# patrickfrey/strusPattern

Hardware: AMD Instinct MI355X
Metric: GB/s input text scanned + matches/s, 10k-regex lexer + 10k-rule automaton (higher is better)
Workload: dtype u64; 1 GPU; configs[4] per-GPU shard: 10001 regexes + 10000 token rules, 12288 docs x 64KiB UTF-8 per step (the same 805 MB resident in HBM every step; configs[4] asks 32 GB per GPU: 39 such steps)

## Files before the change

include/strus_pattern_amd.h:

```cpp
#ifndef STRUS_PATTERN_AMD_H
#define STRUS_PATTERN_AMD_H
#include <stddef.h>
#include <stdint.h>

#ifdef __cplusplus
extern "C" {
#endif

#define SP_OK                    0
#define SP_ERR_INVALID          -1
#define SP_ERR_NOMEM            -2
#define SP_ERR_DEVICE           -3
#define SP_ERR_COMPILE          -4
#define SP_ERR_MATCH            -5
#define SP_ERR_UNAVAILABLE      -6

#define SP_DOC_OK                0
#define SP_DOC_ERR_ORDER         1
#define SP_DOC_ERR_ARENA         2
#define SP_DOC_ERR_KEYTRIGGERS   3
#define SP_DOC_ERR_PASTFOLLOW    4
#define SP_DOC_ERR_RANGE         5
#define SP_DOC_ERR_DATAREF       6
#define SP_DOC_ERR_LEXEMSIZE     7
#define SP_DOC_ERR_INTERNAL      8
#define SP_DOC_ERR_OUTPUT        9

enum sp_join_op {
	SP_OP_SEQUENCE = 0, SP_OP_SEQUENCE_IMM = 1, SP_OP_SEQUENCE_STRUCT = 2,
	SP_OP_WITHIN = 3, SP_OP_WITHIN_STRUCT = 4, SP_OP_ANY = 5, SP_OP_AND = 6
};

enum sp_position_bind {
	SP_BIND_CONTENT = 0, SP_BIND_SUCCESSOR = 1, SP_BIND_PREDECESSOR = 2, SP_BIND_UNIQUE = 3
};

typedef struct sp_lexem {
	uint32_t id;
	uint32_t ordpos;
	uint32_t origpos;
	uint32_t origsize;
} sp_lexem_t;

typedef struct sp_result {
	uint32_t handle;
	uint32_t ordpos;
	uint32_t ordend;
	uint32_t origseg;
	uint32_t origpos;
	uint32_t origendseg;
	uint32_t origend;
	uint32_t item_begin;
	uint32_t item_count;
} sp_result_t;

typedef struct sp_result_item {
	uint32_t variable;
	uint32_t ordpos;
	uint32_t ordend;
	uint32_t origseg;
	uint32_t origpos;
	uint32_t origendseg;
	uint32_t origend;
} sp_result_item_t;

typedef struct sp_matcher_stats {
	double nofProgramsInstalled;
	double nofAltKeyProgramsInstalled;
	double nofSignalsFired;
	double nofTriggersAvgActive;
} sp_matcher_stats_t;

typedef struct sp_matcher sp_matcher_t;
typedef struct sp_matcher_ctx sp_matcher_ctx_t;
typedef struct sp_lexer sp_lexer_t;
typedef struct sp_lexer_ctx sp_lexer_ctx_t;

const char* sp_version(void);
int sp_device_count(void);
void sp_free(void* p);
void sp_test_fail_alloc_above(uint64_t bytes);


sp_matcher_t* sp_matcher_create(void);
void sp_matcher_free(sp_matcher_t* m);
const char* sp_matcher_last_error(const sp_matcher_t* m);

int sp_matcher_define_term_frequency(sp_matcher_t* m, uint32_t termid, double df);
int sp_matcher_push_term(sp_matcher_t* m, uint32_t termid);
int sp_matcher_push_expression(sp_matcher_t* m, int joinop, size_t argc, uint32_t range, uint32_t cardinality);
int sp_matcher_push_pattern(sp_matcher_t* m, const char* name);
int sp_matcher_attach_variable(sp_matcher_t* m, const char* name);
int sp_matcher_define_pattern(sp_matcher_t* m, const char* name, const char* formatstring, int visible);
int sp_matcher_define_option(sp_matcher_t* m, const char* name, double value);
int sp_matcher_compile(sp_matcher_t* m);
uint32_t sp_matcher_pattern_id(const sp_matcher_t* m, const char* name);
const char* sp_matcher_pattern_name(const sp_matcher_t* m, uint32_t handle);
uint32_t sp_matcher_variable_id(const sp_matcher_t* m, const char* name);
const char* sp_matcher_variable_name(const sp_matcher_t* m, uint32_t variable);
size_t sp_matcher_dump_table(const sp_matcher_t* m, uint32_t** out);
int sp_matcher_fast_tier(const sp_matcher_t* m, char* why, size_t whysize);
int sp_matcher_result_set_tier(const sp_matcher_t* m, char* why, size_t whysize, uint32_t* alt_programs);

int sp_matcher_serialize(const sp_matcher_t* m, void** blob, size_t* size);
sp_matcher_t* sp_matcher_deserialize(const void* blob, size_t size, char* err, size_t errsize);

uint32_t sp_matcher_format_count(const sp_matcher_t* m);
const char* sp_matcher_format_string(const sp_matcher_t* m, uint32_t format_handle);

sp_matcher_ctx_t* sp_matcher_ctx_create(const sp_matcher_t* m, int device);
#define SP_CTX_RESULT_SETS       1u
sp_matcher_ctx_t* sp_matcher_ctx_create_ex(const sp_matcher_t* m, int device, uint32_t flags);
void sp_matcher_ctx_free(sp_matcher_ctx_t* c);
const char* sp_matcher_ctx_last_error(const sp_matcher_ctx_t* c);

int sp_matcher_ctx_put_input(sp_matcher_ctx_t* c, const sp_lexem_t* lexems, const uint32_t* origseg, size_t n);
int sp_matcher_ctx_fetch_results(sp_matcher_ctx_t* c, sp_result_t** results, size_t* nresults,
                                 sp_result_item_t** items, size_t* nitems);
int sp_matcher_ctx_fetch_formats(sp_matcher_ctx_t* c, const uint32_t** result_format, const uint32_t** item_format);
int sp_matcher_ctx_statistics(sp_matcher_ctx_t* c, sp_matcher_stats_t* out);
int sp_matcher_ctx_reset(sp_matcher_ctx_t* c);

typedef struct sp_match_batch {
	size_t ndocs;
	size_t nresults;
	size_t nitems;
	sp_result_t* results;
	sp_result_item_t* items;
	uint64_t* doc_result_offsets;
	uint64_t* doc_stats;
	int32_t* doc_status;
	uint32_t* result_format;
	uint32_t* item_format;
} sp_match_batch_t;

int sp_matcher_ctx_match_docs(sp_matcher_ctx_t* c, const sp_lexem_t* lexems, const uint32_t* origseg,
                              const uint64_t* doc_offsets, size_t ndocs, sp_match_batch_t* out);
void sp_match_batch_free(sp_match_batch_t* b);

typedef struct sp_match_device_batch {
	size_t ndocs;
	void* d_results;
	void* d_items;
	void* d_doc_result_offsets;
	void* d_doc_stats;
	void* d_doc_status;
	void* d_counters;
	void* d_result_format;
	void* d_item_format;
} sp_match_device_batch_t;
int sp_matcher_ctx_match_docs_device(sp_matcher_ctx_t* c, const void* d_lexems, const void* d_origseg,
                                     const void* d_doc_offsets, size_t ndocs, size_t nlexems,
                                     void* stream, sp_match_device_batch_t* out);
int sp_matcher_ctx_match_lexed_device(sp_matcher_ctx_t* c, const void* d_lexems, const void* d_doc_ranges,
                                      size_t ndocs, size_t nlexems_hint, void* stream, sp_match_device_batch_t* out);
typedef struct sp_match_finished_batch {
	size_t ndocs;
	void* d_results;
	void* d_items;
	void* d_doc_result_offsets;
	void* d_doc_item_offsets;
	void* d_result_format;
	void* d_item_format;
	void* d_totals;
} sp_match_finished_batch_t;
int sp_matcher_ctx_batch_finish_device(sp_matcher_ctx_t* c, void* stream, sp_match_finished_batch_t* out);
int sp_matcher_ctx_finished_fetch(sp_matcher_ctx_t* c, sp_match_batch_t* out);
int sp_matcher_ctx_last_finish_ms(sp_matcher_ctx_t* c, double* count_ms, double* offsets_ms, double* place_ms);
int sp_matcher_ctx_batch_fetch(sp_matcher_ctx_t* c, sp_match_batch_t* out);
int sp_matcher_ctx_batch_fetch_docs(sp_matcher_ctx_t* c, size_t first_doc, size_t ndocs, sp_match_batch_t* out);
int sp_matcher_ctx_batch_counters(sp_matcher_ctx_t* c, uint64_t counters[8]);
double sp_matcher_ctx_last_kernel_ms(sp_matcher_ctx_t* c);
int sp_matcher_ctx_kernel_kind(const sp_matcher_ctx_t* c);
const char* sp_matcher_ctx_kernel_name(const sp_matcher_ctx_t* c);
int sp_matcher_ctx_batch_status(sp_matcher_ctx_t* c, int32_t* status, size_t ndocs);
int sp_matcher_ctx_grow_arena(sp_matcher_ctx_t* c);
int sp_matcher_ctx_reserve_output(sp_matcher_ctx_t* c, uint64_t results, uint64_t items);
int sp_matcher_ctx_set_arena(sp_matcher_ctx_t* c, uint32_t max_rules, uint32_t max_triggers, uint32_t bucket_capacity,
                             uint32_t max_items, uint32_t max_follow);


sp_lexer_t* sp_lexer_create(void);
void sp_lexer_free(sp_lexer_t* l);
const char* sp_lexer_last_error(const sp_lexer_t* l);
// ... 54 lines not shown
```

struspattern_amd/__init__.py:

```python
import ctypes

import numpy as np

from . import capi
from .capi import SpLexem, SpResult, SpResultItem

__all__ = ["PatternMatcher", "PatternMatcherInstance", "PatternMatcherContext", "PatternLexer", "PatternLexerInstance",
           "PatternLexerContext", "PatternError", "JOIN_OP", "POSITION_BIND"]

SP_CTX_RESULT_SETS = 1
SP_ERR_UNAVAILABLE = -6

JOIN_OP = {"sequence": 0, "sequence_imm": 1, "sequence_struct": 2, "within": 3, "within_struct": 4, "any": 5, "and": 6}

DOC_STATUS = {
    0: "ok", 1: "term events not fed in ascending order", 2: "working set of the document exceeds the arena",
    3: "pattern with too many identical key events defined", 4: "internal: encountered past trigger with follow",
    5: "term event out of range", 6: "illegal free of event data reference",
}


class PatternError(RuntimeError):
    pass

# ... 112 lines not shown
    def matchDocsDevice(self, d_lexems, d_doc_offsets, ndocs, nlexems, stream=0, d_origseg=0):
        out = capi.SpMatchDeviceBatch()
        rc = self._L.sp_matcher_ctx_match_docs_device(self._h, d_lexems, d_origseg or None, d_doc_offsets, ndocs, nlexems, stream or None, ctypes.byref(out))
        if rc != 0:
            raise PatternError("device batch match failed (%d): %s" % (rc, self._err()))
        return out

    def matchLexedDevice(self, d_lexems, d_doc_ranges, ndocs, nlexems_hint, stream=0):
        out = capi.SpMatchDeviceBatch()
        rc = self._L.sp_matcher_ctx_match_lexed_device(self._h, d_lexems, d_doc_ranges, ndocs, nlexems_hint, stream or None, ctypes.byref(out))
        if rc != 0:
            raise PatternError("device batch match failed (%d): %s" % (rc, self._err()))
        return out

    def batchFinishDevice(self, stream=0):
        out = capi.SpMatchFinishedBatch()
        rc = self._L.sp_matcher_ctx_batch_finish_device(self._h, stream or None, ctypes.byref(out))
        if rc != 0:
            raise PatternError("finishing the batch on the device failed (%d): %s" % (rc, self._err()))
        return out

    def finishedFetch(self):
        return self._fetched(lambda b: self._L.sp_matcher_ctx_finished_fetch(self._h, ctypes.byref(b)))

    def lastFinishMs(self):
        a, b, d = ctypes.c_double(-1.0), ctypes.c_double(-1.0), ctypes.c_double(-1.0)
        if self._L.sp_matcher_ctx_last_finish_ms(self._h, ctypes.byref(a), ctypes.byref(b), ctypes.byref(d)) != 0:
            raise PatternError("no timed finish")
        return a.value, b.value, d.value

    def batchFetch(self, first_doc=None, ndocs=None):
        if first_doc is None:
            return self._fetched(lambda b: self._L.sp_matcher_ctx_batch_fetch(self._h, ctypes.byref(b)))
        return self._fetched(lambda b: self._L.sp_matcher_ctx_batch_fetch_docs(self._h, first_doc, ndocs, ctypes.byref(b)))

    def _fetched(self, call):
        b = capi.SpMatchBatch()
        rc = call(b)
        try:
            if rc != 0:
                raise PatternError("fetching the batch failed (%d): %s" % (rc, self._err()))
            ndocs = b.ndocs
            u32p = ctypes.POINTER(ctypes.c_uint32)
            res = np.ctypeslib.as_array(ctypes.cast(b.results, u32p), shape=(b.nresults * 9 + 1,))[:b.nresults * 9].reshape(-1, 9).copy()
            items = np.ctypeslib.as_array(ctypes.cast(b.items, u32p), shape=(b.nitems * 7 + 1,))[:b.nitems * 7].reshape(-1, 7).copy()
            offs = np.ctypeslib.as_array(b.doc_result_offsets, shape=(ndocs + 1,)).copy()
            stats = np.ctypeslib.as_array(b.doc_stats, shape=(ndocs * 4 + 1,))[:ndocs * 4].reshape(-1, 4).copy()
            status = np.ctypeslib.as_array(b.doc_status, shape=(ndocs + 1,))[:ndocs].copy()
            rfmt, ifmt = _formats_of(b)
        finally:
            self._L.sp_match_batch_free(ctypes.byref(b))
        return MatchBatch(res, items, offs, stats, status, rfmt, ifmt)

    def batchCounters(self):
        arr = (ctypes.c_uint64 * 8)()
        rc = self._L.sp_matcher_ctx_batch_counters(self._h, arr)
        if rc != 0:
            raise PatternError("reading batch counters failed: " + self._err())
        return {"results": arr[0], "items": arr[1], "events": arr[2], "failed_docs": arr[3], "handed_over": arr[4], "prof": [arr[4], arr[5], arr[6], arr[7]]}

    def batchStatus(self, ndocs):
        st = np.zeros(ndocs, np.int32)
        rc = self._L.sp_matcher_ctx_batch_status(self._h, st.ctypes.data, ndocs)
        if rc != 0:
            raise PatternError("reading batch status failed: " + self._err())
        return st

    def growArena(self):
        return self._L.sp_matcher_ctx_grow_arena(self._h) == 0

    def reserveOutput(self, results, items):
        self._L.sp_matcher_ctx_reserve_output(self._h, results, items)

    def lastKernelMs(self):
        return self._L.sp_matcher_ctx_last_kernel_ms(self._h)

    def kernelKind(self):
        return self._L.sp_matcher_ctx_kernel_kind(self._h)

    def kernelName(self):
        return self._L.sp_matcher_ctx_kernel_name(self._h).decode()


def _serialize(L, fn, handle, err):
    blob = ctypes.c_void_p()
    size = ctypes.c_size_t()
    if fn(handle, ctypes.byref(blob), ctypes.byref(size)) != 0:
        raise PatternError("serialisation failed: " + err())
    try:
        return ctypes.string_at(blob, size.value)
    finally:
        L.sp_free(blob)


class PatternMatcherInstance:

    def __init__(self, _handle=None):
        self._L = capi.lib()
        self._h = _handle or self._L.sp_matcher_create()
        if not self._h:
            raise PatternError("failed to create pattern matcher instance")

    def serialize(self):
        return _serialize(self._L, self._L.sp_matcher_serialize, self._h, lambda: self._L.sp_matcher_last_error(self._h).decode())

    @classmethod
    def deserialize(cls, blob):
        L = capi.lib()
        err = ctypes.create_string_buffer(256)
        h = L.sp_matcher_deserialize(blob, len(blob), err, 256)
        if not h:
            raise PatternError("cannot load the rule set: " + err.value.decode())
        return cls(_handle=h)

    def __del__(self):
        try:
            if self._h:
                self._L.sp_matcher_free(self._h)
        except Exception:
            pass

    def _chk(self, rc, what):
        if rc != 0:
            raise PatternError("%s: %s" % (what, self._L.sp_matcher_last_error(self._h).decode()))

    def defineTermFrequency(self, termid, df):
        self._chk(self._L.sp_matcher_define_term_frequency(self._h, termid, df), "failed to define term frequency")

    def pushTerm(self, termid):
        self._chk(self._L.sp_matcher_push_term(self._h, termid), "failed to push term on the pattern match expression stack")

    def pushExpression(self, joinop, argc, range_, cardinality=0):
        op = JOIN_OP[joinop] if isinstance(joinop, str) else int(joinop)
        self._chk(self._L.sp_matcher_push_expression(self._h, op, argc, range_, cardinality), "failed to push expression on the pattern match expression stack")

    def pushPattern(self, name):
        self._chk(self._L.sp_matcher_push_pattern(self._h, name.encode()), "failed to push pattern reference on the pattern match expression stack")

    def attachVariable(self, name):
        self._chk(self._L.sp_matcher_attach_variable(self._h, name.encode()), "failed to attach variable to top element of the pattern match expression stack")

    def definePattern(self, name, formatstring="", visible=True):
        self._chk(self._L.sp_matcher_define_pattern(self._h, name.encode(), formatstring.encode(), int(visible)), "failed to close pattern definition on the pattern match expression stack")

    def defineOption(self, name, value=0.0):
        self._chk(self._L.sp_matcher_define_option(self._h, name.encode(), value), "failed to define pattern matching automaton option")

    def compile(self):
        self._chk(self._L.sp_matcher_compile(self._h), "failed to compile (optimize) pattern matching automaton")
        return True

    def createContext(self, device=0, result_sets=False):
        return PatternMatcherContext(self, device, result_sets)

    def patternId(self, name):
        return self._L.sp_matcher_pattern_id(self._h, name.encode())

    def patternName(self, handle):
        s = self._L.sp_matcher_pattern_name(self._h, handle)
        return s.decode() if s else None

    def variableId(self, name):
        return self._L.sp_matcher_variable_id(self._h, name.encode())

    def variableName(self, vid):
        s = self._L.sp_matcher_variable_name(self._h, vid)
        return s.decode() if s else None

    def formatCount(self):
        return int(self._L.sp_matcher_format_count(self._h))

    def formatString(self, handle):
        s = self._L.sp_matcher_format_string(self._h, handle)
        return s.decode() if s else None

    def fastTier(self):
        buf = ctypes.create_string_buffer(256)
        ok = self._L.sp_matcher_fast_tier(self._h, buf, 256)
        return bool(ok), buf.value.decode()

    def resultSetTier(self):
        buf = ctypes.create_string_buffer(256)
        alt = ctypes.c_uint32(0)
        ok = self._L.sp_matcher_result_set_tier(self._h, buf, 256, ctypes.byref(alt))
        return bool(ok), buf.value.decode(), int(alt.value)

    def dumpTable(self):
        p = ctypes.POINTER(ctypes.c_uint32)()
        n = self._L.sp_matcher_dump_table(self._h, ctypes.byref(p))
        arr = np.ctypeslib.as_array(p, shape=(n,)).copy() if n else np.zeros(0, np.uint32)
        self._L.sp_free(p)
        return arr

    def name(self):
        return "std"


class PatternMatcher:

    def getCompileOptionNames(self):
        return ["stopwordOccurrenceFactor", "weightFactor", "maxRange", "exclusive", "maxResultSize"]

    def createInstance(self):
        return PatternMatcherInstance()

    def name(self):
        return "std"


POSITION_BIND = {"content": 0, "successor": 1, "predecessor": 2, "unique": 3}


class LexBatch:
    def __init__(self, lexems, doc_offsets, status):
        self.lexems = lexems
        self.doc_offsets = doc_offsets
        self.status = status

    def doc(self, i):
        return self.lexems[self.doc_offsets[i]:self.doc_offsets[i + 1]]


class PatternLexerContext:

    def __init__(self, instance, device=0):
        self._L = capi.lib()
        self._inst = instance
        self._h = self._L.sp_lexer_ctx_create(instance._h, device)
        if not self._h:
            raise PatternError("failed to create term match context: " + self._L.sp_lexer_last_error(instance._h).decode())

    def __del__(self):
        try:
            if self._h:
                self._L.sp_lexer_ctx_free(self._h)
        except Exception:
            pass

    def _err(self):
        return self._L.sp_lexer_ctx_last_error(self._h).decode(errors="replace")

    def match(self, src):
        buf = bytes(src)
        lex = ctypes.POINTER(SpLexem)()
        n = ctypes.c_size_t()
        rc = self._L.sp_lexer_ctx_match(self._h, buf, len(buf), ctypes.byref(lex), ctypes.byref(n))
        if rc != 0:
            raise PatternError("failed to run pattern matching terms with regular expressions: " + self._err())
        try:
            arr = np.ctypeslib.as_array(ctypes.cast(lex, ctypes.POINTER(ctypes.c_uint32)), shape=(n.value * 4 + 1,))[:n.value * 4].reshape(-1, 4).copy()
        finally:
            self._L.sp_free(lex)
        return arr

    def reset(self):
        self._L.sp_lexer_ctx_reset(self._h)

    def matchDocs(self, text, doc_offsets, check=True):
        buf = bytes(text)
        doc_offsets = np.ascontiguousarray(doc_offsets, dtype=np.uint64)
        ndocs = len(doc_offsets) - 1
        b = capi.SpLexBatch()
        rc = self._L.sp_lexer_ctx_match_docs(self._h, buf, doc_offsets.ctypes.data, ndocs, ctypes.byref(b))
# ... 159 lines not shown
```

struspattern_amd/capi.py:

```python
import ctypes
import os

from . import build as _build

c_u32 = ctypes.c_uint32
c_u64 = ctypes.c_uint64
c_vp = ctypes.c_void_p
c_cp = ctypes.c_char_p
P = ctypes.POINTER


class SpLexem(ctypes.Structure):
    _fields_ = [("id", c_u32), ("ordpos", c_u32), ("origpos", c_u32), ("origsize", c_u32)]


class SpResult(ctypes.Structure):
    _fields_ = [(n, c_u32) for n in ("handle", "ordpos", "ordend", "origseg", "origpos", "origendseg", "origend", "item_begin", "item_count")]


class SpResultItem(ctypes.Structure):
    _fields_ = [(n, c_u32) for n in ("variable", "ordpos", "ordend", "origseg", "origpos", "origendseg", "origend")]


class SpMatcherStats(ctypes.Structure):
    _fields_ = [(n, ctypes.c_double) for n in ("nofProgramsInstalled", "nofAltKeyProgramsInstalled", "nofSignalsFired", "nofTriggersAvgActive")]


class SpMatchBatch(ctypes.Structure):
    _fields_ = [
        ("ndocs", ctypes.c_size_t), ("nresults", ctypes.c_size_t), ("nitems", ctypes.c_size_t),
        ("results", P(SpResult)), ("items", P(SpResultItem)),
        ("doc_result_offsets", P(c_u64)), ("doc_stats", P(c_u64)), ("doc_status", P(ctypes.c_int32)),
        ("result_format", P(c_u32)), ("item_format", P(c_u32)),
    ]


class SpLexBatch(ctypes.Structure):
    _fields_ = [
        ("ndocs", ctypes.c_size_t), ("nlexems", ctypes.c_size_t), ("lexems", P(SpLexem)),
        ("doc_lexem_offsets", P(c_u64)), ("doc_status", P(ctypes.c_int32)),
    ]


class SpLexDeviceBatch(ctypes.Structure):
    _fields_ = [("ndocs", ctypes.c_size_t), ("d_lexems", c_vp), ("d_doc_ranges", c_vp), ("d_doc_status", c_vp), ("d_counters", c_vp)]


class SpMatchDeviceBatch(ctypes.Structure):
    _fields_ = [
        ("ndocs", ctypes.c_size_t), ("d_results", c_vp), ("d_items", c_vp), ("d_doc_result_offsets", c_vp),
        ("d_doc_stats", c_vp), ("d_doc_status", c_vp), ("d_counters", c_vp),
        ("d_result_format", c_vp), ("d_item_format", c_vp),
    ]


class SpMatchFinishedBatch(ctypes.Structure):
    _fields_ = [
        ("ndocs", ctypes.c_size_t), ("d_results", c_vp), ("d_items", c_vp), ("d_doc_result_offsets", c_vp),
        ("d_doc_item_offsets", c_vp), ("d_result_format", c_vp), ("d_item_format", c_vp), ("d_totals", c_vp),
    ]


SIGNATURES = {
    "sp_version": (c_cp, []),
    "sp_device_count": (ctypes.c_int, []),
    "sp_free": (None, [c_vp]),
    "sp_test_fail_alloc_above": (None, [c_u64]),
    "sp_matcher_create": (c_vp, []),
    "sp_matcher_free": (None, [c_vp]),
    "sp_matcher_last_error": (c_cp, [c_vp]),
    "sp_matcher_define_term_frequency": (ctypes.c_int, [c_vp, c_u32, ctypes.c_double]),
    "sp_matcher_push_term": (ctypes.c_int, [c_vp, c_u32]),
    "sp_matcher_push_expression": (ctypes.c_int, [c_vp, ctypes.c_int, ctypes.c_size_t, c_u32, c_u32]),
    "sp_matcher_push_pattern": (ctypes.c_int, [c_vp, c_cp]),
    "sp_matcher_attach_variable": (ctypes.c_int, [c_vp, c_cp]),
    "sp_matcher_define_pattern": (ctypes.c_int, [c_vp, c_cp, c_cp, ctypes.c_int]),
    "sp_matcher_define_option": (ctypes.c_int, [c_vp, c_cp, ctypes.c_double]),
    "sp_matcher_compile": (ctypes.c_int, [c_vp]),
    "sp_matcher_pattern_id": (c_u32, [c_vp, c_cp]),
    "sp_matcher_pattern_name": (c_cp, [c_vp, c_u32]),
    "sp_matcher_variable_id": (c_u32, [c_vp, c_cp]),
    "sp_matcher_variable_name": (c_cp, [c_vp, c_u32]),
    "sp_matcher_dump_table": (ctypes.c_size_t, [c_vp, P(P(c_u32))]),
    "sp_matcher_fast_tier": (ctypes.c_int, [c_vp, ctypes.c_char_p, ctypes.c_size_t]),
    "sp_matcher_result_set_tier": (ctypes.c_int, [c_vp, ctypes.c_char_p, ctypes.c_size_t, P(c_u32)]),
    "sp_matcher_serialize": (ctypes.c_int, [c_vp, P(c_vp), P(ctypes.c_size_t)]),
    "sp_matcher_deserialize": (c_vp, [c_vp, ctypes.c_size_t, ctypes.c_char_p, ctypes.c_size_t]),
    "sp_lexer_serialize": (ctypes.c_int, [c_vp, P(c_vp), P(ctypes.c_size_t)]),
    "sp_lexer_deserialize": (c_vp, [c_vp, ctypes.c_size_t, ctypes.c_char_p, ctypes.c_size_t]),
    "sp_matcher_format_count": (c_u32, [c_vp]),
    "sp_matcher_format_string": (c_cp, [c_vp, c_u32]),
    "sp_matcher_ctx_fetch_formats": (ctypes.c_int, [c_vp, P(P(c_u32)), P(P(c_u32))]),
    "sp_matcher_ctx_create": (c_vp, [c_vp, ctypes.c_int]),
    "sp_matcher_ctx_create_ex": (c_vp, [c_vp, ctypes.c_int, c_u32]),
    "sp_matcher_ctx_free": (None, [c_vp]),
    "sp_matcher_ctx_last_error": (c_cp, [c_vp]),
    "sp_matcher_ctx_put_input": (ctypes.c_int, [c_vp, c_vp, c_vp, ctypes.c_size_t]),
    "sp_matcher_ctx_fetch_results": (ctypes.c_int, [c_vp, P(P(SpResult)), P(ctypes.c_size_t), P(P(SpResultItem)), P(ctypes.c_size_t)]),
    "sp_matcher_ctx_statistics": (ctypes.c_int, [c_vp, P(SpMatcherStats)]),
    "sp_matcher_ctx_reset": (ctypes.c_int, [c_vp]),
    "sp_matcher_ctx_match_docs": (ctypes.c_int, [c_vp, c_vp, c_vp, c_vp, ctypes.c_size_t, P(SpMatchBatch)]),
    "sp_match_batch_free": (None, [P(SpMatchBatch)]),
    "sp_matcher_ctx_match_docs_device": (ctypes.c_int, [c_vp, c_vp, c_vp, c_vp, ctypes.c_size_t, ctypes.c_size_t, c_vp, P(SpMatchDeviceBatch)]),
    "sp_matcher_ctx_match_lexed_device": (ctypes.c_int, [c_vp, c_vp, c_vp, ctypes.c_size_t, ctypes.c_size_t, c_vp, P(SpMatchDeviceBatch)]),
    "sp_matcher_ctx_batch_fetch": (ctypes.c_int, [c_vp, P(SpMatchBatch)]),
    "sp_matcher_ctx_batch_fetch_docs": (ctypes.c_int, [c_vp, ctypes.c_size_t, ctypes.c_size_t, P(SpMatchBatch)]),
    "sp_matcher_ctx_batch_finish_device": (ctypes.c_int, [c_vp, c_vp, P(SpMatchFinishedBatch)]),
    "sp_matcher_ctx_finished_fetch": (ctypes.c_int, [c_vp, P(SpMatchBatch)]),
    "sp_matcher_ctx_last_finish_ms": (ctypes.c_int, [c_vp, P(ctypes.c_double), P(ctypes.c_double), P(ctypes.c_double)]),
    "sp_matcher_ctx_batch_counters": (ctypes.c_int, [c_vp, P(c_u64)]),
    "sp_matcher_ctx_last_kernel_ms": (ctypes.c_double, [c_vp]),
    "sp_matcher_ctx_kernel_kind": (ctypes.c_int, [c_vp]),
    "sp_matcher_ctx_kernel_name": (ctypes.c_char_p, [c_vp]),
    "sp_matcher_ctx_batch_status": (ctypes.c_int, [c_vp, c_vp, ctypes.c_size_t]),
    "sp_matcher_ctx_grow_arena": (ctypes.c_int, [c_vp]),
    "sp_matcher_ctx_reserve_output": (ctypes.c_int, [c_vp, c_u64, c_u64]),
    "sp_matcher_ctx_set_arena": (ctypes.c_int, [c_vp, c_u32, c_u32, c_u32, c_u32, c_u32]),
    "sp_lexer_create": (c_vp, []),
    "sp_lexer_free": (None, [c_vp]),
    "sp_lexer_last_error": (c_cp, [c_vp]),
    "sp_lexer_define_lexem_name": (ctypes.c_int, [c_vp, c_u32, c_cp]),
    "sp_lexer_get_lexem_name": (c_cp, [c_vp, c_u32]),
    "sp_lexer_define_lexem": (ctypes.c_int, [c_vp, c_u32, c_cp, c_u32, c_u32, ctypes.c_int]),
    "sp_lexer_define_symbol": (ctypes.c_int, [c_vp, c_u32, c_u32, c_cp]),
    "sp_lexer_get_symbol": (c_u32, [c_vp, c_u32, c_cp]),
    "sp_lexer_define_option": (ctypes.c_int, [c_vp, c_cp, ctypes.c_double]),
    "sp_lexer_compile": (ctypes.c_int, [c_vp]),
    "sp_lexer_dump_tables": (ctypes.c_size_t, [c_vp, P(P(c_u64))]),
    "sp_lexer_ctx_create": (c_vp, [c_vp, ctypes.c_int]),
    "sp_lexer_ctx_free": (None, [c_vp]),
    "sp_lexer_ctx_last_error": (c_cp, [c_vp]),
    "sp_lexer_ctx_match": (ctypes.c_int, [c_vp, c_cp, ctypes.c_size_t, P(P(SpLexem)), P(ctypes.c_size_t)]),
    "sp_lexer_ctx_reset": (ctypes.c_int, [c_vp]),
    "sp_lexer_ctx_match_docs": (ctypes.c_int, [c_vp, c_cp, c_vp, ctypes.c_size_t, P(SpLexBatch)]),
    "sp_lex_batch_free": (None, [P(SpLexBatch)]),
    "sp_lexer_ctx_match_docs_device": (ctypes.c_int, [c_vp, c_vp, c_vp, ctypes.c_size_t, ctypes.c_size_t, c_vp, P(SpLexDeviceBatch)]),
    "sp_lexer_ctx_batch_fetch_docs": (ctypes.c_int, [c_vp, ctypes.c_size_t, ctypes.c_size_t, P(SpLexBatch)]),
    "sp_lexer_ctx_batch_counters": (ctypes.c_int, [c_vp, P(c_u64)]),
    "sp_lexer_ctx_batch_status": (ctypes.c_int, [c_vp, c_vp, ctypes.c_size_t]),
    "sp_lexer_ctx_last_kernel_ms": (ctypes.c_double, [c_vp]),
    "sp_lexer_ctx_last_kernel_ms_split": (ctypes.c_int, [c_vp, ctypes.POINTER(ctypes.c_double), ctypes.POINTER(ctypes.c_double)]),
    "sp_lexer_ctx_scan_kernel_name": (ctypes.c_char_p, [c_vp]),
    "sp_lexer_ctx_words_kernel_name": (ctypes.c_char_p, [c_vp]),
    "sp_lexer_ctx_last_kernel_ms_split3": (ctypes.c_int, [c_vp, ctypes.POINTER(ctypes.c_double), ctypes.POINTER(ctypes.c_double), ctypes.POINTER(ctypes.c_double)]),
    "sp_lexer_ctx_reserve_output": (ctypes.c_int, [c_vp, c_u64]),
    "sp_lexer_ctx_grow_arena": (ctypes.c_int, [c_vp]),
}

_LIB = None


def lib():
    global _LIB
    if _LIB is None:
        path = _build.LIB
        if _build.needs_build():
            path = _build.build()
        L = ctypes.CDLL(path, mode=ctypes.RTLD_GLOBAL)
        for name, (res, args) in SIGNATURES.items():
            fn = getattr(L, name)
            fn.restype = res
            fn.argtypes = args
        _LIB = L
    return _LIB
```

struspattern_amd/csrc/capi_l2.cpp:

```cpp
#include "../../include/strus_pattern_amd.h"
#include "l2_compile.hpp"
#include "l2_device.h"
#include "l2_fast.h"
#include "l2_join.h"
#include "l2_finish.h"
#include "hip_util.hpp"
#include <hip/hip_runtime_api.h>
#include <cstdlib>
#include <cstdio>
#include <cstring>
#include <new>
#include <stdexcept>
#include <string>
#include <vector>

namespace spa {
hipError_t launchL2Match( const L2Params& P, unsigned nblocks, hipStream_t stream);
hipError_t launchL2Fast( const FastParams& P, unsigned variant, unsigned nblocks, hipStream_t stream);
int fastBlocksPerCU( unsigned variant);
void fastCapacities( unsigned variant, uint32_t& R, uint32_t& T);
unsigned fastVariantNamed( const char* size);
const char* fastKernelName( unsigned variant);
std::string buildFastTables( const FlatTables& ft, std::vector<FastKeyInst>& out, std::vector<FastStatic>* statics);
std::string buildJoinTables( const FlatTables& ft, std::vector<JoinKey>& keytab, std::vector<JoinRule>& rules, std::vector<uint32_t>& filter, uint32_t& maxRange, uint32_t& delimiter, uint32_t& altPrograms);
hipError_t launchL2Join( const JoinParams& P, unsigned nwaves, hipStream_t stream);
void layoutFast( FastSpillLayout& S, uint32_t bucketMeta[16], uint32_t& expShift, const std::vector<FastKeyInst>& keyinst, uint32_t R, uint32_t T, uint32_t maxRules, uint32_t maxStaged);
}

using namespace spa;

#ifndef SPA_L2_WAVES_PER_CU
#define SPA_L2_WAVES_PER_CU 12
#endif

struct sp_matcher
{
	RuleCompiler compiler;
	bool compiled;
	mutable std::string lasterror;
	sp_matcher() :compiled(false){}
};

namespace {

template <class FN>
int guardedCall( std::string& err, int errcode, FN fn)
{
	try { fn(); return SP_OK; }
	catch (const std::bad_alloc&) { err = "memory allocation error in strus pattern"; return SP_ERR_NOMEM; }
	catch (const HipError& e) { err = e.what(); return SP_ERR_DEVICE; }
	catch (const std::exception& e) { err = e.what(); return errcode; }
}

uint32_t alignUp( uint32_t v, uint32_t a) { return (v + a-1) / a * a; }

void layoutArena( ArenaLayout& L)
{
	uint32_t o = 0;
	L.oRules = o;	o += L.maxRules*32;
	L.oTrigs = 0; L.oBIdx = 0; L.oTrigFree = 0;
	L.oBEvent = o;	o += alignUp( 2*16*L.bucketCap, 32);
	L.oBSize = o;	o += 16;
	L.oWindow = o;	o += 64;
	L.oHeap = o;	o += alignUp( L.maxHeap*2, 4);
	L.oFollow = o;	o += alignUp( L.maxFollow*12, 4);
	L.oDispose = o;	o += alignUp( L.maxDispose, 4);
	L.oStop = o;	o += alignUp( (L.nStop?L.nStop:1)*12, 4);
	L.oItems = o;	o += alignUp( L.maxItems*12, 4);
	L.oRefs = o;	o += alignUp( L.maxRefs*2, 4);
	L.oGStack = o;	o += alignUp( L.maxGStack, 4);
	L.oStaged = o;	o += alignUp( L.maxStaged*8, 4);
	L.oRuleFree = o; o += alignUp( L.maxRules, 4);
	L.oItemFree = o; o += alignUp( L.maxItems, 4);
	L.oRefFree = o;	o += alignUp( L.maxRefs, 4);
	L.winChunk = L.winCap/8 < 16 ? 16 : L.winCap/8;
	L.winChunks = L.maxRules/L.winChunk + 64;
	L.oWinArr = o;	o += alignUp( L.winChunks*L.winChunk, 4);
	L.oWinChunk = o; o += 64*8;
	L.oWinFree = o;	o += alignUp( L.winChunks, 4);
	L.oScratch = o;	o += alignUp( 16*L.scratchCap, 4);
	L.totalWords = alignUp( o, 64);
}

}

struct sp_matcher_ctx
{
	const sp_matcher* inst;
	int device;
	std::string lasterror;
	DeviceBuffer dPrograms, dTrigdefs, dKeytab, dKeylist;
	uint32_t keymask, nofStopWords;
	bool fast;
	std::string whyNotFast;
	DeviceBuffer dKeyinst, dStatics, dSpill, dFallbackList;
	bool join, joinAltRules; std::string whyNotJoin; uint32_t joinKeymask, joinMaxRange, joinDelimiter; DeviceBuffer dJoinKeytab, dJoinRules, dJoinFilter, dJoinCounts;
	std::vector<FastKeyInst> fastKeyinst;
	FastSpillLayout fastSpill; uint32_t fastBucketMeta[ 16]; uint32_t fastExpShift;
	unsigned fastWaves, fastBlocksPerCU, fastVariant;
	uint32_t fastMaxRules, fastMaxStaged;
	ArenaLayout arena;
	DeviceBuffer dArena; unsigned arenaWaves;
	DeviceBuffer dCursor, dCounters;
	DeviceBuffer dLexems, dOrigseg, dDocOffsets, dResults, dItems, dDocRange, dDocStats, dDocStatus;
	DeviceBuffer dResultFormat, dItemFormat;
	bool withFormats;
	std::vector<uint32_t> curResultFormat, curItemFormat;
	uint64_t resultCapacity, itemCapacity, minResultCapacity, minItemCapacity;
	size_t lastNdocs;
	hipEvent_t evStart, evStop; bool evValid;
	hipStream_t lastStream;
	hipStream_t own;
	bool withItems;
	unsigned numCUs;
	std::vector<sp_lexem_t> curLexems;
	std::vector<uint32_t> curOrigseg; bool curHasSeg;
	sp_matcher_stats_t lastStats;
	DeviceBuffer fResults, fItems, fResultFormat, fItemFormat, fDocResultOffsets, fDocItemOffsets, fTotals, fKept, fCovered, fCursor;
	bool haveBatch, finished;
	hipStream_t finishStream;
	hipEvent_t evFinish[ 4]; bool evFinishValid;

	sp_matcher_ctx() :inst(0),device(0),keymask(0),nofStopWords(0),fast(false),join(false),joinAltRules(false),joinKeymask(0),joinMaxRange(0),joinDelimiter(0),fastWaves(0),fastBlocksPerCU(0),fastVariant(4),fastMaxRules(2048),fastMaxStaged(32768),arenaWaves(0),withFormats(false),resultCapacity(0),itemCapacity(0),minResultCapacity(0),minItemCapacity(0)
		,lastNdocs(0),evStart(0),evStop(0),evValid(false),lastStream(0),own(0),withItems(true),numCUs(256),curHasSeg(false),haveBatch(false),finished(false),finishStream(0),evFinishValid(false)
	{
		std::memset( evFinish, 0, sizeof(evFinish));
		std::memset( &arena, 0, sizeof(arena));
		std::memset( &fastSpill, 0, sizeof(fastSpill)); std::memset( fastBucketMeta, 0, sizeof(fastBucketMeta));
		std::memset( &lastStats, 0, sizeof(lastStats));
		arena.maxRules = 1024; arena.maxTrigs = 1024; arena.bucketCap = 256; arena.maxItems = 2048;
		arena.maxRefs = 1024; arena.maxFollow = 256; arena.maxDispose = 512; arena.maxHeap = 256;
		arena.maxGStack = 64; arena.maxStaged = 1024; arena.winCap = 128; arena.scratchCap = 256;
	}
};

static void copySync( sp_matcher_ctx* c, void* dst, const void* src, size_t n, hipMemcpyKind kind)
{
	HIP_CHECK( hipMemcpyAsync( dst, src, n, kind, c->own));
	HIP_CHECK( hipStreamSynchronize( c->own));
}

extern "C" {

const char* sp_version(void) { return "struspattern_amd 0.1 (gfx950)"; }

int sp_device_count(void)
{
	int n = 0;
	if (hipGetDeviceCount( &n) != hipSuccess) return 0;
	return n;
}

void sp_free( void* p) { std::free( p); }

void sp_test_fail_alloc_above( uint64_t bytes) { allocFailureThreshold().store( bytes, std::memory_order_relaxed); }

sp_matcher_t* sp_matcher_create(void)
{
	try { return new sp_matcher(); } catch (...) { return 0; }
}
void sp_matcher_free( sp_matcher_t* m) { delete m; }
const char* sp_matcher_last_error( const sp_matcher_t* m) { return m->lasterror.c_str(); }

#define MGUARD( CODE, BODY) return guardedCall( m->lasterror, CODE, [&]{ BODY; })

int sp_matcher_define_term_frequency( sp_matcher_t* m, uint32_t termid, double df)
{ MGUARD( SP_ERR_INVALID, m->compiler.defineTermFrequency( termid, df)); }
int sp_matcher_push_term( sp_matcher_t* m, uint32_t termid)
{ MGUARD( SP_ERR_INVALID, m->compiler.pushTerm( termid)); }
int sp_matcher_push_expression( sp_matcher_t* m, int joinop, size_t argc, uint32_t range, uint32_t cardinality)
{ MGUARD( SP_ERR_INVALID, m->compiler.pushExpression( joinop, argc, range, cardinality)); }
int sp_matcher_push_pattern( sp_matcher_t* m, const char* name)
{ MGUARD( SP_ERR_INVALID, m->compiler.pushPattern( name ? name : "")); }
int sp_matcher_attach_variable( sp_matcher_t* m, const char* name)
{ MGUARD( SP_ERR_INVALID, m->compiler.attachVariable( name ? name : "")); }
int sp_matcher_define_pattern( sp_matcher_t* m, const char* name, const char* formatstring, int visible)
{ MGUARD( SP_ERR_INVALID, m->compiler.definePattern( name ? name : "", formatstring ? formatstring : "", visible != 0)); }
int sp_matcher_define_option( sp_matcher_t* m, const char* name, double value)
{ MGUARD( SP_ERR_INVALID, m->compiler.defineOption( name ? name : "", value)); }
int sp_matcher_compile( sp_matcher_t* m)
{ MGUARD( SP_ERR_COMPILE, m->compiler.compile(); m->compiled = true); }

uint32_t sp_matcher_pattern_id( const sp_matcher_t* m, const char* name) { return m->compiler.patterns().get( name); }
const char* sp_matcher_pattern_name( const sp_matcher_t* m, uint32_t handle) { return m->compiler.patterns().key( handle); }
uint32_t sp_matcher_variable_id( const sp_matcher_t* m, const char* name) { return m->compiler.variables().get( name); }
const char* sp_matcher_variable_name( const sp_matcher_t* m, uint32_t variable) { return m->compiler.variables().key( variable); }

uint32_t sp_matcher_format_count( const sp_matcher_t* m) { return m->compiler.formatCount(); }
const char* sp_matcher_format_string( const sp_matcher_t* m, uint32_t format_handle) { return m->compiler.formatString( format_handle); }

int sp_matcher_ctx_kernel_kind( const sp_matcher_ctx_t* c) { return c->join ? 2 : c->fast ? 1 : 0; }
const char* sp_matcher_ctx_kernel_name( const sp_matcher_ctx_t* c)
{
	if (c->join) return "spa_l2_join_kernel";
	if (!c->fast) return "spa_l2_match_kernel";
	return fastKernelName( c->fastVariant);
}

int sp_matcher_fast_tier( const sp_matcher_t* m, char* why, size_t whysize)
{
	try
	{
		FlatTables ft;
		m->compiler.flatten( ft);
		std::vector<FastKeyInst> ki;
		const std::string reason = buildFastTables( ft, ki, 0);
		if (why && whysize) { std::strncpy( why, reason.c_str(), whysize-1); why[ whysize-1] = 0; }
		return reason.empty() ? 1 : 0;
	}
	catch (const std::exception& e)
	{
		if (why && whysize) { std::strncpy( why, e.what(), whysize-1); why[ whysize-1] = 0; }
		return 0;
	}
}

static std::string buildResultSetTables( const sp_matcher* m, const FlatTables& ft, std::vector<JoinKey>& keytab, std::vector<JoinRule>& rules,
					std::vector<uint32_t>& filter, uint32_t& maxRange, uint32_t& delimiter, uint32_t& altPrograms)
{
	altPrograms = 0;
	if (m->compiler.exclusive()) return "the `exclusive` option (its outcome depends on the order of the results)";
	return buildJoinTables( ft, keytab, rules, filter, maxRange, delimiter, altPrograms);
}

int sp_matcher_result_set_tier( const sp_matcher_t* m, char* why, size_t whysize, uint32_t* alt_programs)
{
	if (alt_programs) *alt_programs = 0;
	try
	{
		FlatTables ft;
		m->compiler.flatten( ft);
		std::vector<JoinKey> jk; std::vector<JoinRule> jr; std::vector<uint32_t> jf;
		uint32_t maxRange = 0, delimiter = 0, alt = 0;
		const std::string reason = buildResultSetTables( m, ft, jk, jr, jf, maxRange, delimiter, alt);
		if (why && whysize) { std::strncpy( why, reason.c_str(), whysize-1); why[ whysize-1] = 0; }
		if (alt_programs && reason.empty()) *alt_programs = alt;
		return reason.empty() ? 1 : 0;
	}
	catch (const std::exception& e)
	{
		if (why && whysize) { std::strncpy( why, e.what(), whysize-1); why[ whysize-1] = 0; }
		return 0;
	}
}

int sp_matcher_serialize( const sp_matcher_t* m, void** blob, size_t* size)
{
	*blob = 0; *size = 0;
	return guardedCall( m->lasterror, SP_ERR_INVALID, [&]{
		std::vector<uint8_t> buf;
		m->compiler.save( buf, m->compiled);
		*blob = std::malloc( buf.size() ? buf.size() : 1);
		if (!*blob) throw std::bad_alloc();
		std::memcpy( *blob, buf.data(), buf.size());
		*size = buf.size();
	});
}
sp_matcher_t* sp_matcher_deserialize( const void* blob, size_t size, char* err, size_t errsize)
{
	sp_matcher* m = 0;
	try
	{
		m = new sp_matcher();
		m->compiled = m->compiler.load( blob, size);
		return m;
	}
	catch (const std::exception& e)
	{
		if (err && errsize) { std::strncpy( err, e.what(), errsize-1); err[ errsize-1] = 0; }
		delete m;
		return 0;
	}
}

size_t sp_matcher_dump_table( const sp_matcher_t* m, uint32_t** out)
{
	std::vector<uint32_t> buf = m->compiler.dump();
	*out = (uint32_t*)std::malloc( buf.size()*sizeof(uint32_t) + 4);
	if (!*out) return 0;
	std::memcpy( *out, buf.data(), buf.size()*sizeof(uint32_t));
	return buf.size();
}

sp_matcher_ctx_t* sp_matcher_ctx_create( const sp_matcher_t* m, int device)
{
	return sp_matcher_ctx_create_ex( m, device, 0);
}

sp_matcher_ctx_t* sp_matcher_ctx_create_ex( const sp_matcher_t* m, int device, uint32_t flags)
{
	sp_matcher_ctx* c = 0;
	if (flags & ~(uint32_t)SP_CTX_RESULT_SETS)
	{
		m->lasterror = "unknown context flags";
		return 0;
	}
	try
	{
		c = new sp_matcher_ctx();
		c->inst = m; c->device = device;
		int ndev = 0;
		hipError_t e = hipGetDeviceCount( &ndev);
		if (e != hipSuccess || ndev <= 0 || device < 0 || device >= ndev)
		{
			m->lasterror = "no usable HIP device: the rule automaton runs on the GPU only (no CPU fallback)";
			delete c; return 0;
		}
		HIP_CHECK( hipSetDevice( device));
		hipDeviceProp_t prop;
		HIP_CHECK( hipGetDeviceProperties( &prop, device));
		c->numCUs = prop.multiProcessorCount > 0 ? (unsigned)prop.multiProcessorCount : 256u;

		FlatTables ft;
		m->compiler.flatten( ft);
		c->dPrograms.upload( ft.programs.data(), ft.programs.size()*sizeof(DevProgram));
		c->dTrigdefs.upload( ft.trigdefs.data(), ft.trigdefs.size()*sizeof(DevTrigDef));
		c->dKeytab.upload( ft.keytab.data(), ft.keytab.size()*sizeof(DevKeyEntry));
		c->dKeylist.upload( ft.keylist.data(), ft.keylist.size()*sizeof(DevKeyRef));
		c->keymask = (uint32_t)ft.keytab.size()-1;
		c->nofStopWords = ft.nofStopWords;
		c->arena.nStop = ft.nofStopWords;
		c->withFormats = m->compiler.formatCount() != 0;
		{
			std::vector<FastKeyInst> ki;
			std::vector<FastStatic> ks;
			c->whyNotFast = buildFastTables( ft, ki, &ks);
			const char* sw = getenv( "SPA_L2_FAST");
			if (sw && sw[0] == '0') c->whyNotFast = "disabled by SPA_L2_FAST=0";
			c->fast = c->whyNotFast.empty();
			if (c->fast)
			{
				if (ki.empty()) ki.resize( 1);
				c->dKeyinst.upload( ki.data(), ki.size()*sizeof(FastKeyInst));
				c->dStatics.upload( ks.data(), ks.size()*sizeof(FastStatic));
				c->fastKeyinst.swap( ki);
				if (const char* e = getenv( "SPA_L2_FAST_SIZE")) c->fastVariant = fastVariantNamed( e);
				if (const char* e = getenv( "SPA_L2_FAST_MAXRULES")) c->fastMaxRules = (uint32_t)atoi( e);
				if (const char* e = getenv( "SPA_L2_FAST_MAXSTAGED")) c->fastMaxStaged = (uint32_t)atoi( e);
				if (c->fastMaxRules > 4095) c->fastMaxRules = 4095;
			}
			if (getenv( "SPA_L2_VERBOSE")) fprintf( stderr, "[spa] fast tier: %s\n", c->fast ? "on" : c->whyNotFast.c_str());
		}
		if (const char* e = getenv( "SPA_L2_JOIN")) if (e[0] == '1') flags |= SP_CTX_RESULT_SETS;
		if (flags & SP_CTX_RESULT_SETS)
		{
			std::vector<JoinKey> jk; std::vector<JoinRule> jr; std::vector<uint32_t> jf;
			uint32_t altPrograms = 0;
			c->whyNotJoin = buildResultSetTables( m, ft, jk, jr, jf, c->joinMaxRange, c->joinDelimiter, altPrograms);
			c->join = c->whyNotJoin.empty();
			if (c->join)
			{
				c->dJoinKeytab.upload( jk.data(), jk.size()*sizeof(JoinKey)); c->dJoinRules.upload( jr.data(), jr.size()*sizeof(JoinRule)); c->dJoinFilter.upload( jf.data(), jf.size()*sizeof(uint32_t));
				c->joinKeymask = (uint32_t)jk.size()-1;
				c->joinAltRules = altPrograms != 0;
			}
			if (getenv( "SPA_L2_VERBOSE")) fprintf( stderr, "[spa] result-set mode: %s\n", c->join ? "join kernel" : c->whyNotJoin.c_str());
		}
		c->dCursor.alloc( 256);
		c->dCounters.alloc( SPC_COUNT*sizeof(uint64_t));
		HIP_CHECK( hipStreamCreateWithFlags( &c->own, hipStreamNonBlocking));
		HIP_CHECK( hipEventCreate( &c->evStart));
		HIP_CHECK( hipEventCreate( &c->evStop));
		return c;
	}
	catch (const std::exception& e)
	{
		m->lasterror = e.what();
		delete c;
		return 0;
	}
}

void sp_matcher_ctx_free( sp_matcher_ctx_t* c)
{
	if (!c) return;
	if (c->own) { (void)hipSetDevice( c->device); (void)hipStreamSynchronize( c->own); (void)hipStreamDestroy( c->own); }
	if (c->evStart) (void)hipEventDestroy( c->evStart);
	if (c->evStop) (void)hipEventDestroy( c->evStop);
	for (int i=0; i<4; ++i) if (c->evFinish[ i]) (void)hipEventDestroy( c->evFinish[ i]);
	delete c;
}
const char* sp_matcher_ctx_last_error( const sp_matcher_ctx_t* c) { return c->lasterror.c_str(); }

int sp_matcher_ctx_set_arena( sp_matcher_ctx_t* c, uint32_t max_rules, uint32_t max_triggers, uint32_t bucket_capacity,
				uint32_t max_items, uint32_t max_follow)
{
	if (max_rules) { c->arena.maxRules = max_rules; c->arena.maxHeap = max_rules; c->arena.maxDispose = max_rules; c->arena.winCap = max_rules/4 < 64 ? 64 : max_rules/4; }
	if (max_triggers) c->arena.maxTrigs = max_triggers;
	if (bucket_capacity) c->arena.bucketCap = bucket_capacity;
	if (max_items) { c->arena.maxItems = max_items; c->arena.maxRefs = max_items; }
	if (max_follow) { c->arena.maxFollow = max_follow; }
	c->arenaWaves = 0;
	return SP_OK;
}

}

namespace {

void copyOutBatch( sp_matcher_ctx* c, size_t firstDoc, size_t ndocs, const uint64_t* counters, sp_match_batch_t* out)
{
	const bool whole = (firstDoc == 0 && ndocs == c->lastNdocs);
	std::vector<uint64_t> range( ndocs*2+2);
	if (ndocs) copySync( c, range.data(), (const uint64_t*)c->dDocRange.ptr + 2*firstDoc, ndocs*2*sizeof(uint64_t), hipMemcpyDeviceToHost);
	out->ndocs = ndocs;
	out->doc_stats = (uint64_t*)std::malloc( (ndocs*4+1)*sizeof(uint64_t));
	out->doc_status = (int32_t*)std::malloc( (ndocs+1)*sizeof(int32_t));
	out->doc_result_offsets = (uint64_t*)std::malloc( (ndocs+1)*sizeof(uint64_t));
	if (!out->doc_stats || !out->doc_status || !out->doc_result_offsets) throw std::bad_alloc();
	if (ndocs)
	{
		copySync( c, out->doc_stats, (const uint64_t*)c->dDocStats.ptr + 4*firstDoc, ndocs*4*sizeof(uint64_t), hipMemcpyDeviceToHost);
		copySync( c, out->doc_status, (const int32_t*)c->dDocStatus.ptr + firstDoc, ndocs*sizeof(int32_t), hipMemcpyDeviceToHost);
	}
	const uint64_t devResults = counters[ SPC_RESULTS] < c->resultCapacity ? counters[ SPC_RESULTS] : c->resultCapacity;
	const uint64_t devItems = counters[ SPC_ITEMS] < c->itemCapacity ? counters[ SPC_ITEMS] : c->itemCapacity;
	std::vector<sp_result_t> raw;
	std::vector<sp_result_item_t> rawitems;
	std::vector<uint32_t> rawrf, rawif;
	if (whole)
	{
		raw.resize( devResults+1); rawitems.resize( devItems+1);
// ... 194 lines not shown
		size_t maxWaves = ((size_t)48 << 30) / perWave;
		if (maxWaves < 4) maxWaves = 4;
		if (nwaves > maxWaves) { nblocks = (unsigned)maxWaves; nwaves = nblocks; }
	}
	if (c->arenaWaves < nwaves)
	{
		if (getenv( "SPA_L2_VERBOSE")) fprintf( stderr, "[spa] arena: rules %u bucket %u items %u refs %u staged %u winCap %u -> %.2f MB per wave, %u waves\n", c->arena.maxRules, c->arena.bucketCap, c->arena.maxItems, c->arena.maxRefs, c->arena.maxStaged, c->arena.winCap, c->arena.totalWords*4/1e6, nwaves);
		size_t perWave = (size_t)c->arena.totalWords * sizeof(uint32_t);
		size_t full = (size_t)c->numCUs*SPA_L2_WAVES_PER_CU;
		if (full * perWave > ((size_t)48 << 30)) full = ((size_t)48 << 30) / perWave;
		unsigned alloc = (nwaves >= 64 && nwaves < full && !rerun) ? (unsigned)full : nwaves;
		c->arenaWaves = 0;
		c->dArena.alloc( (size_t)alloc * perWave);
		c->arenaWaves = alloc;
	}
	uint64_t wantResults = (uint64_t)nlexems*2 + 1024;
	if (wantResults < c->minResultCapacity) wantResults = c->minResultCapacity;
	if (wantResults > 0xFFFFFFFFull) wantResults = 0xFFFFFFFFull;
	if (c->resultCapacity < wantResults)
	{
		c->resultCapacity = 0;
		c->dResults.alloc( wantResults*sizeof(sp_result_t));
		c->resultCapacity = wantResults;
	}
	uint64_t wantItems = (uint64_t)nlexems*6 + 1024;
	if (wantItems < c->minItemCapacity) wantItems = c->minItemCapacity;
	if (wantItems > 0xFFFFFFFFull) wantItems = 0xFFFFFFFFull;
	if (c->itemCapacity < wantItems)
	{
		c->itemCapacity = 0;
		c->dItems.alloc( wantItems*sizeof(sp_result_item_t));
		c->itemCapacity = wantItems;
	}
	if (c->withFormats)
	{
		c->dResultFormat.reserve( c->resultCapacity*sizeof(uint32_t));
		c->dItemFormat.reserve( c->itemCapacity*2*sizeof(uint32_t));
	}
	c->dDocRange.reserve( (ndocs+1)*2*sizeof(uint64_t));
	c->dDocStats.reserve( (ndocs+1)*4*sizeof(uint64_t));
	c->dDocStatus.reserve( (ndocs+1)*sizeof(int32_t));

	HIP_CHECK( hipMemsetAsync( c->dCursor.ptr, 0, 256, stream));
	if (!rerun) HIP_CHECK( hipMemsetAsync( c->dCounters.ptr, 0, SPC_COUNT*sizeof(uint64_t), stream));
	else HIP_CHECK( hipMemsetAsync( (uint64_t*)c->dCounters.ptr + SPC_FAILED, 0, sizeof(uint64_t), stream));

	L2Params P;
	std::memset( &P, 0, sizeof(P));
	P.programs = (const DevProgram*)c->dPrograms.ptr;
	P.trigdefs = (const DevTrigDef*)c->dTrigdefs.ptr;
	P.keytab = (const DevKeyEntry*)c->dKeytab.ptr;
	P.keylist = (const DevKeyRef*)c->dKeylist.ptr;
	P.keymask = c->keymask; P.nofStopWords = c->nofStopWords;
	P.io = batchIO( c, d_lexems, d_origseg, d_doc_offsets, d_doc_ranges, ndocs);
	P.arenaBase = (uint32_t*)c->dArena.ptr; P.arena = c->arena;
	HIP_CHECK( hipEventRecord( c->evStart, stream));
	if (rerun)
	{
		const uint32_t n = (uint32_t)rerun->size();
		c->dFallbackList.reserve( (ndocs+1)*sizeof(uint32_t));
		HIP_CHECK( hipMemcpyAsync( c->dFallbackList.ptr, rerun->data(), n*sizeof(uint32_t), hipMemcpyHostToDevice, stream));
		HIP_CHECK( hipMemcpyAsync( (uint32_t*)c->dCursor.ptr + 2, &n, sizeof(uint32_t), hipMemcpyHostToDevice, stream));
		HIP_CHECK( hipStreamSynchronize( stream));
		P.docList = (const uint32_t*)c->dFallbackList.ptr; P.docListCount = (const uint32_t*)c->dCursor.ptr + 2;
		P.io.docCursor = (uint32_t*)c->dCursor.ptr + 1;
		HIP_CHECK( launchL2Match( P, nblocks, stream));
	}
	else if (c->join)
	{
		JoinParams J;
		std::memset( &J, 0, sizeof(J));
		c->dJoinCounts.reserve( (nlexems + 64) * sizeof(uint32_t));
		J.filter = (const uint32_t*)c->dJoinFilter.ptr; J.counts = (uint32_t*)c->dJoinCounts.ptr; J.countsCapacity = nlexems;
		J.keytab = (const JoinKey*)c->dJoinKeytab.ptr; J.keymask = c->joinKeymask; J.rules = (const JoinRule*)c->dJoinRules.ptr; J.maxRange = c->joinMaxRange; J.delimiter = c->joinDelimiter; J.altRules = c->joinAltRules ? 1u : 0u;
		J.io = P.io;
		const size_t jslots = (size_t)c->numCUs * 32;
		HIP_CHECK( launchL2Join( J, (unsigned)(ndocs < jslots ? (ndocs ? ndocs : 1) : jslots), stream));
	}
	else if (c->fast)
	{
		uint32_t fR = 0, fT = 0;
		fastCapacities( c->fastVariant, fR, fT);
		layoutFast( c->fastSpill, c->fastBucketMeta, c->fastExpShift, c->fastKeyinst, fR, fT, c->fastMaxRules, c->fastMaxStaged);
		if (!c->fastBlocksPerCU) c->fastBlocksPerCU = (unsigned)fastBlocksPerCU( c->fastVariant);
		size_t fslots = (size_t)c->numCUs * c->fastBlocksPerCU;
		unsigned fblocks = (unsigned)(ndocs < fslots ? ndocs : fslots);
		if (fblocks == 0) fblocks = 1;
		if (c->fastWaves < fblocks)
		{
			c->fastWaves = 0;
			const size_t spillSlots = fblocks >= 64 ? fslots : fblocks;
			c->dSpill.alloc( spillSlots * (size_t)c->fastSpill.totalWords * sizeof(uint32_t));
			c->fastWaves = (unsigned)spillSlots;
			if (getenv( "SPA_L2_VERBOSE")) fprintf( stderr, "[spa] fast tier: %u waves/CU, LDS capacities R %u T %u, spill %.2f MB per wave\n", c->fastBlocksPerCU, fR, fT, c->fastSpill.totalWords*4/1e6);
		}
		c->dFallbackList.reserve( (ndocs+1)*sizeof(uint32_t));
		FastParams F;
		std::memset( &F, 0, sizeof(F));
		F.keyinst = (const FastKeyInst*)c->dKeyinst.ptr; F.statics = (const FastStatic*)c->dStatics.ptr; F.keytab = (const FastKeyEntry*)c->dKeytab.ptr;
		F.keymask = c->keymask; F.nofStopWords = c->nofStopWords;
		F.io = P.io;
		std::memcpy( F.bucketMeta, c->fastBucketMeta, sizeof(F.bucketMeta)); F.expShift = c->fastExpShift;
		F.spill = c->fastSpill; F.spillBase = (uint32_t*)c->dSpill.ptr;
		F.fallbackList = (uint32_t*)c->dFallbackList.ptr; F.fallbackCount = (uint32_t*)c->dCursor.ptr + 2;
		F.diag = (uint32_t*)c->dCursor.ptr + 16; F.prof = (uint64_t*)((uint32_t*)c->dCursor.ptr + 32);
		HIP_CHECK( launchL2Fast( F, c->fastVariant, fblocks, stream));
		P.docList = F.fallbackList; P.docListCount = F.fallbackCount;
		P.io.docCursor = (uint32_t*)c->dCursor.ptr + 1;
		const unsigned listBlocks = nblocks < 2*c->numCUs ? nblocks : 2*c->numCUs;
		HIP_CHECK( launchL2Match( P, listBlocks, stream));
	}
	else
	{
		HIP_CHECK( launchL2Match( P, nblocks, stream));
	}
	HIP_CHECK( hipEventRecord( c->evStop, stream));
	c->evValid = true; c->lastStream = stream; c->lastNdocs = ndocs; c->haveBatch = true;
}

void deviceBatch( const sp_matcher_ctx* c, size_t ndocs, sp_match_device_batch_t* out)
{
	out->ndocs = ndocs;
	out->d_results = c->dResults.ptr; out->d_items = c->dItems.ptr;
	out->d_doc_result_offsets = c->dDocRange.ptr;
	out->d_doc_stats = c->dDocStats.ptr; out->d_doc_status = c->dDocStatus.ptr;
	out->d_counters = c->dCounters.ptr;
	out->d_result_format = c->withFormats ? c->dResultFormat.ptr : 0;
	out->d_item_format = c->withFormats ? c->dItemFormat.ptr : 0;
}

}

extern "C" {

int sp_matcher_ctx_match_docs_device( sp_matcher_ctx_t* c, const void* d_lexems, const void* d_origseg,
				      const void* d_doc_offsets, size_t ndocs, size_t nlexems,
				      void* stream, sp_match_device_batch_t* out)
{
	return guardedCall( c->lasterror, SP_ERR_INVALID, [&]{
		if (ndocs >= 0xFFFFFFFFull) throw std::runtime_error( "too many documents in one batch");
		launchBatch( c, d_lexems, d_origseg, d_doc_offsets, ndocs, nlexems, (hipStream_t)stream);
		if (out) deviceBatch( c, ndocs, out);
	});
}

int sp_matcher_ctx_match_lexed_device( sp_matcher_ctx_t* c, const void* d_lexems, const void* d_doc_ranges,
				       size_t ndocs, size_t nlexems_hint, void* stream, sp_match_device_batch_t* out)
{
	return guardedCall( c->lasterror, SP_ERR_INVALID, [&]{
		if (ndocs >= 0xFFFFFFFFull) throw std::runtime_error( "too many documents in one batch");
		launchBatch( c, d_lexems, 0, 0, ndocs, nlexems_hint, (hipStream_t)stream, d_doc_ranges);
		if (out) deviceBatch( c, ndocs, out);
	});
}

int sp_matcher_ctx_batch_counters( sp_matcher_ctx_t* c, uint64_t counters[8])
{
	return guardedCall( c->lasterror, SP_ERR_DEVICE, [&]{
		HIP_CHECK( hipSetDevice( c->device));
		HIP_CHECK( hipStreamSynchronize( c->lastStream));
		copySync( c, counters, c->dCounters.ptr, SPC_COUNT*sizeof(uint64_t), hipMemcpyDeviceToHost);
		if (c->fast && getenv( "SPA_L2_VERBOSE"))
		{
			uint32_t diag[ 16];
			copySync( c, diag, (const uint32_t*)c->dCursor.ptr + 16, sizeof(diag), hipMemcpyDeviceToHost);
#ifdef SPA_PROF
			uint64_t prof[ 12];
			copySync( c, prof, (const uint32_t*)c->dCursor.ptr + 32, sizeof(prof), hipMemcpyDeviceToHost);
			double tot = 0; for (int i=0; i<6; ++i) tot += (double)prof[ i];
			
			fprintf( stderr, "[spa] fast tier phases (share of wave cycles): scan+fire %.1f%% install %.1f%% deactivate %.1f%% expiry %.1f%% results %.1f%% fetch %.1f%% | inside deactivation: loads %.1f%% ranks+queue %.1f%% replay %.1f%% (%.2f replay steps, %.2f batches, %.2f rules per event); %.0f cycles per event\n",
				100*prof[0]/tot, 100*prof[1]/tot, 100*prof[2]/tot, 100*prof[3]/tot, 100*prof[4]/tot, 100*prof[5]/tot, 100*prof[6]/tot, 100*prof[7]/tot, 100*prof[11]/tot,
				(double)prof[ 8] / (double)(counters[ SPC_EVENTS] ? counters[ SPC_EVENTS] : 1), (double)prof[ 9] / (double)(counters[ SPC_EVENTS] ? counters[ SPC_EVENTS] : 1), (double)prof[ 10] / (double)(counters[ SPC_EVENTS] ? counters[ SPC_EVENTS] : 1),
				tot / (double)(counters[ SPC_EVENTS] ? counters[ SPC_EVENTS] : 1));
#endif
			if (diag[ 0])
			{
				fprintf( stderr, "[spa] fast tier handed %u of %zu documents to the general kernel; by reason:", diag[ 0], c->lastNdocs);
				for (int i=1; i<16; ++i) if (diag[ i]) fprintf( stderr, " [%d]=%u", i, diag[ i]);
				fprintf( stderr, "\n");
			}
		}
	});
}

int sp_matcher_ctx_batch_finish_device( sp_matcher_ctx_t* c, void* stream_, sp_match_finished_batch_t* out)
{
	if (out) std::memset( out, 0, sizeof(*out));
	return guardedCall( c->lasterror, SP_ERR_INVALID, [&]{
// ... 272 lines not shown
```

struspattern_amd/csrc/l2_fast.h:

```cpp
#ifndef SPA_L2_FAST_H
#define SPA_L2_FAST_H
#include <stdint.h>
#include "l2_tables.h"
#include "l2_device.h"

namespace spa {

struct FastKeyInst
{
	uint32_t resultHandle;
	uint32_t formatHandle;
	uint32_t pastEvent;
	uint32_t meta;
	struct { uint32_t event; uint32_t info; } trig[ 3];
	uint32_t hw0;
	uint32_t ranksA;
	uint32_t ranksB;
	uint32_t totals;
	uint32_t items;
	uint32_t flags;
};
enum {
	FKI_VALUE_MASK=0xFu, FKI_COUNT_SHIFT=4, FKI_COUNT_MASK=0x1Fu, FKI_RANGE_SHIFT=9, FKI_RANGE_MASK=0x3Fu,
	FKI_NTRIG_SHIFT=15, FKI_NTRIG_MASK=0x3u, FKI_PASTSTOP_SHIFT=17, FKI_PASTSTOP_MASK=0xFFu,
	FTI_SIGVAL_MASK=0xFu, FTI_SIGTYPE_SHIFT=4, FTI_SIGTYPE_MASK=0x7u, FTI_INSTALL=1u<<7, FTI_KEY=1u<<8,
	FTI_BUCKET_SHIFT=9, FTI_HASVAR=1u<<13, FTI_DELSTOP_SHIFT=14, FTI_DELSTOP_MASK=0xFFu, FTI_VAR_SHIFT=24,
	FKF_BATCH_STATIC=1u,
	FKF_END_SET=2u,
	FKF_START_SET=4u,
	FKF_RESULT_NOW=8u,
	FKF_DISPOSE_NOW=16u
};
struct FastStatic
{
	uint32_t ev0, info0;
	uint32_t ev1, info1;
	uint32_t hw0;
	uint32_t misc;
	uint32_t ranks;
	uint32_t totals;
};
enum {
	FSI_BUCKET_SHIFT=16, FSI_RANK_SHIFT=20, FSI_LAST=1u<<28, FSI_PRESENT=1u<<29, FSI_SLOT_SHIFT=30,
	FSM_RANGE_MASK=0x3Fu, FSM_EXPRANK_SHIFT=6, FSM_EXPCLOSE_SHIFT=14,
	FSM_END_SET=1u<<22, FSM_START_SET=1u<<23, FSM_RESULT_NOW=1u<<24, FSM_DISPOSE_NOW=1u<<25, FSM_BATCH_COMPACT=1u<<26
};

enum {
	H_VALUE_MASK=0xFu, H_COUNT_SHIFT=4, H_COUNT_MASK=0x1Fu, H_END_SHIFT=9, H_END_MASK=0xFFu, H_ENDZERO=1u<<17,
	H_DONE=1u<<18, H_ACTIVE=1u<<19, H_TMASK_SHIFT=20, H_TMASK_MASK=0x7u, H_NITEMS_SHIFT=23, H_NITEMS_MASK=0x3u, H_HASSTART=1u<<25,
	H_COLD=1u<<26,
	H_LISTED=1u<<27,
	H_VISIBLE=1u<<28,
	H_MARK=1u<<31
};

enum {S_HASSTART=1u, S_DONE=2u, S_FIN=4u, S_DEL=8u, S_ODD=16u, S_RESULT=32u, S_HASLIST=64u, S_TOOK=128u};
struct Sim
{
	uint32_t value, count, end, startLex, nItems, it0, it1, it2, nFires, flags;
};
SPA_HD static inline void fireLocal( Sim& s, uint32_t info, uint32_t esord, uint32_t elex, uint32_t withItems)
{
	const uint32_t sigtype = (info >> FTI_SIGTYPE_SHIFT) & FTI_SIGTYPE_MASK, sigval = info & FTI_SIGVAL_MASK;
	uint32_t m = 0, f = 0, took = 0;
	s.nFires += 1;
	if (sigtype == SIG_ANY)
	{
		took = 1;
		if (s.count > 0) { m = 1; s.count -= 1; f = (s.count == 0); if (s.end < esord+1) s.end = esord+1; }
	}
	else if (sigtype == SIG_SEQUENCE || sigtype == SIG_SEQUENCE_IMM)
	{
		if (sigval == s.value && (sigtype == SIG_SEQUENCE ? (s.end <= esord) : (s.end == esord)))
		{
			s.end = esord+1; s.value = sigval-1;
			if (s.count > 0) { s.count -= 1; m = (s.count == 0); } else m = 1;
			f = (s.value == 0); took = 1;
		}
	}
	else if (sigtype == SIG_WITHIN)
	{
		if ((sigval & s.value) != 0 && s.end <= esord)
		{
			s.end = esord+1; s.value &= ~sigval;
			if (s.count > 0) { s.count -= 1; m = (s.count == 0); } else m = 1;
			took = 1;
		}
	}
	else
	{
		s.count = 0; s.value = 0; s.flags |= S_DEL;
		return;
	}
	if (took)
	{
		if ((info & FTI_HASVAR) && withItems)
		{
			const uint32_t item = elex | ((info >> FTI_VAR_SHIFT) << 24);
			if ((s.flags & S_DONE) && !(s.flags & S_HASLIST)) {}
			else if (s.nItems == 0) { s.it0 = item; s.nItems = 1; }
			else if (s.nItems == 1) { s.it1 = item; s.nItems = 2; }
			else if (s.nItems == 2) { s.it2 = item; s.nItems = 3; }
			else s.flags |= S_ODD;
		}
		if (!(s.flags & S_HASSTART)) { s.startLex = elex; s.flags |= S_TOOK; if (esord) s.flags |= S_HASSTART; }
	}
	if (m)
	{
		if (!(s.flags & S_DONE)) { s.flags |= S_DONE | S_RESULT; if (s.nItems) s.flags |= S_HASLIST; }
		if (f) s.flags |= S_FIN;
	}
}

struct FastKeyEntry
{
	uint32_t event;
	uint32_t kiBegin;
	uint32_t kiCount;
	uint32_t stopIdx;
};

enum {FAST_LISTCAP=64, FAST_EXPCAP=1024, FAST_MAXSTOP=64, FAST_SPILL_BUCKET=1024, FAST_VARIANTS=5, FAST_RQCAP=192};

struct FastSpillLayout
{
	uint32_t maxRules;
	uint32_t oCold;
	uint32_t oHot, oLink;
	uint32_t oKi, oLex0;
	uint32_t oFree;
	uint32_t oEnt;
	uint32_t oStaged;
	uint32_t maxStaged;
	uint32_t oList;
	uint32_t oExp;
	uint32_t totalWords;
};

enum {SPD_FAST_FALLBACK=100};

struct FastParams
{
	const FastKeyInst* keyinst;
	const FastStatic* statics;
	const FastKeyEntry* keytab;
	uint32_t keymask;
	uint32_t nofStopWords;
	uint32_t expShift;
	uint32_t bucketMeta[ 16];
	FastSpillLayout spill;
	uint32_t* spillBase;
	uint32_t* fallbackList; uint32_t* fallbackCount;
	uint32_t* diag;
	L2BatchIO io;
	uint64_t* prof;
};

}
#endif
```

struspattern_amd/csrc/l2_fast_kernel.hip:

```cpp
#include <hip/hip_runtime.h>
#include <stdint.h>
#include "l2_fast.h"
#include "l2_device.h"
#include "wave_scan.h"

using namespace spa;

namespace {

typedef uint16_t u16;
typedef uint8_t u8;

typedef const __attribute__((address_space(4))) FastParams& KP;
__device__ __forceinline__ KP kernelParams() { return *(const __attribute__((address_space(4))) FastParams*)__builtin_amdgcn_kernarg_segment_ptr(); }

#define WAVE_FENCE() __builtin_amdgcn_fence( __ATOMIC_ACQ_REL, "wavefront")

enum {NIL16=0xFFFFu};

#ifdef SPA_PROF
#define PROF_DECL u64 prof_t0 = __builtin_amdgcn_s_memtime()
#define PROF_ADD( SLOT) do { const u64 prof_t1 = __builtin_amdgcn_s_memtime(); w.prof[ SLOT] += prof_t1 - prof_t0; prof_t0 = prof_t1; } while (0)
#else
#define PROF_DECL do {} while (0)
// ... 5 lines not shown
{
	a += ~(a>>5);
	a +=  (a<<3);
	a ^=  (a>>4);
	return a;
}
__device__ __forceinline__ void st4( void* p, u32 a, u32 b, u32 c, u32 d) { u32x4 v; v.x = a; v.y = b; v.z = c; v.w = d; *(u32x4*)p = v; }
__device__ __forceinline__ uint4 ldu4( const void* p)
{
	uint4 v = ld4( p);
	v.x = uni( v.x); v.y = uni( v.y); v.z = uni( v.z); v.w = uni( v.w);
	return v;
}
__device__ __forceinline__ u32 waveScanOr( u32 v)
{
	v |= (u32)__builtin_amdgcn_update_dpp( 0, (int)v, 0x111, 0xF, 0xF, true);
	v |= (u32)__builtin_amdgcn_update_dpp( 0, (int)v, 0x112, 0xF, 0xF, true);
	v |= (u32)__builtin_amdgcn_update_dpp( 0, (int)v, 0x114, 0xF, 0xF, true);
	v |= (u32)__builtin_amdgcn_update_dpp( 0, (int)v, 0x118, 0xF, 0xF, true);
	v |= (u32)__builtin_amdgcn_update_dpp( 0, (int)v, 0x142, 0xA, 0xF, false);
	v |= (u32)__builtin_amdgcn_update_dpp( 0, (int)v, 0x143, 0xC, 0xF, false);
	return v;
}
__device__ __forceinline__ u32 fromLaneBelow( u32 v)
{
	const u32 t = (u32)__builtin_amdgcn_ds_bpermute( (int)((LANE - 1u) << 2), (int)v);
	return LANE ? t : 0u;
}
__device__ __forceinline__ u32 byteField( u32 c0, u32 c1, u32 c2, u32 c3, u32 h)
{
	const u32 wsel = h >> 2;
	const u32 v = wsel == 0 ? c0 : wsel == 1 ? c1 : wsel == 2 ? c2 : c3;
	return (v >> ((h & 3u)*8)) & 0xFFu;
}
__device__ __forceinline__ void byteInc( u32& c0, u32& c1, u32& c2, u32& c3, u32 h)
{
	const u32 inc = 1u << ((h & 3u)*8), ws = h >> 2;
	c0 += ws == 0 ? inc : 0u; c1 += ws == 1 ? inc : 0u; c2 += ws == 2 ? inc : 0u; c3 += ws == 3 ? inc : 0u;
}

#define FALLBACK( WHY) do { w.err = SPD_FAST_FALLBACK; w.why = (WHY); } while (0)
enum {FB_LEXEMS=1, FB_DISPOSE=2, FB_ITEM_AFTER_RESULT=3, FB_ITEMS=4, FB_STAGED=5, FB_RULES=8, FB_BUCKET_SIZE=9, FB_POSLEXEMS=10};

__device__ __forceinline__ bool endLE( u32 hw, u32 pos) { return (hw & H_ENDZERO) || ((hw >> H_END_SHIFT) & H_END_MASK) != ((pos + 1u) & 0xFFu); }
__device__ __forceinline__ bool endEQ( u32 hw, u32 pos) { return (hw & H_ENDZERO) ? (pos == 0) : (((hw >> H_END_SHIFT) & H_END_MASK) == (pos & 0xFFu)); }
__device__ __forceinline__ u32 withEnd( u32 hw, u32 end) { return (hw & ~((H_END_MASK << H_END_SHIFT) | H_ENDZERO)) | ((end & 0xFFu) << H_END_SHIFT); }

template <bool SMALL> struct FreeId { typedef u8 type; };
template <> struct FreeId<false> { typedef u16 type; };
template <int R, int T>
struct LdsDoc
{
	u32 hot[ R];
	u32 kl[ R];
	u64 ent[ T];
	u32 bsize[ 16];
	u32 bmeta[ 16];
	u16 link[ 3*R];
	typename FreeId<(R <= 256)>::type freeS[ R];
	u16 exp[ FAST_EXPCAP];
	u16 expCnt[ 64];
	u16 list[ FAST_LISTCAP];
	u16 rq[ FAST_RQCAP];
};

struct Wave
{
	u32* sp;
	u32 curpos, timestamp, nInstalled, nAlt, nSignals, nTrig, openLo, openHi;
	u32 freeN, usedL, sFreeN, usedS;
	u32 nDispose, nStaged, nStagedItems, err;
	u32 lbase;
	u32 spill;
	u32 why;
	u32 posLexems;
	u32 stopLex, stopOrd, stopTs;
	u32 bsizeV, bmetaV;
	u32 expCntV;
#ifdef SPA_PROF
	u64 prof[ 12];
#endif
};

template <int R, int T>
struct Engine
{
typedef LdsDoc<R,T> Lds;
typedef __attribute__((address_space(3))) Lds& LR;

template <bool SP> static __device__ __forceinline__ u32 ldHot( LR L, const Wave& w, KP P, u32 r) { if (!SP || r < (u32)R) return L.hot[ r]; return w.sp[ P.spill.oHot + (r - R)]; }
template <bool SP> static __device__ __forceinline__ void stHot( LR L, const Wave& w, KP P, u32 r, u32 v) { if (!SP || r < (u32)R) L.hot[ r] = v; else w.sp[ P.spill.oHot + (r - R)] = v; }
template <bool SP> static __device__ __forceinline__ u32 ldLink( LR L, const Wave& w, KP P, u32 r, u32 j) { if (!SP || r < (u32)R) return (u32)L.link[ 3*r + j]; return w.sp[ P.spill.oLink + 3*(r - R) + j]; }
template <bool SP> static __device__ __forceinline__ void stLink( LR L, const Wave& w, KP P, u32 r, u32 j, u32 v) { if (!SP || r < (u32)R) L.link[ 3*r + j] = (u16)v; else w.sp[ P.spill.oLink + 3*(r - R) + j] = v; }
template <bool SP> static __device__ __forceinline__ void ldLinks( LR L, const Wave& w, KP P, u32 r, u32& l0, u32& l1, u32& l2)
{
	if (!SP || r < (u32)R) { l0 = (u32)L.link[ 3*r]; l1 = (u32)L.link[ 3*r+1]; l2 = (u32)L.link[ 3*r+2]; }
	else { const u32* q = &w.sp[ P.spill.oLink + 3*(r - R)]; l0 = q[0]; l1 = q[1]; l2 = q[2]; }
}
template <bool SP> static __device__ __forceinline__ u32 ldKl( LR L, const Wave& w, KP P, u32 r) { if (!SP || r < (u32)R) return L.kl[ r]; return w.sp[ P.spill.oKi + (r - R)]; }
template <bool SP> static __device__ __forceinline__ void stKl( LR L, const Wave& w, KP P, u32 r, u32 ki, u32 lx)
{ const u32 v = ki | (lx << 20); if (!SP || r < (u32)R) L.kl[ r] = v; else w.sp[ P.spill.oKi + (r - R)] = v; }
static __device__ __forceinline__ u32 keyLexemOf( u32 kl, u32 lbase) { return lbase - ((lbase - (kl >> 20)) & 0xFFFu); }
template <bool SP> static __device__ __forceinline__ u32 ldExp( LR L, const Wave& w, KP P, u32 row, u32 i)
{ const u32 C = (u32)FAST_EXPCAP >> P.expShift; if (!SP || i < C) return (u32)L.exp[ row*C + i]; return w.sp[ P.spill.oExp + row*P.spill.maxRules + (i - C)]; }
template <bool SP> static __device__ __forceinline__ void stExp( LR L, const Wave& w, KP P, u32 row, u32 i, u32 r)
{ const u32 C = (u32)FAST_EXPCAP >> P.expShift; if (!SP || i < C) L.exp[ row*C + i] = (u16)r; else w.sp[ P.spill.oExp + row*P.spill.maxRules + (i - C)] = r; }
template <bool SP> static __device__ __forceinline__ u32 ldEv( LR L, const Wave& w, KP P, u32 h, u32 meta, u32 pos)
{ if (!SP || pos < (meta >> 16)) return (u32)L.ent[ (meta & 0xFFFFu) + pos]; return w.sp[ P.spill.oEnt + 2*(h*FAST_SPILL_BUCKET + pos - (meta >> 16))]; }
template <bool SP> static __device__ __forceinline__ uint2 ldEnt( LR L, const Wave& w, KP P, u32 h, u32 meta, u32 pos)
{ if (!SP || pos < (meta >> 16)) { const u64 v = L.ent[ (meta & 0xFFFFu) + pos]; return make_uint2( (u32)v, (u32)(v >> 32)); } return *(const uint2*)&w.sp[ P.spill.oEnt + 2*(h*FAST_SPILL_BUCKET + pos - (meta >> 16))]; }
template <bool SP> static __device__ __forceinline__ u32 ldTs( LR L, const Wave& w, KP P, u32 h, u32 meta, u32 pos) { return ldEnt<SP>( L, w, P, h, meta, pos).y; }
template <bool SP> static __device__ __forceinline__ void stEnt( LR L, const Wave& w, KP P, u32 h, u32 meta, u32 pos, u32 e, u32 t)
{
	if (!SP || pos < (meta >> 16)) L.ent[ (meta & 0xFFFFu) + pos] = (u64)e | ((u64)t << 32);
	else *(uint2*)&w.sp[ P.spill.oEnt + 2*(h*FAST_SPILL_BUCKET + pos - (meta >> 16))] = make_uint2( e, t);
}
template <bool SP> static __device__ __forceinline__ u32 ldList( LR L, const Wave& w, KP P, u32 i) { if (!SP || i < (u32)FAST_LISTCAP) return (u32)L.list[ i]; return w.sp[ P.spill.oList + i]; }
static __device__ __forceinline__ void pushList( LR L, Wave& w, KP P, u32 i, u32 r)
{
	if (i < (u32)FAST_LISTCAP) { if (LANE == 0) L.list[ i] = (u16)r; }
	else { w.spill = 1; if (LANE == 0) w.sp[ P.spill.oList + i] = r; }
}

enum {STAGED_LINE=0x80000000u};
static __device__ __forceinline__ void stageLineResult( Wave& w, KP P, u32 at, u32 ki, u32 startLex, u32 endLex, u32 nStatic, u32 hasNew, u32 newVar, u32 keyLex)
{
	u32* S = &w.sp[ P.spill.oStaged + 8*at];
	st4( S, (u32)STAGED_LINE | ki, 0u, startLex, endLex);
	*(uint2*)(S+4) = make_uint2( nStatic | (hasNew << 2) | (newVar << 8), keyLex);
}
static __device__ __forceinline__ void stageResult( Wave& w, KP P, u32 at, u32 handle, u32 fmt, u32 startLex, u32 endLex, u32 nItems, u32 vars, u32 i0, u32 i1, u32 i2)
{
	u32* S = &w.sp[ P.spill.oStaged + 8*at];
	st4( S, handle, fmt, startLex, endLex);
	st4( S+4, nItems | (vars << 8), i0, i1, i2);
}

template <bool SP>
static __device__ __forceinline__ void fireSignal( LR L, Wave& w, KP P, u32 tsv, u32 sord)
{
	const u32 tid = tsv & 0xFFFFu, r = tid >> 2;
	const u32 sigval = (tsv >> 16) & 0xFu, sigtype = (tsv >> 20) & 0x7u, hasVar = (tsv >> 23) & 1u, variable = tsv >> 24;
	u32 hw = uni( ldHot<SP>( L, w, P, r));
	w.nSignals += 1;
	u32 value = hw & H_VALUE_MASK, count = (hw >> H_COUNT_SHIFT) & H_COUNT_MASK;
	bool match = false, take = false, fin = false;
	switch (sigtype)
	{
		case SIG_ANY:
			take = true;
			if (count > 0) { match = true; --count; fin = (count == 0); hw = withEnd( hw, sord+1); }
			break;
		case SIG_SEQUENCE:
		case SIG_SEQUENCE_IMM:
			if (sigval == value && (sigtype == SIG_SEQUENCE ? endLE( hw, sord) : endEQ( hw, sord)))
			{
				hw = withEnd( hw, sord+1); value = sigval-1;
				if (count > 0) { --count; match = (count == 0); } else match = true;
				fin = (value == 0); take = true;
			}
			break;
		case SIG_WITHIN:
			if ((sigval & value) != 0 && endLE( hw, sord))
			{
				hw = withEnd( hw, sord+1); value &= ~sigval;
				if (count > 0) { --count; match = (count == 0); } else match = true;
				take = true;
			}
			break;
		default:
			hw &= ~(H_VALUE_MASK | (H_COUNT_MASK << H_COUNT_SHIFT));
			if (!(hw & H_LISTED))
			{
				if (w.nDispose < P.spill.maxRules) { pushList( L, w, P, w.nDispose, r); w.nDispose += 1; hw |= H_LISTED; } else FALLBACK( FB_DISPOSE);
			}
			if (LANE == 0) stHot<SP>( L, w, P, r, hw);
			return;
	}
	const bool done = (hw & H_DONE) != 0;
	u32 nItems = (hw >> H_NITEMS_SHIFT) & H_NITEMS_MASK;
	bool newItem = false, newStart = false;
	if (take)
	{
		if (hasVar && P.io.withItems)
		{
			if (done)
			{
				if (nItems) { FALLBACK( FB_ITEM_AFTER_RESULT); return; }
			}
			else if (nItems < 3u) newItem = true;
			else { FALLBACK( FB_ITEMS); return; }
		}
		newStart = !(hw & H_HASSTART);
	}
	if (!done && match && !(hw & H_COLD))
	{
		if (hw & H_VISIBLE)
		{
			if (w.nStaged < P.spill.maxStaged)
			{
				const u32 kl = uni( ldKl<SP>( L, w, P, r)), lx = keyLexemOf( kl, w.lbase);
				if (LANE == 0) stageLineResult( w, P, w.nStaged, kl & 0xFFFFFu, newStart ? w.lbase : lx, w.lbase, nItems, newItem ? 1u : 0u, variable, lx);
				w.nStaged += 1; w.nStagedItems += nItems + (newItem ? 1u : 0u);
			}
			else FALLBACK( FB_STAGED);
		}
		if (newItem) ++nItems;
	}
	else if (!done && (match || newItem || newStart))
	{
		u32* cold = &w.sp[ P.spill.oCold + 8*r];
		u32 handle, fmt, startLex, it0, it1, it2;
		if (hw & H_COLD)
		{
			const uint4 c0 = ldu4( cold), c1 = ldu4( cold + 4);
			handle = c0.x; fmt = c0.y; startLex = c0.z; it0 = c0.w; it1 = c1.x; it2 = c1.y;
		}
		else
		{
			const u32 kl = uni( ldKl<SP>( L, w, P, r)), lx = keyLexemOf( kl, w.lbase);
			const u32* K = (const u32*)&P.keyinst[ kl & 0xFFFFFu];
			handle = ldu( K); fmt = ldu( K+1);
			const u32 vars = ldu( K+14);
			startLex = lx;
			it0 = lx | ((vars & 0xFFu) << 24); it1 = lx | (((vars >> 8) & 0xFFu) << 24); it2 = lx | (((vars >> 16) & 0xFFu) << 24);
		}
		if (newItem)
		{
			const u32 item = w.lbase | (variable << 24);
			if (nItems == 0) it0 = item; else if (nItems == 1) it1 = item; else it2 = item;
			++nItems;
		}
		if (newStart) startLex = w.lbase;
		if (match)
		{
			if (handle)
			{
				if (w.nStaged < P.spill.maxStaged)
				{
					const u32 ia = nItems == 3 ? it2 : nItems == 2 ? it1 : it0;
					const u32 ib = nItems == 3 ? it1 : it0;
					const u32 ic = it0;
					const u32 vars = nItems == 0 ? 0u : nItems == 1 ? (ia >> 24) : nItems == 2 ? ((ia >> 24) | ((ib >> 24) << 8)) : ((ia >> 24) | ((ib >> 24) << 8) | ((ic >> 24) << 16));
					if (LANE == 0) stageResult( w, P, w.nStaged, handle, fmt, startLex, w.lbase, nItems, vars, ia & 0xFFFFFFu, ib & 0xFFFFFFu, ic & 0xFFFFFFu);
					w.nStaged += 1; w.nStagedItems += nItems;
				}
				else FALLBACK( FB_STAGED);
			}
		}
		else
		{
			if (LANE == 0) { st4( cold, handle, fmt, startLex, it0); *(uint2*)(cold + 4) = make_uint2( it1, it2); }
			hw |= H_COLD;
			WAVE_FENCE();
		}
	}
	if (newStart && sord) hw |= H_HASSTART;
	hw = (hw & ~(H_VALUE_MASK | (H_COUNT_MASK << H_COUNT_SHIFT) | (H_NITEMS_MASK << H_NITEMS_SHIFT))) | value | (count << H_COUNT_SHIFT) | (nItems << H_NITEMS_SHIFT);
	if (match && !done) hw |= H_DONE;
	if (match && fin && !(hw & H_LISTED))
	{
		if (w.nDispose < P.spill.maxRules) { pushList( L, w, P, w.nDispose, r); w.nDispose += 1; hw |= H_LISTED; } else FALLBACK( FB_DISPOSE);
	}
	if (LANE == 0) stHot<SP>( L, w, P, r, hw);
}

static __device__ __forceinline__ bool fireBatch( LR L, Wave& w, KP P, const u64 m, const u32 tsv, const u32 sord)
{
	const bool hit = ((m >> LANE) & 1ull) != 0;
	const u32 nh = (u32)__popcll( m);
	if (w.nDispose + nh > (u32)FAST_LISTCAP) return false;
	const u32 tid = tsv & 0xFFFFu, r = hit ? (tid >> 2) : 0u;
	const u32 sigval = (tsv >> 16) & 0xFu, sigtype = (tsv >> 20) & 0x7u, hasVar = (tsv >> 23) & 1u, variable = tsv >> 24;
	u32 hw = 0;
	if (hit) hw = __hip_atomic_fetch_or( &L.hot[ r], (u32)H_MARK, __ATOMIC_RELAXED, __HIP_MEMORY_SCOPE_WAVEFRONT);
	if (__ballot( hit && (hw & (u32)H_MARK)))
	{
		if (hit) __hip_atomic_fetch_and( &L.hot[ r], ~(u32)H_MARK, __ATOMIC_RELAXED, __HIP_MEMORY_SCOPE_WAVEFRONT);
		WAVE_FENCE();
		return false;
	}
	u32 value = hw & H_VALUE_MASK, count = (hw >> H_COUNT_SHIFT) & H_COUNT_MASK;
	bool match = false, take = false, fin = false;
	const bool isDel = hit && sigtype != (u32)SIG_ANY && sigtype != (u32)SIG_SEQUENCE && sigtype != (u32)SIG_SEQUENCE_IMM && sigtype != (u32)SIG_WITHIN;
	if (hit && !isDel)
	{
		if (sigtype == (u32)SIG_ANY)
		{
			take = true;
			if (count > 0) { match = true; --count; fin = (count == 0); hw = withEnd( hw, sord+1); }
		}
		else if (sigtype == (u32)SIG_WITHIN)
		{
			if ((sigval & value) != 0 && endLE( hw, sord))
			{
				hw = withEnd( hw, sord+1); value &= ~sigval;
				if (count > 0) { --count; match = (count == 0); } else match = true;
				take = true;
			}
		}
		else if (sigval == value && (sigtype == (u32)SIG_SEQUENCE ? endLE( hw, sord) : endEQ( hw, sord)))
		{
			hw = withEnd( hw, sord+1); value = sigval-1;
			if (count > 0) { --count; match = (count == 0); } else match = true;
			fin = (value == 0); take = true;
		}
	}
	if (isDel) hw &= ~(H_VALUE_MASK | (H_COUNT_MASK << H_COUNT_SHIFT));
	const bool done = (hw & H_DONE) != 0;
	u32 nItems = (hw >> H_NITEMS_SHIFT) & H_NITEMS_MASK;
	bool newItem = false, newStart = false;
	u32 why = 0;
	if (take)
	{
		if (hasVar && P.io.withItems)
		{
			if (done) { if (nItems) why = FB_ITEM_AFTER_RESULT; }
			else if (nItems < 3u) newItem = true;
			else why = FB_ITEMS;
		}
		newStart = !(hw & H_HASSTART);
	}
	const bool live = hit && !isDel && !done;
	const bool lineCase = live && match && !(hw & H_COLD);
	const bool recCase = live && !lineCase && (match || newItem || newStart);
	u32 handle = 0, fmt = 0, startLex = 0, it0 = 0, it1 = 0, it2 = 0, kl = 0, lx = 0;
	if ((lineCase && (hw & H_VISIBLE)) || (recCase && !(hw & H_COLD))) { kl = L.kl[ r]; lx = keyLexemOf( kl, w.lbase); }
	u32* cold = &w.sp[ P.spill.oCold + 8*r];
	u32 nItemsOut = nItems;
	if (recCase)
	{
		if (hw & H_COLD)
		{
			const uint4 c0 = ld4( cold); const uint2 c1 = *(const uint2*)(cold + 4);
			handle = c0.x; fmt = c0.y; startLex = c0.z; it0 = c0.w; it1 = c1.x; it2 = c1.y;
		}
		else
		{
			const u32* K = (const u32*)&P.keyinst[ kl & 0xFFFFFu];
			handle = K[ 0]; fmt = K[ 1];
			const u32 vars = K[ 14];
			startLex = lx;
			it0 = lx | ((vars & 0xFFu) << 24); it1 = lx | (((vars >> 8) & 0xFFu) << 24); it2 = lx | (((vars >> 16) & 0xFFu) << 24);
		}
		if (newItem)
		{
			const u32 item = w.lbase | (variable << 24);
			if (nItems == 0) it0 = item; else if (nItems == 1) it1 = item; else it2 = item;
			nItemsOut = nItems + 1u;
		}
		if (newStart) startLex = w.lbase;
	}
	else if (lineCase && newItem) nItemsOut = nItems + 1u;
	const bool resLine = lineCase && (hw & H_VISIBLE) != 0, resRec = recCase && match && handle != 0;
	const u64 resM = __ballot( resLine || resRec);
	const u32 nres = (u32)__popcll( resM);
	const bool listNow = hit && !(hw & H_LISTED) && (isDel || (match && fin));
	const u64 listM = __ballot( listNow);
	const u32 nlist = (u32)__popcll( listM);
	{
		const u64 whyM = __ballot( why != 0);
		u32 fb = 0;
		if (whyM) fb = (u32)__builtin_amdgcn_readlane( why, (u32)__builtin_ctzll( whyM));
		else if (w.nStaged + nres > P.spill.maxStaged) fb = FB_STAGED;
		else if (w.nDispose + nlist > P.spill.maxRules) fb = FB_DISPOSE;
		if (fb) { FALLBACK( fb); return true; }
	}
	w.nSignals += nh;
	if (nres)
	{
		const u32 at = w.nStaged + (u32)__popcll( resM & lanesBelow());
		if (resLine) stageLineResult( w, P, at, kl & 0xFFFFFu, newStart ? w.lbase : lx, w.lbase, nItems, newItem ? 1u : 0u, variable, lx);
		if (resRec)
		{
			const u32 ia = nItemsOut == 3 ? it2 : nItemsOut == 2 ? it1 : it0;
			const u32 ib = nItemsOut == 3 ? it1 : it0;
			const u32 ic = it0;
			const u32 vars = nItemsOut == 0 ? 0u : nItemsOut == 1 ? (ia >> 24) : nItemsOut == 2 ? ((ia >> 24) | ((ib >> 24) << 8)) : ((ia >> 24) | ((ib >> 24) << 8) | ((ic >> 24) << 16));
			stageResult( w, P, at, handle, fmt, startLex, w.lbase, nItemsOut, vars, ia & 0xFFFFFFu, ib & 0xFFFFFFu, ic & 0xFFFFFFu);
		}
		w.nStaged += nres;
		const u32 itemsIncl = waveScanAdd( (resLine || resRec) ? nItemsOut : 0u);
		w.nStagedItems += (u32)__builtin_amdgcn_readlane( itemsIncl, 63);
	}
	if (recCase && !match)
	{
		st4( cold, handle, fmt, startLex, it0); *(uint2*)(cold + 4) = make_uint2( it1, it2);
		hw |= H_COLD;
	}
	if (nlist)
	{
		if (listNow) L.list[ w.nDispose + (u32)__popcll( listM & lanesBelow())] = (u16)r;
		w.nDispose += nlist;
	}
	if (hit)
	{
		if (listNow) hw |= H_LISTED;
		if (!isDel)
		{
			if (newStart && sord) hw |= H_HASSTART;
			hw = (hw & ~(H_VALUE_MASK | (H_COUNT_MASK << H_COUNT_SHIFT) | (H_NITEMS_MASK << H_NITEMS_SHIFT))) | value | (count << H_COUNT_SHIFT) | ((live ? nItemsOut : nItems) << H_NITEMS_SHIFT);
			if (match && !done) hw |= H_DONE;
		}
		L.hot[ r] = hw & ~(u32)H_MARK;
	}
	WAVE_FENCE();
	return true;
}

template <bool SP>
static __device__ __forceinline__ void deactivateList( LR L, Wave& w, KP P, const u32 nD, const u32 nE, const u32 row)
{
	const u32 n = nD + nE;
	for (u32 base=0; base<n && !w.err; base+=64)
	{
		const u32 nb = (n - base) < 64u ? (n - base) : 64u;
		const bool have = LANE < nb;
		const bool isExp = base + LANE >= nD;
		u32 r = 0, hw = 0;
#if defined(SPA_PROF) && !defined(SPA_PROF_INSTALL)
		u64 pd0 = __builtin_amdgcn_s_memtime();
#define PROF_D( SLOT) do { if (__ballot( hw == 0xFFFFFFFFu)) w.err = SPD_ERR_INTERNAL; const u64 pd1 = __builtin_amdgcn_s_memtime(); w.prof[ SLOT] += pd1 - pd0; pd0 = pd1; } while (0)
#else
#define PROF_D( SLOT) do {} while (0)
#endif
		if (have)
		{
			r = isExp ? ldExp<SP>( L, w, P, row, nE - 1u - (base + LANE - nD)) : ldList<SP>( L, w, P, base + LANE);
			hw = ldHot<SP>( L, w, P, r);
		}
		const bool act = have && (hw & H_ACTIVE) && !(isExp && (hw & H_LISTED));
		const u32 mask = act ? ((hw >> H_TMASK_SHIFT) & H_TMASK_MASK) : 0u;
		if (act) stHot<SP>( L, w, P, r, hw & ~(H_ACTIVE | (H_TMASK_MASK << H_TMASK_SHIFT)));
		if (__ballot( mask != 0))
		{
			u32 lk[ 3] = {0,0,0};
			if (mask) ldLinks<SP>( L, w, P, r, lk[ 0], lk[ 1], lk[ 2]);
#if defined(SPA_PROF) && !defined(SPA_PROF_INSTALL)
			if (__ballot( lk[ 0] == 0xFFFFFFFFu)) w.err = SPD_ERR_INTERNAL;
#endif
			PROF_D( 6);
			const bool slot2 = __ballot( (mask & 4u) != 0) != 0;
			u32 c0 = 0, c1 = 0, c2 = 0, c3 = 0;
#pragma unroll
			for (int j=0; j<2; ++j) if ((mask >> j) & 1u) byteInc( c0, c1, c2, c3, lk[ j] >> 12);
			if (slot2) { if (mask & 4u) byteInc( c0, c1, c2, c3, lk[ 2] >> 12); }
			const u32 i0 = waveScanAdd( c0), i1 = waveScanAdd( c1), i2 = waveScanAdd( c2), i3 = waveScanAdd( c3);
			const u32 e0 = i0 - c0, e1 = i1 - c1, e2 = i2 - c2, e3 = i3 - c3;
			const u32 t0 = (u32)__builtin_amdgcn_readlane( i0, 63), t1 = (u32)__builtin_amdgcn_readlane( i1, 63);
			const u32 t2 = (u32)__builtin_amdgcn_readlane( i2, 63), t3 = (u32)__builtin_amdgcn_readlane( i3, 63);
			const u32 tot = LANE < 16u ? byteField( t0, t1, t2, t3, LANE) : 0u;
			const u32 qoff = waveScanAdd( tot) - tot;
			const u32 total = (u32)__builtin_amdgcn_readlane( qoff + tot, 15);
			if (slot2)
			{
				const u32 h = lk[ 2] >> 12;
				const u32 qo = (u32)__builtin_amdgcn_ds_bpermute( (int)(h << 2), (int)qoff);
				if (mask & 4u) L.rq[ qo + byteField( e0, e1, e2, e3, h)] = (u16)(4u*r + 2u);
			}
#pragma unroll
			for (int j=1; j>=0; --j)
			{
				const u32 h = lk[ j] >> 12;
				const u32 qo = (u32)__builtin_amdgcn_ds_bpermute( (int)(h << 2), (int)qoff);
				if ((mask >> j) & 1u)
				{
					u32 mineBefore = 0;
					if (slot2 && (mask & 4u) && (lk[ 2] >> 12) == h) ++mineBefore;
					if (j == 0 && (mask & 2u) && (lk[ 1] >> 12) == h) ++mineBefore;
					L.rq[ qo + byteField( e0, e1, e2, e3, h) + mineBefore] = (u16)(4u*r + (u32)j);
				}
			}
			WAVE_FENCE();
			PROF_D( 7);
			if (LANE < 16u && tot)
			{
				const u32 h = LANE, meta = w.bmetaV;
				u32 size = w.bsizeV;
				u32 tidNext = (u32)L.rq[ qoff];
				for (u32 q=0; q<tot; ++q)
				{
					const u32 tid = tidNext;
					{ const u32 nx = qoff + q + 1u; tidNext = (u32)L.rq[ nx < (u32)FAST_RQCAP ? nx : (u32)FAST_RQCAP - 1u]; }
					const u32 pos = ldLink<SP>( L, w, P, tid >> 2, tid & 3u) & 0xFFFu;
					const u32 last = size - 1u;
					const uint2 m = ldEnt<SP>( L, w, P, h, meta, last);
					if (!SP || pos != last)
					{
						stEnt<SP>( L, w, P, h, meta, pos, m.x, m.y);
						stLink<SP>( L, w, P, (m.y & 0xFFFFu) >> 2, m.y & 3u, (h << 12) | pos);
					}
					size = last;
					if (SP) WAVE_FENCE();
				}
				L.bsize[ h] = size;
				w.bsizeV = size;
			}
			WAVE_FENCE();
			PROF_D( 11);
			w.nTrig -= total;
#ifdef SPA_PROF
			w.prof[ 8] += (u32)__builtin_amdgcn_readlane( waveScanMax( tot), 63); w.prof[ 9] += 1; w.prof[ 10] += nb;
#endif
		}
		if (nE)
		{
			const bool fr = have && isExp;
			const u64 mL = __ballot( fr && r < (u32)R);
			if (fr && r < (u32)R) L.freeS[ w.freeN + (u32)__popcll( mL & lanesBelow())] = (typename FreeId<(R <= 256)>::type)r;
			w.freeN += (u32)__popcll( mL);
			if (SP)
			{
				const u64 mS = __ballot( fr && r >= (u32)R);
				if (fr && r >= (u32)R) w.sp[ P.spill.oFree + w.sFreeN + (u32)__popcll( mS & lanesBelow())] = r - R;
				w.sFreeN += (u32)__popcll( mS);
			}
		}
		WAVE_FENCE();
	}
}

static __device__ __forceinline__ void setCurrentPos( LR L, Wave& w, KP P, u32 pos)
{
	const u32 W = 1u << P.expShift;
	u32 wcnt = 0;
	while (!w.err)
	{
		u32 n = 0, row = 0;
		while (wcnt < W && w.curpos < pos && !n)
		{
			row = w.curpos & (W-1u);
			n = (u32)__builtin_amdgcn_readlane( w.expCntV, row);
			++wcnt; ++w.curpos;
		}
		u32 nD = w.nDispose;
		if (!n && !nD) break;
		if (nD && n && nD + n > 64u) { n = 0; --wcnt; --w.curpos; }
		w.nDispose = 0;
		if (w.spill) deactivateList<true>( L, w, P, nD, n, row); else deactivateList<false>( L, w, P, nD, n, row);
		if (n)
		{
			if (LANE == 0) L.expCnt[ row] = 0;
			if (LANE == row) w.expCntV = 0;
			WAVE_FENCE();
		}
	}
	if (w.curpos < pos) w.curpos = pos;
	if (w.spill)
	{
		bool over = false;
		if (LANE < 16u) over = w.bsizeV > (w.bmetaV >> 16);
		if (w.expCntV > ((u32)FAST_EXPCAP >> P.expShift)) over = true;
		if (!__ballot( over) && w.sFreeN == w.usedS) { w.spill = 0; w.sFreeN = 0; w.usedS = 0; }
	}
}

template <bool SP>
static __device__ __forceinline__ void installBatchT( LR L, Wave& w, KP P, u32 kb, u32 nb, u32 sord, u64 matMaskIn, u32 rIn,
	const uint4 q0, const uint4 q1, const uint4 q2, const Sim sim)
{
	const u32 value = sim.value, count = sim.count, end = sim.end, startLex = sim.startLex, nItems = sim.nItems, it0 = sim.it0, it1 = sim.it1, it2 = sim.it2;
	const bool hasStart = (sim.flags & S_HASSTART) != 0, done = (sim.flags & S_DONE) != 0, fin = (sim.flags & S_FIN) != 0, del = (sim.flags & S_DEL) != 0, resultNow = (sim.flags & S_RESULT) != 0;
	const bool have = LANE < nb;
	const u32 handle = q0.x, fmt = q0.y, meta = q0.w;
	const u32 tEv[ 3] = {q1.x, q1.z, q2.x};
	const u32 tInfo[ 3] = {q1.y, q1.w, q2.y};
	const u32 range = (meta >> FKI_RANGE_SHIFT) & FKI_RANGE_MASK;
	const u64 matMask = matMaskIn;
	const bool mat = (matMask >> LANE) & 1ull;
	const u32 nmat = (u32)__popcll( matMask);
	const u32 r = rIn;
	if (nmat)
	{
		const u32 row = (sord + range) & ((1u << P.expShift) - 1u);
		u64 same = matMask;
#pragma unroll
		for (int k=0; k<6; ++k)
		{
			const u64 bk = __ballot( mat && ((row >> k) & 1u));
			same &= ((row >> k) & 1u) ? bk : ~bk;
		}
		if (mat)
		{
			const u32 cnt = (u32)L.expCnt[ row];
			stExp<SP>( L, w, P, row, cnt + (u32)__popcll( same & lanesBelow()), r);
			WAVE_FENCE();
			if (!(same >> LANE >> 1)) L.expCnt[ row] = (u16)(cnt + (u32)__popcll( same));
		}
	}
	u32 c0 = 0, c1 = 0, c2 = 0, c3 = 0;
	u32 hB[ 3]; bool inst[ 3];
#pragma unroll
	for (int j=0; j<3; ++j)
	{
		hB[ j] = (tInfo[ j] >> FTI_BUCKET_SHIFT) & 15u;
		inst[ j] = mat && (tInfo[ j] & FTI_INSTALL);
		if (inst[ j]) byteInc( c0, c1, c2, c3, hB[ j]);
	}
	u32 tmask = 0;
	if (__ballot( inst[ 0] || inst[ 1] || inst[ 2]))
	{
		u32 i0 = waveScanAdd( c0), i1 = waveScanAdd( c1), i2 = waveScanAdd( c2), i3 = waveScanAdd( c3);
		const u32 e0 = i0 - c0, e1 = i1 - c1, e2 = i2 - c2, e3 = i3 - c3;
		const u32 t0 = (u32)__builtin_amdgcn_readlane( i0, 63), t1 = (u32)__builtin_amdgcn_readlane( i1, 63);
		const u32 t2 = (u32)__builtin_amdgcn_readlane( i2, 63), t3 = (u32)__builtin_amdgcn_readlane( i3, 63);
		u32 oldSize = 0, add = 0;
		if (LANE < 16u) { oldSize = L.bsize[ LANE]; add = byteField( t0, t1, t2, t3, LANE); }
#pragma unroll
		for (int j=0; j<3; ++j)
		{
			if (inst[ j])
			{
				const u32 h = hB[ j];
				u32 sameB = 0;
#pragma unroll
				for (int jj=0; jj<j; ++jj) if (inst[ jj] && hB[ jj] == h) ++sameB;
				const u32 pos = L.bsize[ h] + byteField( e0, e1, e2, e3, h) + sameB;
				const u32 sv = (tInfo[ j] & FTI_SIGVAL_MASK) | (((tInfo[ j] >> FTI_SIGTYPE_SHIFT) & FTI_SIGTYPE_MASK) << 4) | ((tInfo[ j] & FTI_HASVAR) ? 0x80u : 0u);
				stEnt<SP>( L, w, P, h, L.bmeta[ h], pos, tEv[ j], (4*r + (u32)j) | (sv << 16) | ((tInfo[ j] >> FTI_VAR_SHIFT) << 24));
				stLink<SP>( L, w, P, r, (u32)j, (h << 12) | pos);
				tmask |= 1u << j;
			}
		}
		WAVE_FENCE();
		if (LANE < 16u && add) L.bsize[ LANE] = oldSize + add;
		{
			const u32 s = t0 + t1 + t2 + t3;
			w.nTrig += (s & 0xFFu) + ((s >> 8) & 0xFFu) + ((s >> 16) & 0xFFu) + (s >> 24);
		}
	}
	if (mat)
	{
		u32 hw = value | (count << H_COUNT_SHIFT) | H_ACTIVE | H_COLD | (tmask << H_TMASK_SHIFT) | (nItems << H_NITEMS_SHIFT);
		hw |= end ? ((end & 0xFFu) << H_END_SHIFT) : (u32)H_ENDZERO;
		if (done) hw |= H_DONE;
		if (hasStart) hw |= H_HASSTART;
		if (del || fin) hw |= H_LISTED;
		stHot<SP>( L, w, P, r, hw);
		u32* cold = &w.sp[ P.spill.oCold + 8*r];
		st4( cold, handle, fmt, startLex, it0);
		*(uint2*)(cold + 4) = make_uint2( it1, it2);
	}
	{
		const bool emit = have && resultNow && handle != 0;
		const u64 rm = __ballot( emit);
		if (rm)
		{
			const u32 nr = (u32)__popcll( rm);
			if (w.nStaged + nr > P.spill.maxStaged) { FALLBACK( FB_STAGED); return; }
			if (emit)
			{
				const u32 ia = nItems == 3 ? it2 : nItems == 2 ? it1 : it0;
				const u32 ib = nItems == 3 ? it1 : it0;
				const u32 ic = it0;
				const u32 vars = nItems == 0 ? 0u : nItems == 1 ? (ia >> 24) : nItems == 2 ? ((ia >> 24) | ((ib >> 24) << 8)) : ((ia >> 24) | ((ib >> 24) << 8) | ((ic >> 24) << 16));
				stageResult( w, P, w.nStaged + (u32)__popcll( rm & lanesBelow()), handle, fmt, startLex, w.lbase, nItems, vars, ia & 0xFFFFFFu, ib & 0xFFFFFFu, ic & 0xFFFFFFu);
			}
			w.nStaged += nr;
			u32 incl = waveScanAdd( emit ? nItems : 0u);
			w.nStagedItems += (u32)__builtin_amdgcn_readlane( incl, 63);
		}
	}
	{
		const bool wantDispose = mat && (del || fin);
		const u64 dm = __ballot( wantDispose);
		if (dm)
		{
			const u32 nd = (u32)__popcll( dm);
			if (w.nDispose + nd > P.spill.maxRules) { FALLBACK( FB_DISPOSE); return; }
			if (w.nDispose + nd > (u32)FAST_LISTCAP) w.spill = 1;
			if (wantDispose)
			{
				const u32 at = w.nDispose + (u32)__popcll( dm & lanesBelow());
				if (at < (u32)FAST_LISTCAP) L.list[ at] = (u16)r; else w.sp[ P.spill.oList + at] = r;
			}
			w.nDispose += nd;
		}
	}
	WAVE_FENCE();
}

template <bool SP>
static __device__ __forceinline__ void installStaticT( LR L, Wave& w, KP P, u32 ki0, u32 nb, u32 sord, u32 r,
	const uint4 q0, const uint4 q1, const uint4 q2, const uint4 q3)
{
	const bool have = LANE < nb;
	const u32 handle = q0.x, fmt = q0.y, meta = q0.w;
	const u32 tEv[ 3] = {q1.x, q1.z, q2.x};
	const u32 tInfo[ 3] = {q1.y, q1.w, q2.y};
	const u32 hw0 = q2.z, ranksA = q2.w, ranksB = q3.x, fl = q3.w;
	const u32 totals = uni( q3.y), itemsTotal = uni( q3.z) >> 24;
	const u32 range = (meta >> FKI_RANGE_SHIFT) & FKI_RANGE_MASK;
	const u32 row = (sord + range) & ((1u << P.expShift) - 1u);
	u32 cnt = 0, oldB[ 3] = {0,0,0};
	if (have)
	{
		cnt = (u32)L.expCnt[ row];
		stExp<SP>( L, w, P, row, cnt + (ranksA & 0xFFu), r);
#pragma unroll
		for (int j=0; j<3; ++j)
		{
			if (tInfo[ j] & FTI_INSTALL)
			{
				const u32 h = (tInfo[ j] >> FTI_BUCKET_SHIFT) & 15u;
				oldB[ j] = L.bsize[ h];
				const u32 pos = oldB[ j] + ((ranksB >> (8*j)) & 0xFFu);
				const u32 sv = (tInfo[ j] & FTI_SIGVAL_MASK) | (((tInfo[ j] >> FTI_SIGTYPE_SHIFT) & FTI_SIGTYPE_MASK) << 4) | ((tInfo[ j] & FTI_HASVAR) ? 0x80u : 0u);
				stEnt<SP>( L, w, P, h, L.bmeta[ h], pos, tEv[ j], (4*r + (u32)j) | (sv << 16) | ((tInfo[ j] >> FTI_VAR_SHIFT) << 24));
				stLink<SP>( L, w, P, r, (u32)j, (h << 12) | pos);
			}
		}
	}
	WAVE_FENCE();
	const u32 nItems = P.io.withItems ? ((hw0 >> H_NITEMS_SHIFT) & H_NITEMS_MASK) : 0u;
	if (have)
	{
		const u32 close = (ranksA >> 8) & 0xFFu;
		if (close) L.expCnt[ row] = (u16)(cnt + close);
#pragma unroll
		for (int j=0; j<3; ++j)
		{
			if ((tInfo[ j] & FTI_INSTALL) && ((ranksB >> (24+j)) & 1u)) L.bsize[ (tInfo[ j] >> FTI_BUCKET_SHIFT) & 15u] = oldB[ j] + ((ranksB >> (8*j)) & 0xFFu) + 1u;
		}
		u32 hw = (hw0 & ~(H_NITEMS_MASK << H_NITEMS_SHIFT)) | (nItems << H_NITEMS_SHIFT);
		hw |= (fl & FKF_END_SET) ? (((sord + 1u) & 0xFFu) << H_END_SHIFT) : (u32)H_ENDZERO;
		stHot<SP>( L, w, P, r, hw);
		stKl<SP>( L, w, P, r, ki0 + LANE, w.lbase);
	}
	const u32 nres = (totals >> 16) & 0xFFu;
	if (nres)
	{
		if (w.nStaged + nres > P.spill.maxStaged) { FALLBACK( FB_STAGED); return; }
		if (have && (fl & FKF_RESULT_NOW))
		{
			const u32 v0 = q3.z & 0xFFu, v1 = (q3.z >> 8) & 0xFFu, v2 = (q3.z >> 16) & 0xFFu;
			const u32 va = nItems == 3 ? v2 : nItems == 2 ? v1 : v0;
			const u32 vb = nItems == 3 ? v1 : v0;
			const u32 vars = nItems == 0 ? 0u : nItems == 1 ? va : nItems == 2 ? (va | (vb << 8)) : (va | (vb << 8) | (v0 << 16));
			stageResult( w, P, w.nStaged + ((ranksA >> 16) & 0xFFu), handle, fmt, (fl & FKF_START_SET) ? w.lbase : 0u, w.lbase, nItems, vars, w.lbase, w.lbase, w.lbase);
		}
		w.nStaged += nres;
		if (P.io.withItems) w.nStagedItems += itemsTotal;
	}
	const u32 nd = totals >> 24;
	if (nd)
	{
		if (w.nDispose + nd > P.spill.maxRules) { FALLBACK( FB_DISPOSE); return; }
		if (w.nDispose + nd > (u32)FAST_LISTCAP) w.spill = 1;
		if (have && (fl & FKF_DISPOSE_NOW))
		{
			const u32 at = w.nDispose + (ranksA >> 24);
			if (at < (u32)FAST_LISTCAP) L.list[ at] = (u16)r; else w.sp[ P.spill.oList + at] = r;
		}
		w.nDispose += nd;
	}
	w.nTrig += totals & 0xFFu;
	WAVE_FENCE();
}

static __device__ __forceinline__ bool allocRuleIds( LR L, Wave& w, KP P, u64 matMask, u32& r)
{
	const bool mat = (matMask >> LANE) & 1ull;
	const u32 nmat = (u32)__popcll( matMask);
	const u32 rank = (u32)__popcll( matMask & lanesBelow());
	r = 0;
	if (nmat)
	{
		const u32 a = w.freeN < nmat ? w.freeN : nmat;
		const u32 roomL = (u32)R - w.usedL;
		const u32 b = (nmat - a) < roomL ? (nmat - a) : roomL;
		const u32 rest = nmat - a - b;
		if (rest)
		{
			const u32 c = w.sFreeN < rest ? w.sFreeN : rest;
			const u32 d = rest - c;
			if ((u32)R + w.usedS + d > P.spill.maxRules) { FALLBACK( FB_RULES); return false; }
			w.spill = 1;
			if (mat && rank >= a+b)
			{
				if (rank < a+b+c) r = (u32)R + w.sp[ P.spill.oFree + w.sFreeN - 1 - (rank - a - b)];
				else r = (u32)R + w.usedS + (rank - a - b - c);
			}
			w.sFreeN -= c; w.usedS += d;
		}
		if (mat)
		{
			if (rank < a) r = (u32)L.freeS[ w.freeN - 1 - rank];
			else if (rank < a+b) r = w.usedL + (rank - a);
		}
		w.freeN -= a; w.usedL += b;
	}
	return true;
}
static __device__ __forceinline__ bool checkBuckets( LR L, Wave& w, KP P, u32 bound, const bool inst[ 3], const u32 hB[ 3])
{
	bool over = false, fail = false;
	if (LANE < 16u)
	{
		const u32 sz = w.bsizeV, cap = w.bmetaV >> 16;
		over = sz + bound > cap;
		fail = sz + bound > cap + (u32)FAST_SPILL_BUCKET || sz + bound > 0xFFFu;
	}
	if (__ballot( over))
	{
		u32 c0 = 0, c1 = 0, c2 = 0, c3 = 0;
#pragma unroll
		for (int j=0; j<3; ++j) if (inst[ j]) byteInc( c0, c1, c2, c3, hB[ j]);
		const u32 i0 = waveScanAdd( c0), i1 = waveScanAdd( c1), i2 = waveScanAdd( c2), i3 = waveScanAdd( c3);
		const u32 t0 = (u32)__builtin_amdgcn_readlane( i0, 63), t1 = (u32)__builtin_amdgcn_readlane( i1, 63);
		const u32 t2 = (u32)__builtin_amdgcn_readlane( i2, 63), t3 = (u32)__builtin_amdgcn_readlane( i3, 63);
		over = false; fail = false;
		if (LANE < 16u)
		{
			const u32 sz = w.bsizeV + byteField( t0, t1, t2, t3, LANE), cap = w.bmetaV >> 16;
			over = sz > cap;
			fail = sz > cap + (u32)FAST_SPILL_BUCKET || sz > 0xFFFu;
		}
		if (__ballot( fail)) { FALLBACK( FB_BUCKET_SIZE); return false; }
		if (__ballot( over)) w.spill = 1;
	}
	return true;
}

template <bool SP>
static __device__ __forceinline__ void installCompactT( LR L, Wave& w, KP P, u32 ki0, u32 nb, u32 sord, u32 r,
	const uint4 c0, const uint4 c1, u32 row, u32 cnt, const u32 oldB[ 2], const u32 metaB[ 2])
{
	const bool have = LANE < nb;
	const u32 ev[ 2] = {c0.x, c0.z}, info[ 2] = {c0.y, c0.w};
	const u32 hw0 = c1.x, misc = c1.y, ranks = c1.z;
	const u32 totals = uni( c1.w), itemsTotal = (uni( c1.z) >> 16) & 0xFFu;
	if (have)
	{
		stExp<SP>( L, w, P, row, cnt + ((misc >> FSM_EXPRANK_SHIFT) & 0xFFu), r);
#pragma unroll
		for (int t=0; t<2; ++t)
		{
			if (info[ t] & FSI_PRESENT)
			{
				const u32 h = (info[ t] >> FSI_BUCKET_SHIFT) & 15u, j = info[ t] >> FSI_SLOT_SHIFT;
				const u32 pos = oldB[ t] + ((info[ t] >> FSI_RANK_SHIFT) & 0xFFu);
				stEnt<SP>( L, w, P, h, metaB[ t], pos, ev[ t], (4*r + j) | ((info[ t] & 0xFFu) << 16) | (((info[ t] >> 8) & 0xFFu) << 24));
				stLink<SP>( L, w, P, r, j, (h << 12) | pos);
			}
		}
	}
	WAVE_FENCE();
	const u32 nItems = P.io.withItems ? ((hw0 >> H_NITEMS_SHIFT) & H_NITEMS_MASK) : 0u;
	if (have)
	{
		const u32 close = (misc >> FSM_EXPCLOSE_SHIFT) & 0xFFu;
		if (close) L.expCnt[ row] = (u16)(cnt + close);
#pragma unroll
		for (int t=0; t<2; ++t) if (info[ t] & FSI_LAST) L.bsize[ (info[ t] >> FSI_BUCKET_SHIFT) & 15u] = oldB[ t] + ((info[ t] >> FSI_RANK_SHIFT) & 0xFFu) + 1u;
		u32 hw = (hw0 & ~(H_NITEMS_MASK << H_NITEMS_SHIFT)) | (nItems << H_NITEMS_SHIFT);
		hw |= (misc & FSM_END_SET) ? (((sord + 1u) & 0xFFu) << H_END_SHIFT) : (u32)H_ENDZERO;
		stHot<SP>( L, w, P, r, hw);
		stKl<SP>( L, w, P, r, ki0 + LANE, w.lbase);
	}
	const u32 nres = (totals >> 16) & 0xFFu;
	if (nres)
	{
		if (w.nStaged + nres > P.spill.maxStaged) { FALLBACK( FB_STAGED); return; }
		if (have && (misc & FSM_RESULT_NOW))
			stageLineResult( w, P, w.nStaged + (ranks & 0xFFu), ki0 + LANE, (misc & FSM_START_SET) ? w.lbase : 0u, w.lbase, nItems, 0u, 0u, w.lbase);
		w.nStaged += nres;
		if (P.io.withItems) w.nStagedItems += itemsTotal;
	}
	const u32 nd = totals >> 24;
	if (nd)
	{
		if (w.nDispose + nd > P.spill.maxRules) { FALLBACK( FB_DISPOSE); return; }
		if (w.nDispose + nd > (u32)FAST_LISTCAP) w.spill = 1;
		if (have && (misc & FSM_DISPOSE_NOW))
		{
			const u32 at = w.nDispose + ((ranks >> 8) & 0xFFu);
			if (at < (u32)FAST_LISTCAP) L.list[ at] = (u16)r; else w.sp[ P.spill.oList + at] = r;
		}
		w.nDispose += nd;
	}
	w.nTrig += totals & 0xFFu;
	w.nSignals += (totals >> 8) & 0xFFu;
	WAVE_FENCE();
}

static __device__ __forceinline__ void installBatch( LR L, Wave& w, KP P, u32 kb, u32 kc, u32 sord, const uint4 pc0, const uint4 pc1)
{
	for (u32 base=0; base<kc && !w.err; base+=64)
	{
		const u32 nb = (kc - base) < 64u ? (kc - base) : 64u;
		const bool have = LANE < nb;
		uint4 c0 = pc0, c1 = pc1;
		if (base)
		{
			c0 = make_uint4( 0,0,0,0); c1 = c0;
			if (have) { const u32* S = (const u32*)&P.statics[ kb + base + LANE]; c0 = ld4( S); c1 = ld4( S+4); }
		}
#ifdef SPA_PROF_INSTALL
		u64 pi0 = __builtin_amdgcn_s_memtime();
#define PROF_I( SLOT, V) do { if (__ballot( (V) == 0xFFFFFFF1u)) w.err = SPD_ERR_INTERNAL; const u64 pi1 = __builtin_amdgcn_s_memtime(); w.prof[ SLOT] += pi1 - pi0; pi0 = pi1; } while (0)
#else
#define PROF_I( SLOT, V) do {} while (0)
#endif
		if ((uni( c1.y) & FSM_BATCH_COMPACT) && sord != 0)
		{
			PROF_I( 6, c1.y);
			const u32 info[ 2] = {c0.y, c0.w};
			const u32 row = (sord + (c1.y & FSM_RANGE_MASK)) & ((1u << P.expShift) - 1u);
			u32 cnt = 0, oldB[ 2] = {0,0}, metaB[ 2] = {0,0};
			bool inst[ 3] = {false,false,false}; u32 hB[ 3] = {0,0,0};
			if (have)
			{
				cnt = (u32)L.expCnt[ row];
#pragma unroll
				for (int t=0; t<2; ++t)
				{
					if (info[ t] & FSI_PRESENT) { hB[ t] = (info[ t] >> FSI_BUCKET_SHIFT) & 15u; inst[ t] = true; oldB[ t] = L.bsize[ hB[ t]]; metaB[ t] = L.bmeta[ hB[ t]]; }
				}
			}
			w.nInstalled += nb;
			u32 r;
			if (!allocRuleIds( L, w, P, __ballot( have), r)) return;
			if (!w.spill)
			{
				if (__ballot( have && cnt + nb > ((u32)FAST_EXPCAP >> P.expShift))) w.spill = 1;
			}
			if (!checkBuckets( L, w, P, uni( c1.w) & 0xFFu, inst, hB)) return;
			PROF_I( 7, cnt + oldB[ 0] + oldB[ 1] + r);
			if (w.spill) installCompactT<true>( L, w, P, kb + base, nb, sord, r, c0, c1, row, cnt, oldB, metaB);
			else installCompactT<false>( L, w, P, kb + base, nb, sord, r, c0, c1, row, cnt, oldB, metaB);
			PROF_I( 11, 0u);
			w.bsizeV = L.bsize[ LANE & 15u];
			continue;
		}
		uint4 q0 = make_uint4( 0,0,0,0), q1 = q0, q2 = q0, q3 = q0;
		if (have)
		{
			const FastKeyInst* K = &P.keyinst[ kb + base + LANE];
			q0 = ld4( K); q1 = ld4( (const u32*)K + 4); q2 = ld4( (const u32*)K + 8); q3 = ld4( (const u32*)K + 12);
		}
		const bool isStatic = (uni( q3.w) & FKF_BATCH_STATIC) != 0 && sord != 0;
		const u32 pastEvent = q0.z, meta = q0.w;
		const u32 tEv[ 3] = {q1.x, q1.z, q2.x};
		const u32 tInfo[ 3] = {q1.y, q1.w, q2.y};
		const u32 range = (meta >> FKI_RANGE_SHIFT) & FKI_RANGE_MASK;
		Sim sim;
		sim.value = meta & FKI_VALUE_MASK; sim.count = (meta >> FKI_COUNT_SHIFT) & FKI_COUNT_MASK; sim.end = 0;
		sim.startLex = 0; sim.nItems = 0; sim.it0 = 0; sim.it1 = 0; sim.it2 = 0; sim.nFires = 0; sim.flags = 0;
		bool dropped = false;
		if (!isStatic && __ballot( have && pastEvent != 0))
		{
			const u32 psi = (have && pastEvent) ? ((meta >> FKI_PASTSTOP_SHIFT) & FKI_PASTSTOP_MASK) : 0u;
			const u32 plex = (u32)__builtin_amdgcn_ds_bpermute( (int)((psi-1u) << 2), (int)w.stopLex);
			const u32 psord = (u32)__builtin_amdgcn_ds_bpermute( (int)((psi-1u) << 2), (int)w.stopOrd);
			const u32 pts = (u32)__builtin_amdgcn_ds_bpermute( (int)((psi-1u) << 2), (int)w.stopTs);
			u32 delTs[ 3];
#pragma unroll
			for (int j=0; j<3; ++j)
			{
				const u32 esi = (tInfo[ j] >> FTI_DELSTOP_SHIFT) & FTI_DELSTOP_MASK;
				delTs[ j] = (u32)__builtin_amdgcn_ds_bpermute( (int)((esi-1u) << 2), (int)w.stopTs);
				if (!esi) delTs[ j] = 0;
			}
			if (psi)
			{
				if (pts && psord + range >= w.curpos)
				{
#pragma unroll
					for (int j=2; j>=0; --j)
					{
						if ((tInfo[ j] & FTI_INSTALL) && tEv[ j] == pastEvent) fireLocal( sim, tInfo[ j], psord, plex, P.io.withItems);
					}
					bool cancelled = false;
#pragma unroll
					for (int j=0; j<3; ++j)
					{
						if ((tInfo[ j] & FTI_INSTALL) && ((tInfo[ j] >> FTI_SIGTYPE_SHIFT) & FTI_SIGTYPE_MASK) == SIG_DEL)
						{
							const u32 ts = delTs[ j];
							if (ts && ts > pts) cancelled = true;
						}
					}
					if (cancelled || (sim.flags & (S_DEL | S_FIN))) dropped = true;
				}
			}
			w.nAlt += (u32)__popcll( __ballot( have && pastEvent != 0));
		}
		if (!isStatic)
		{
			if (have && !dropped)
			{
#pragma unroll
				for (int j=0; j<3; ++j) if (tInfo[ j] & FTI_KEY) fireLocal( sim, tInfo[ j], sord, w.lbase, P.io.withItems);
			}
			if (__ballot( (sim.flags & S_ODD) != 0)) { FALLBACK( FB_ITEMS); return; }
		}
		const bool mat = have && !dropped;
		const u64 matMask = __ballot( mat);
		const u32 nmat = (u32)__popcll( matMask);
		w.nInstalled += nb;
		if (isStatic) w.nSignals += (uni( q3.y) >> 8) & 0xFFu;
		else
		{
			u32 incl = waveScanAdd( have ? sim.nFires : 0u);
			w.nSignals += (u32)__builtin_amdgcn_readlane( incl, 63);
		}
		u32 r;
		if (!allocRuleIds( L, w, P, matMask, r)) return;
		if (nmat && !w.spill)
		{
			const u32 row = (sord + range) & ((1u << P.expShift) - 1u);
			const bool over = mat && (u32)L.expCnt[ row] + nmat > ((u32)FAST_EXPCAP >> P.expShift);
			if (__ballot( over)) w.spill = 1;
		}
		{
			bool inst[ 3]; u32 hB[ 3];
#pragma unroll
			for (int j=0; j<3; ++j) { inst[ j] = mat && (tInfo[ j] & FTI_INSTALL); hB[ j] = (tInfo[ j] >> FTI_BUCKET_SHIFT) & 15u; }
			if (!checkBuckets( L, w, P, isStatic ? (uni( q3.y) & 0xFFu) : 3*nmat, inst, hB)) return;
		}
		if (isStatic)
		{
			if (w.spill) installStaticT<true>( L, w, P, kb + base, nb, sord, r, q0, q1, q2, q3);
			else installStaticT<false>( L, w, P, kb + base, nb, sord, r, q0, q1, q2, q3);
		}
		else if (w.spill) installBatchT<true>( L, w, P, kb, nb, sord, matMask, r, q0, q1, q2, sim);
		else installBatchT<false>( L, w, P, kb, nb, sord, matMask, r, q0, q1, q2, sim);
		w.bsizeV = L.bsize[ LANE & 15u];
	}
	w.bsizeV = L.bsize[ LANE & 15u];
	w.expCntV = (u32)L.expCnt[ LANE];
}

template <bool SP>
static __device__ __forceinline__ void scanAndFire( LR L, Wave& w, KP P, u32 id, u32 ordpos)
{
	const u32 h = evhash( id) & 15u;
	const u32 n = (u32)__builtin_amdgcn_readlane( w.bsizeV, h);
	const u32 meta = (u32)__builtin_amdgcn_readlane( w.bmetaV, h);
	for (u32 base=0; base<n && !w.err; base+=64)
	{
		const u32 i = base + LANE;
		uint2 en = make_uint2( 0, 0);
		if (i < n) en = ldEnt<SP>( L, w, P, h, meta, i);
		u64 m = __ballot( i < n && en.x == id);
		if (!SP && (m & (m - 1ull)) != 0)
		{
			if (fireBatch( L, w, P, m, en.y, ordpos)) m = 0;
		}
		while (m && !w.err)
		{
			const u32 p = (u32)__builtin_ctzll( m);
			m &= m-1;
			const u32 tsv = (u32)__builtin_amdgcn_readlane( en.y, p);
			fireSignal<SP>( L, w, P, tsv, ordpos);
		}
	}
}

static __device__ __forceinline__ void runKernel()
{
	KP P = kernelParams();
	__shared__ Lds ldsDoc;
	LR L = *(__attribute__((address_space(3))) Lds*)&ldsDoc;
	Wave w;
	w.sp = P.spillBase + (u64)blockIdx.x * P.spill.totalWords;
	const u32 ndocs = P.io.ndocs;
	const u32 waveSlot = blockIdx.x, nWaveSlots = gridDim.x;

	for (u32 round=0; round<=ndocs; ++round)
	{
		u32 doc = waveSlot;
		if (round)
		{
			u32 nx = 0;
			if (LANE == 0) nx = atomicAdd( P.io.docCursor, 1u);
			doc = nWaveSlots + uni( nx);
		}
		if (doc >= ndocs) break;
		w.bmetaV = P.bucketMeta[ LANE & 15u]; w.bsizeV = 0; w.expCntV = 0;
		if (LANE < 16u) { L.bsize[ LANE] = 0; L.bmeta[ LANE] = w.bmetaV; }
		L.expCnt[ LANE] = 0;
		w.stopLex = 0; w.stopOrd = 0; w.stopTs = 0; w.posLexems = 0;
		w.curpos = 0; w.timestamp = 0; w.nInstalled = 0; w.nAlt = 0; w.nSignals = 0; w.nTrig = 0; w.openLo = 0; w.openHi = 0;
		w.freeN = 0; w.usedL = 0; w.sFreeN = 0; w.usedS = 0;
		w.nDispose = 0; w.nStaged = 0; w.nStagedItems = 0; w.err = 0; w.lbase = 0; w.why = 0; w.spill = 0;
#ifdef SPA_PROF
		for (int pi=0; pi<12; ++pi) w.prof[ pi] = 0;
#endif
		WAVE_FENCE();

		u64 lbeg, lend;
		docLexems( P.io, doc, lbeg, lend);
		if (lend - lbeg >= (1ull << 24)) FALLBACK( FB_LEXEMS);
		u32 curPosition = 0, nEvents = 0;
		for (u64 tile=lbeg; tile<lend && !w.err; tile+=64)
		{
			PROF_DECL;
			uint4 lx = make_uint4( 0,0,0,0); u32 seg = 0;
			const bool mine = tile + LANE < lend;
			if (mine)
			{
				lx = ((const uint4*)P.io.lexems)[ tile + LANE];
				if (P.io.origseg) seg = P.io.origseg[ tile + LANE];
			}
			u32 kBegin = 0, kCount = 0, kStop = 0;
			if (mine && lx.x && lx.x < (1u<<29))
			{
				u32 slot = keyHash( lx.x) & P.keymask;
				for (u32 probes=0; probes<=P.keymask; ++probes)
				{
					const uint4 eq = ld4( &P.keytab[ slot]);
					if (eq.x == lx.x) { kBegin = eq.y; kCount = eq.z; kStop = eq.w; break; }
					if (eq.x == 0) break;
					slot = (slot+1) & P.keymask;
				}
			}
			const u32 cnt = (lend - tile) < 64 ? (u32)(lend - tile) : 64u;
#ifdef SPA_PROF
			if (__ballot( kBegin == 0xFFFFFFFFu)) break;
#endif
			PROF_ADD( 5);
			for (u32 k=0; k<cnt && !w.err; ++k)
			{
				const u32 id = __builtin_amdgcn_readlane( lx.x, k), ordpos = __builtin_amdgcn_readlane( lx.y, k);
				const u32 origpos = __builtin_amdgcn_readlane( lx.z, k), origsize = __builtin_amdgcn_readlane( lx.w, k);
				const u32 origseg = __builtin_amdgcn_readlane( seg, k);
				if (curPosition > ordpos) { w.err = SPD_ERR_ORDER; break; }
				else if (curPosition < ordpos) { curPosition = ordpos; w.posLexems = 0; }
				else if (origsize >= 0x7FFFFFFFu || origseg >= 0x7FFFFFFFu || origpos >= 0x7FFFFFFFu) { w.err = SPD_ERR_RANGE; break; }
				if (w.curpos != ordpos || w.nDispose) { setCurrentPos( L, w, P, ordpos); PROF_ADD( 3); if (w.err) break; }
				if (id >= (1u<<29)) { w.err = SPD_ERR_RANGE; break; }
				w.lbase = (u32)(tile - lbeg) + k;
				if (++w.posLexems > 60u) { FALLBACK( FB_POSLEXEMS); break; }
				{
					const u32 lo = w.openLo + w.nTrig;
					if (lo < w.openLo) w.openHi += 1;
					w.openLo = lo;
				}
				const u32 kb = __builtin_amdgcn_readlane( kBegin, k), kc = __builtin_amdgcn_readlane( kCount, k);
				const u32 stopIdx = __builtin_amdgcn_readlane( kStop, k);
				uint4 pc0 = make_uint4( 0,0,0,0), pc1 = pc0;
				if (LANE < kc) { const u32* S = (const u32*)&P.statics[ kb + LANE]; pc0 = ld4( S); pc1 = ld4( S+4); }
				if (id)
				{
					if (w.spill) scanAndFire<true>( L, w, P, id, ordpos); else scanAndFire<false>( L, w, P, id, ordpos);
				}
				PROF_ADD( 0);
				if (w.err) break;
				if (kc) installBatch( L, w, P, kb, kc, ordpos, pc0, pc1);
				PROF_ADD( 1);
				if (w.err) break;
				WAVE_FENCE();
				if (stopIdx)
				{
					if (LANE == stopIdx-1u) { w.stopLex = w.lbase; w.stopOrd = ordpos; w.stopTs = w.timestamp + 1u; }
					w.timestamp += 1;
					WAVE_FENCE();
				}
				PROF_ADD( 2);
				++nEvents;
			}
		}

		PROF_DECL;
		u32 nres = w.err ? 0 : w.nStaged;
		const u32 nitems = (w.err || !P.io.withItems) ? 0 : w.nStagedItems;
		u64 resBase = 0, itemBase = 0;
		if (nres && !reserveOutput( P.io, SPC_RESULTS, nres, resBase)) { w.err = SPD_ERR_OUTPUT; nres = 0; }
		if (nres && nitems && !reserveOutput( P.io, SPC_ITEMS, nitems, itemBase)) { w.err = SPD_ERR_OUTPUT; nres = 0; }
		if (nres)
		{
			WAVE_FENCE();
			u64 ip = itemBase;
			for (u32 base=0; base<nres; base+=64)
			{
				const u32 ri = base + LANE;
				const bool hv = ri < nres;
				uint4 s0 = make_uint4( 0,0,0,0), s1 = s0;
				if (hv) { const u32* S = &w.sp[ P.spill.oStaged + 8*ri]; s0 = ld4( S); s1 = ld4( S+4); }
				if (hv && (s0.x & (u32)STAGED_LINE))
				{
					const u32* K = (const u32*)&P.keyinst[ s0.x & 0xFFFFFu];
					const u32 handle = K[ 0], fmt = K[ 1], vw = K[ 14];
					const u32 nStatic = s1.x & 3u, hasNew = (s1.x >> 2) & 1u, newVar = (s1.x >> 8) & 0xFFu, lx = s1.y, endLex = s0.w;
					u32 vv[ 3] = {0,0,0}, ll[ 3] = {0,0,0};
					u32 n = 0;
					if (hasNew) { vv[ 0] = newVar; ll[ 0] = endLex; n = 1; }
#pragma unroll
					for (int k=2; k>=0; --k)
					{
						if ((u32)k < nStatic)
						{
							const u32 v = (vw >> (8*k)) & 0xFFu;
							if (n == 0) { vv[ 0] = v; ll[ 0] = lx; } else if (n == 1) { vv[ 1] = v; ll[ 1] = lx; } else if (n == 2) { vv[ 2] = v; ll[ 2] = lx; }
							++n;
						}
					}
					s0.x = handle; s0.y = fmt;
					s1.x = n | (vv[ 0] << 8) | (vv[ 1] << 16) | (vv[ 2] << 24); s1.y = ll[ 0]; s1.z = ll[ 1]; s1.w = ll[ 2];
				}
				const u32 ni = P.io.withItems ? (s1.x & 0xFFu) : 0u;
				u32 incl = waveScanAdd( ni);
				const u64 mine = ip + (incl - ni);
				if (hv)
				{
					const uint4 a = ((const uint4*)P.io.lexems)[ lbeg + s0.z], z = ((const uint4*)P.io.lexems)[ lbeg + s0.w];
					const u32 sa = P.io.origseg ? P.io.origseg[ lbeg + s0.z] : 0u, sz = P.io.origseg ? P.io.origseg[ lbeg + s0.w] : 0u;
					u32* o = P.io.results + (resBase + ri)*9;
					o[0] = s0.x; o[1] = a.y; o[2] = z.y + 1u; o[3] = sa; o[4] = a.z; o[5] = sz; o[6] = z.z + z.w;
					o[7] = P.io.withItems ? (u32)mine : 0u; o[8] = ni;
					if (P.io.withFormats) P.io.resultFormat[ resBase + ri] = s0.y;
					const u32 il[ 3] = {s1.y, s1.z, s1.w};
#pragma unroll
					for (int q=0; q<3; ++q)
					{
						if ((u32)q < ni)
						{
							const uint4 t = ((const uint4*)P.io.lexems)[ lbeg + il[ q]];
							const u32 st = P.io.origseg ? P.io.origseg[ lbeg + il[ q]] : 0u;
							u32* io = P.io.items + (mine + (u32)q)*7;
							io[0] = (s1.x >> (8 + 8*q)) & 0xFFu; io[1] = t.y; io[2] = t.y + 1u; io[3] = st; io[4] = t.z; io[5] = st; io[6] = t.z + t.w;
							if (P.io.withFormats) { P.io.itemFormat[ 2*(mine + (u32)q)] = 0; P.io.itemFormat[ 2*(mine + (u32)q)+1] = 0; }
						}
					}
				}
				ip += (u32)__builtin_amdgcn_readlane( incl, 63);
			}
		}
		PROF_ADD( 4);
#ifdef SPA_PROF
		if (LANE == 0 && P.prof) for (int pi=0; pi<12; ++pi) atomicAdd( (unsigned long long*)&P.prof[ pi], (unsigned long long)w.prof[ pi]);
#endif
		if (w.err != SPD_FAST_FALLBACK) finishDocument( P.io, doc, resBase, nres, w.nInstalled, w.nAlt, w.nSignals, ((u64)w.openHi << 32) | w.openLo, w.err, nEvents);
		else if (LANE == 0)
		{
			const u32 at = atomicAdd( P.fallbackCount, 1u);
			P.fallbackList[ at] = doc;
			P.io.docRange[ 2*(u64)doc] = 0; P.io.docRange[ 2*(u64)doc+1] = 0;
			P.io.docStatus[ doc] = (int32_t)SPD_FAST_FALLBACK;
			atomicAdd( (unsigned long long*)&P.io.counters[ SPC_HANDOVER], 1ull);
			if (P.diag) { atomicAdd( &P.diag[ 0], 1u); atomicAdd( &P.diag[ w.why & 15u], 1u); }
		}
	}
}
};

}

#ifndef SPA_L2_FAST_WAVES_PER_EU
#define SPA_L2_FAST_WAVES_PER_EU 4
#endif
#define SPA_L2_FAST_OCC __attribute__((amdgpu_waves_per_eu( SPA_L2_FAST_WAVES_PER_EU, SPA_L2_FAST_WAVES_PER_EU)))
#define SPA_FAST_VARIANTS( V) \
	V( s, 192, 312) \
	V( m, 320, 512) \
	V( l, 512, 1024) \
	V( t, 8, 128)		 \
	V( n, 256, 448)
#define SPA_FAST_INSTANCE( X, RR, TT) \
	extern "C" __global__ __launch_bounds__(64) SPA_L2_FAST_OCC void spa_l2_fast_kernel_##X( FastParams kernelArgs) { Engine<RR,TT>::runKernel(); }
SPA_FAST_VARIANTS( SPA_FAST_INSTANCE)

namespace spa {
struct FastVariant { void (*kernel)( FastParams); uint32_t R, T; const char* name; };
#define SPA_FAST_ENTRY( X, RR, TT) {spa_l2_fast_kernel_##X, RR, TT, "spa_l2_fast_kernel_" #X},
static const FastVariant fastVariants[ FAST_VARIANTS] = { SPA_FAST_VARIANTS( SPA_FAST_ENTRY) };
static const FastVariant& fastVariantOf( unsigned variant) { return fastVariants[ variant < FAST_VARIANTS ? variant : FAST_VARIANTS-1]; }

unsigned fastVariantNamed( const char* size)
{
	for (unsigned v=0; v<FAST_VARIANTS; ++v) if (size[ 0] == fastVariants[ v].name[ sizeof("spa_l2_fast_kernel_")-1]) return v;
	return FAST_VARIANTS-1;
}
const char* fastKernelName( unsigned variant) { return fastVariantOf( variant).name; }
void fastCapacities( unsigned variant, uint32_t& R, uint32_t& T) { R = fastVariantOf( variant).R; T = fastVariantOf( variant).T; }
int fastBlocksPerCU( unsigned variant)
{
	int n = 0;
	if (hipOccupancyMaxActiveBlocksPerMultiprocessor( &n, (const void*)fastVariantOf( variant).kernel, 64, 0) != hipSuccess || n < 1) n = 1;
	if (n > 32) n = 32;
	return n;
}
hipError_t launchL2Fast( const FastParams& P, unsigned variant, unsigned nblocks, hipStream_t stream)
{
	hipLaunchKernelGGL( fastVariantOf( variant).kernel, dim3( nblocks), dim3( 64), 0, stream, P);
	return hipGetLastError();
}
}
```

struspattern_amd/csrc/l2_fast_tables.cpp:

```cpp
#include "l2_fast.h"
#include "l2_compile.hpp"
#include <map>
#include <set>
#include <cstring>

namespace spa {

static_assert( sizeof(FastKeyInst) == 64, "one install record per 64-byte line");
static_assert( sizeof(FastStatic) == 32, "compact static line");
static_assert( sizeof(FastKeyEntry) == sizeof(DevKeyEntry), "the fast kernel reads the general key table in place");

std::string buildFastTables( const FlatTables& ft, std::vector<FastKeyInst>& out, std::vector<FastStatic>* statics)
{
	out.clear();
	if (statics) statics->clear();
	if (ft.nofStopWords > FAST_MAXSTOP) return "more than 64 stop words";
	if (ft.keylist.size() >= (1u<<20)) return "more than 2^20 key list entries";
	std::set<uint32_t> listened;
	std::map<uint32_t,uint32_t> stopIdxOf;
	for (size_t i=0; i<ft.trigdefs.size(); ++i) listened.insert( ft.trigdefs[ i].event);
	for (size_t i=0; i<ft.keytab.size(); ++i)
	{
		const DevKeyEntry& e = ft.keytab[ i];
		if (!e.event) continue;
// ... 125 lines not shown
				B[ l].totals = trigTotal | (firesTotal << 8) | (resTotal << 16) | (dispTotal << 24);
				B[ l].items |= itemsTotal << 24;
			}
			if (!statics) continue;
			bool compact = true;
			for (uint32_t l=0; l<nb && compact; ++l)
			{
				int n = 0;
				for (int j=0; j<3; ++j) if (B[ l].trig[ j].info & FTI_INSTALL) ++n;
				if (n > 2) compact = false;
			}
			if (!compact) continue;
			FastStatic* C = &(*statics)[ e.listBegin + b0];
			for (uint32_t l=0; l<nb; ++l)
			{
				const FastKeyInst& ki = B[ l];
				FastStatic& fs = C[ l];
				int n = 0;
				for (int j=0; j<3; ++j)
				{
					const uint32_t info = ki.trig[ j].info;
					if (!(info & FTI_INSTALL)) continue;
					const uint32_t sv = (info & FTI_SIGVAL_MASK) | (((info >> FTI_SIGTYPE_SHIFT) & FTI_SIGTYPE_MASK) << 4) | ((info & FTI_HASVAR) ? 0x80u : 0u);
					const uint32_t ci = sv | ((info >> FTI_VAR_SHIFT) << 8) | (((info >> FTI_BUCKET_SHIFT) & 15u) << FSI_BUCKET_SHIFT)
						| (((ki.ranksB >> (8*j)) & 0xFFu) << FSI_RANK_SHIFT) | (((ki.ranksB >> (24+j)) & 1u) ? (uint32_t)FSI_LAST : 0u) | (uint32_t)FSI_PRESENT | ((uint32_t)j << FSI_SLOT_SHIFT);
					if (n == 0) { fs.ev0 = ki.trig[ j].event; fs.info0 = ci; } else { fs.ev1 = ki.trig[ j].event; fs.info1 = ci; }
					++n;
				}
				fs.hw0 = ki.hw0;
				fs.misc = ((ki.meta >> FKI_RANGE_SHIFT) & FKI_RANGE_MASK) | ((ki.ranksA & 0xFFu) << FSM_EXPRANK_SHIFT) | (((ki.ranksA >> 8) & 0xFFu) << FSM_EXPCLOSE_SHIFT)
					| ((ki.flags & FKF_END_SET) ? (uint32_t)FSM_END_SET : 0u) | ((ki.flags & FKF_START_SET) ? (uint32_t)FSM_START_SET : 0u)
					| ((ki.flags & FKF_RESULT_NOW) ? (uint32_t)FSM_RESULT_NOW : 0u) | ((ki.flags & FKF_DISPOSE_NOW) ? (uint32_t)FSM_DISPOSE_NOW : 0u) | (uint32_t)FSM_BATCH_COMPACT;
				fs.ranks = ((ki.ranksA >> 16) & 0xFFu) | (((ki.ranksA >> 24) & 0xFFu) << 8) | (itemsTotal << 16);
				fs.totals = ki.totals;
			}
		}
	}
	return std::string();
}

void layoutFast( FastSpillLayout& S, uint32_t bucketMeta[16], uint32_t& expShift, const std::vector<FastKeyInst>& keyinst, uint32_t R, uint32_t T, uint32_t maxRules, uint32_t maxStaged)
{
	uint32_t maxRange = 0;
	for (size_t i=0; i<keyinst.size(); ++i) { const uint32_t rg = (keyinst[ i].meta >> FKI_RANGE_SHIFT) & FKI_RANGE_MASK; if (rg > maxRange) maxRange = rg; }
	expShift = 0;
	while ((1u << expShift) < maxRange + 1u) ++expShift;
	if (maxRules < R) maxRules = R;
	uint64_t weight[ 16], total = 0;
	for (int b=0; b<16; ++b) weight[ b] = 1;
	for (size_t i=0; i<keyinst.size(); ++i)
	{
		for (int j=0; j<3; ++j)
		{
			const uint32_t info = keyinst[ i].trig[ j].info;
			if (info & FTI_INSTALL) weight[ (info >> FTI_BUCKET_SHIFT) & 15u] += 1;
		}
	}
	for (int b=0; b<16; ++b) total += weight[ b];
	const uint32_t floorCap = 8;
	uint32_t base = 0;
	for (int b=0; b<16; ++b)
	{
		uint32_t cap = floorCap + (uint32_t)((uint64_t)(T - 16*floorCap) * weight[ b] / total);
		if (cap > 0xFFFu) cap = 0xFFFu;
		bucketMeta[ b] = base | (cap << 16);
		base += cap;
	}
	uint32_t w = 0;
	auto takeW = [&]( uint32_t words) { uint32_t at = w; w += (words + 3u) & ~3u; return at; };
	const uint32_t spillRules = maxRules - R;
	S.maxRules = maxRules;
	S.oCold = takeW( 8*maxRules);
	S.oHot = takeW( spillRules); S.oLink = takeW( 3*spillRules);
	S.oKi = takeW( spillRules); S.oLex0 = takeW( spillRules);
	S.oFree = takeW( spillRules);
	S.oEnt = takeW( 2*16*FAST_SPILL_BUCKET);
	S.maxStaged = maxStaged;
	S.oStaged = takeW( 8*maxStaged);
	S.oList = takeW( maxRules > FAST_LISTCAP ? maxRules : FAST_LISTCAP);
	S.oExp = takeW( (1u << expShift) * maxRules);
	S.totalWords = (w + 63u) & ~63u;
}

}
```

Before: 4.247 GB/s.

## Add specialised fast-tier kernel instances selected from compiled automaton facts

Adds a Spec template parameter to the fast matching engine so that trigger count, compact batches, items/formats/origseg flags and the expansion shift become compile-time constants. Three specialised kernel instances are added (two-trigger compact, compact) and a host-side selector picks one from facts computed over the compiled key tables and the launch flags. The goal is to drop runtime branches, the third link slot and parameter loads from the hot matching loop, and possibly reduce register pressure. In exchange it adds more kernel instances (longer compile, larger binary) and selection logic that must match the table layout exactly.

Measured after the change: 4.276 GB/s, median of 6. Within noise of the previous version (+0.7%).

```diff
diff --git a/include/strus_pattern_amd.h b/include/strus_pattern_amd.h
--- a/include/strus_pattern_amd.h
+++ b/include/strus_pattern_amd.h
@@ -100,6 +100,8 @@
 const char* sp_matcher_variable_name(const sp_matcher_t* m, uint32_t variable);
 size_t sp_matcher_dump_table(const sp_matcher_t* m, uint32_t** out);
 int sp_matcher_fast_tier(const sp_matcher_t* m, char* why, size_t whysize);
+int sp_matcher_fast_facts(const sp_matcher_t* m, uint32_t facts[9]);
+const char* sp_l2_fast_select_instance(const char* size, uint32_t max_triggers, uint32_t static_batches, uint32_t exp_shift, int with_items, int with_formats, int has_origseg, int generic);
 int sp_matcher_result_set_tier(const sp_matcher_t* m, char* why, size_t whysize, uint32_t* alt_programs);
 
 int sp_matcher_serialize(const sp_matcher_t* m, void** blob, size_t* size);
diff --git a/struspattern_amd/__init__.py b/struspattern_amd/__init__.py
--- a/struspattern_amd/__init__.py
+++ b/struspattern_amd/__init__.py
@@ -218,6 +218,12 @@
         return self._L.sp_matcher_ctx_kernel_name(self._h).decode()
 
 
+def fastInstanceFor(max_triggers, exp_shift, static_batches=0, with_items=True, with_formats=False, has_origseg=False, size=None, generic=False):
+    from . import capi
+    return capi.lib().sp_l2_fast_select_instance(size.encode() if size else None, max_triggers, static_batches, exp_shift, int(with_items),
+                                                 int(with_formats), int(has_origseg), int(generic)).decode()
+
+
 def _serialize(L, fn, handle, err):
     blob = ctypes.c_void_p()
     size = ctypes.c_size_t()
@@ -315,6 +321,15 @@
         ok = self._L.sp_matcher_fast_tier(self._h, buf, 256)
         return bool(ok), buf.value.decode()
 
+    FAST_FACTS = ("lines", "max_triggers", "max_range", "exp_shift", "batches", "compact_batches", "static_batches",
+                  "dynamic_batches", "alt_key_lines")
+
+    def fastFacts(self):
+        v = (ctypes.c_uint32 * 9)()
+        if not self._L.sp_matcher_fast_facts(self._h, v):
+            return None
+        return dict(zip(self.FAST_FACTS, (int(x) for x in v)))
+
     def resultSetTier(self):
         buf = ctypes.create_string_buffer(256)
         alt = ctypes.c_uint32(0)
diff --git a/struspattern_amd/capi.py b/struspattern_amd/capi.py
--- a/struspattern_amd/capi.py
+++ b/struspattern_amd/capi.py
@@ -83,6 +83,8 @@
     "sp_matcher_variable_name": (c_cp, [c_vp, c_u32]),
     "sp_matcher_dump_table": (ctypes.c_size_t, [c_vp, P(P(c_u32))]),
     "sp_matcher_fast_tier": (ctypes.c_int, [c_vp, ctypes.c_char_p, ctypes.c_size_t]),
+    "sp_matcher_fast_facts": (ctypes.c_int, [c_vp, ctypes.POINTER(ctypes.c_uint32)]),
+    "sp_l2_fast_select_instance": (ctypes.c_char_p, [ctypes.c_char_p, ctypes.c_uint32, ctypes.c_uint32, ctypes.c_uint32, ctypes.c_int, ctypes.c_int, ctypes.c_int, ctypes.c_int]),
     "sp_matcher_result_set_tier": (ctypes.c_int, [c_vp, ctypes.c_char_p, ctypes.c_size_t, P(c_u32)]),
     "sp_matcher_serialize": (ctypes.c_int, [c_vp, P(c_vp), P(ctypes.c_size_t)]),
     "sp_matcher_deserialize": (c_vp, [c_vp, ctypes.c_size_t, ctypes.c_char_p, ctypes.c_size_t]),
diff --git a/struspattern_amd/csrc/capi_l2.cpp b/struspattern_amd/csrc/capi_l2.cpp
--- a/struspattern_amd/csrc/capi_l2.cpp
+++ b/struspattern_amd/csrc/capi_l2.cpp
@@ -16,8 +16,8 @@
 
 namespace spa {
 hipError_t launchL2Match( const L2Params& P, unsigned nblocks, hipStream_t stream);
-hipError_t launchL2Fast( const FastParams& P, unsigned variant, unsigned nblocks, hipStream_t stream);
-int fastBlocksPerCU( unsigned variant);
+hipError_t launchL2Fast( const FastParams& P, unsigned instance, unsigned nblocks, hipStream_t stream);
+int fastBlocksPerCU( unsigned instance);
 void fastCapacities( unsigned variant, uint32_t& R, uint32_t& T);
 unsigned fastVariantNamed( const char* size);
 const char* fastKernelName( unsigned variant);
@@ -98,6 +98,8 @@
 	std::vector<FastKeyInst> fastKeyinst;
 	FastSpillLayout fastSpill; uint32_t fastBucketMeta[ 16]; uint32_t fastExpShift;
 	unsigned fastWaves, fastBlocksPerCU, fastVariant;
+	FastFacts fastFacts; bool fastGeneric;
+	unsigned fastInstance;
 	uint32_t fastMaxRules, fastMaxStaged;
 	ArenaLayout arena;
 	DeviceBuffer dArena; unsigned arenaWaves;
@@ -121,11 +123,12 @@
 	hipStream_t finishStream;
 	hipEvent_t evFinish[ 4]; bool evFinishValid;
 
-	sp_matcher_ctx() :inst(0),device(0),keymask(0),nofStopWords(0),fast(false),join(false),joinAltRules(false),joinKeymask(0),joinMaxRange(0),joinDelimiter(0),fastWaves(0),fastBlocksPerCU(0),fastVariant(4),fastMaxRules(2048),fastMaxStaged(32768),arenaWaves(0),withFormats(false),resultCapacity(0),itemCapacity(0),minResultCapacity(0),minItemCapacity(0)
+	sp_matcher_ctx() :inst(0),device(0),keymask(0),nofStopWords(0),fast(false),join(false),joinAltRules(false),joinKeymask(0),joinMaxRange(0),joinDelimiter(0),fastWaves(0),fastBlocksPerCU(0),fastVariant(4),fastGeneric(false),fastInstance(4),fastMaxRules(2048),fastMaxStaged(32768),arenaWaves(0),withFormats(false),resultCapacity(0),itemCapacity(0),minResultCapacity(0),minItemCapacity(0)
 		,lastNdocs(0),evStart(0),evStop(0),evValid(false),lastStream(0),own(0),withItems(true),numCUs(256),curHasSeg(false),haveBatch(false),finished(false),finishStream(0),evFinishValid(false)
 	{
 		std::memset( evFinish, 0, sizeof(evFinish));
 		std::memset( &arena, 0, sizeof(arena));
+		std::memset( &fastFacts, 0, sizeof(fastFacts));
 		std::memset( &fastSpill, 0, sizeof(fastSpill)); std::memset( fastBucketMeta, 0, sizeof(fastBucketMeta));
 		std::memset( &lastStats, 0, sizeof(lastStats));
 		arena.maxRules = 1024; arena.maxTrigs = 1024; arena.bucketCap = 256; arena.maxItems = 2048;
@@ -194,7 +197,7 @@
 {
 	if (c->join) return "spa_l2_join_kernel";
 	if (!c->fast) return "spa_l2_match_kernel";
-	return fastKernelName( c->fastVariant);
+	return fastKernelName( c->fastInstance);
 }
 
 int sp_matcher_fast_tier( const sp_matcher_t* m, char* why, size_t whysize)
@@ -213,6 +216,30 @@
 		if (why && whysize) { std::strncpy( why, e.what(), whysize-1); why[ whysize-1] = 0; }
 		return 0;
 	}
+}
+
+int sp_matcher_fast_facts( const sp_matcher_t* m, uint32_t facts[9])
+{
+	try
+	{
+		FlatTables ft;
+		m->compiler.flatten( ft);
+		std::vector<FastKeyInst> ki; std::vector<FastStatic> ks;
+		if (!buildFastTables( ft, ki, &ks).empty()) return 0;
+		FastFacts f;
+		fastFactsOf( ft, ki, &ks, f);
+		const uint32_t v[ 9] = {f.lines, f.maxTriggers, f.maxRange, f.expShift, f.batches, f.compactBatches, f.staticBatches, f.dynamicBatches, f.altKeyLines};
+		std::memcpy( facts, v, sizeof(v));
+		return 1;
+	}
+	catch (const std::exception&) { return 0; }
+}
+const char* sp_l2_fast_select_instance( const char* size, uint32_t max_triggers, uint32_t static_batches, uint32_t exp_shift, int with_items, int with_formats, int has_origseg, int generic)
+{
+	FastFacts f; std::memset( &f, 0, sizeof(f));
+	f.maxTriggers = max_triggers; f.staticBatches = static_batches; f.expShift = exp_shift;
+	FastLaunchFacts lf = {with_items ? 1u : 0u, with_formats ? 1u : 0u, has_origseg ? 1u : 0u};
+	return fastKernelName( fastSelectInstance( fastVariantNamed( size && size[ 0] ? size : "n"), max_triggers ? &f : 0, &lf, generic != 0));
 }
 
 static std::string buildResultSetTables( const sp_matcher* m, const FlatTables& ft, std::vector<JoinKey>& keytab, std::vector<JoinRule>& rules,
@@ -338,6 +365,10 @@
 				if (const char* e = getenv( "SPA_L2_FAST_MAXRULES")) c->fastMaxRules = (uint32_t)atoi( e);
 				if (const char* e = getenv( "SPA_L2_FAST_MAXSTAGED")) c->fastMaxStaged = (uint32_t)atoi( e);
 				if (c->fastMaxRules > 4095) c->fastMaxRules = 4095;
+				fastFactsOf( ft, c->fastKeyinst, &ks, c->fastFacts);
+				if (const char* e = getenv( "SPA_L2_FAST_GENERIC")) c->fastGeneric = e[ 0] == '1';
+				const FastLaunchFacts lf = {c->withItems ? 1u : 0u, c->withFormats ? 1u : 0u, 0u};
+				c->fastInstance = fastSelectInstance( c->fastVariant, &c->fastFacts, &lf, c->fastGeneric);
 			}
 			if (getenv( "SPA_L2_VERBOSE")) fprintf( stderr, "[spa] fast tier: %s\n", c->fast ? "on" : c->whyNotFast.c_str());
 		}
@@ -698,7 +729,11 @@
 		uint32_t fR = 0, fT = 0;
 		fastCapacities( c->fastVariant, fR, fT);
 		layoutFast( c->fastSpill, c->fastBucketMeta, c->fastExpShift, c->fastKeyinst, fR, fT, c->fastMaxRules, c->fastMaxStaged);
-		if (!c->fastBlocksPerCU) c->fastBlocksPerCU = (unsigned)fastBlocksPerCU( c->fastVariant);
+		const FastLaunchFacts lf = {P.io.withItems, P.io.withFormats, P.io.origseg ? 1u : 0u};
+		c->fastFacts.expShift = c->fastExpShift;
+		const unsigned instance = fastSelectInstance( c->fastVariant, &c->fastFacts, &lf, c->fastGeneric);
+		if (instance != c->fastInstance) { c->fastInstance = instance; c->fastBlocksPerCU = 0; }
+		if (!c->fastBlocksPerCU) c->fastBlocksPerCU = (unsigned)fastBlocksPerCU( c->fastInstance);
 		size_t fslots = (size_t)c->numCUs * c->fastBlocksPerCU;
 		unsigned fblocks = (unsigned)(ndocs < fslots ? ndocs : fslots);
 		if (fblocks == 0) fblocks = 1;
@@ -720,7 +755,7 @@
 		F.spill = c->fastSpill; F.spillBase = (uint32_t*)c->dSpill.ptr;
 		F.fallbackList = (uint32_t*)c->dFallbackList.ptr; F.fallbackCount = (uint32_t*)c->dCursor.ptr + 2;
 		F.diag = (uint32_t*)c->dCursor.ptr + 16; F.prof = (uint64_t*)((uint32_t*)c->dCursor.ptr + 32);
-		HIP_CHECK( launchL2Fast( F, c->fastVariant, fblocks, stream));
+		HIP_CHECK( launchL2Fast( F, c->fastInstance, fblocks, stream));
 		P.docList = F.fallbackList; P.docListCount = F.fallbackCount;
 		P.io.docCursor = (uint32_t*)c->dCursor.ptr + 1;
 		const unsigned listBlocks = nblocks < 2*c->numCUs ? nblocks : 2*c->numCUs;
diff --git a/struspattern_amd/csrc/l2_fast.h b/struspattern_amd/csrc/l2_fast.h
--- a/struspattern_amd/csrc/l2_fast.h
+++ b/struspattern_amd/csrc/l2_fast.h
@@ -1,6 +1,7 @@
 #ifndef SPA_L2_FAST_H
 #define SPA_L2_FAST_H
 #include <stdint.h>
+#include <vector>
 #include "l2_tables.h"
 #include "l2_device.h"
 
@@ -157,5 +158,37 @@
 	uint64_t* prof;
 };
 
+#define SPA_FAST_VARIANTS( V) \
+	V( s, 192, 312) \
+	V( m, 320, 512) \
+	V( l, 512, 1024) \
+	V( t, 8, 128)		 \
+	V( n, 256, 448)
+#define SPA_FAST_SPECIALISED( V) \
+	V( n_t2, 256, 448, 1, 1, 1, 0, 0, 4) \
+	V( n_c, 256, 448, 0, 1, 1, 0, 0, 4) \
+	V( t_c, 8, 128, 0, 1, 1, 0, 0, 4)
+enum {FAST_SPECIALISED=3, FAST_INSTANCES=FAST_VARIANTS+FAST_SPECIALISED};
+
+struct FastFacts
+{
+	uint32_t lines;
+	uint32_t maxTriggers;
+	uint32_t maxRange;
+	uint32_t expShift;
+	uint32_t batches;
+	uint32_t compactBatches;
+	uint32_t staticBatches;
+	uint32_t dynamicBatches;
+	uint32_t altKeyLines;
+};
+struct FastLaunchFacts { uint32_t withItems, withFormats, hasOrigseg; };
+struct FastInstanceDesc { const char* name; uint32_t R, T; int two, compact, items, formats, origseg, expShift; };
+
+struct FlatTables;
+void fastFactsOf( const FlatTables& ft, const std::vector<FastKeyInst>& keyinst, const std::vector<FastStatic>* statics, FastFacts& facts);
+unsigned fastSelectInstance( unsigned variant, const FastFacts* facts, const FastLaunchFacts* launch, bool generic);
+const FastInstanceDesc& fastInstanceDesc( unsigned instance);
+
 }
 #endif
diff --git a/struspattern_amd/csrc/l2_fast_kernel.hip b/struspattern_amd/csrc/l2_fast_kernel.hip
--- a/struspattern_amd/csrc/l2_fast_kernel.hip
+++ b/struspattern_amd/csrc/l2_fast_kernel.hip
@@ -111,11 +111,21 @@
 #endif
 };
 
-template <int R, int T>
+template <int TWO_, int COMPACT_, int ITEMS_, int FORMATS_, int ORIGSEG_, int EXPSHIFT_>
+struct Spec { enum {SPECIAL=(TWO_ || COMPACT_ || ITEMS_ >= 0 || FORMATS_ >= 0 || ORIGSEG_ >= 0 || EXPSHIFT_ >= 0), TWO=TWO_, COMPACT=(COMPACT_ || TWO_), ITEMS=ITEMS_, FORMATS=FORMATS_, ORIGSEG=ORIGSEG_, EXPSHIFT=EXPSHIFT_}; };
+typedef Spec<0,0,-1,-1,-1,-1> SpecGeneral;
+
+template <int R, int T, class SPEC>
 struct Engine
 {
 typedef LdsDoc<R,T> Lds;
 typedef __attribute__((address_space(3))) Lds& LR;
+enum {NT = SPEC::TWO ? 2 : 3};
+static __device__ __forceinline__ u32 expShiftOf( KP P) { return SPEC::EXPSHIFT >= 0 ? (u32)SPEC::EXPSHIFT : P.expShift; }
+static __device__ __forceinline__ u32 withItemsOf( KP P) { return SPEC::ITEMS >= 0 ? (u32)SPEC::ITEMS : P.io.withItems; }
+static __device__ __forceinline__ u32 withFormatsOf( KP P) { return SPEC::FORMATS >= 0 ? (u32)SPEC::FORMATS : P.io.withFormats; }
+static __device__ __forceinline__ const u32* origsegOf( KP P) { return SPEC::ORIGSEG == 0 ? (const u32*)0 : P.io.origseg; }
+static __device__ __forceinline__ bool hasOrigseg( KP P) { return SPEC::ORIGSEG >= 0 ? SPEC::ORIGSEG != 0 : P.io.origseg != 0; }
 
 template <bool SP> static __device__ __forceinline__ u32 ldHot( LR L, const Wave& w, KP P, u32 r) { if (!SP || r < (u32)R) return L.hot[ r]; return w.sp[ P.spill.oHot + (r - R)]; }
 template <bool SP> static __device__ __forceinline__ void stHot( LR L, const Wave& w, KP P, u32 r, u32 v) { if (!SP || r < (u32)R) L.hot[ r] = v; else w.sp[ P.spill.oHot + (r - R)] = v; }
@@ -123,17 +133,17 @@
 template <bool SP> static __device__ __forceinline__ void stLink( LR L, const Wave& w, KP P, u32 r, u32 j, u32 v) { if (!SP || r < (u32)R) L.link[ 3*r + j] = (u16)v; else w.sp[ P.spill.oLink + 3*(r - R) + j] = v; }
 template <bool SP> static __device__ __forceinline__ void ldLinks( LR L, const Wave& w, KP P, u32 r, u32& l0, u32& l1, u32& l2)
 {
-	if (!SP || r < (u32)R) { l0 = (u32)L.link[ 3*r]; l1 = (u32)L.link[ 3*r+1]; l2 = (u32)L.link[ 3*r+2]; }
-	else { const u32* q = &w.sp[ P.spill.oLink + 3*(r - R)]; l0 = q[0]; l1 = q[1]; l2 = q[2]; }
+	if (!SP || r < (u32)R) { l0 = (u32)L.link[ 3*r]; l1 = (u32)L.link[ 3*r+1]; l2 = SPEC::TWO ? 0u : (u32)L.link[ 3*r+2]; }
+	else { const u32* q = &w.sp[ P.spill.oLink + 3*(r - R)]; l0 = q[0]; l1 = q[1]; l2 = SPEC::TWO ? 0u : q[2]; }
 }
 template <bool SP> static __device__ __forceinline__ u32 ldKl( LR L, const Wave& w, KP P, u32 r) { if (!SP || r < (u32)R) return L.kl[ r]; return w.sp[ P.spill.oKi + (r - R)]; }
 template <bool SP> static __device__ __forceinline__ void stKl( LR L, const Wave& w, KP P, u32 r, u32 ki, u32 lx)
 { const u32 v = ki | (lx << 20); if (!SP || r < (u32)R) L.kl[ r] = v; else w.sp[ P.spill.oKi + (r - R)] = v; }
 static __device__ __forceinline__ u32 keyLexemOf( u32 kl, u32 lbase) { return lbase - ((lbase - (kl >> 20)) & 0xFFFu); }
 template <bool SP> static __device__ __forceinline__ u32 ldExp( LR L, const Wave& w, KP P, u32 row, u32 i)
-{ const u32 C = (u32)FAST_EXPCAP >> P.expShift; if (!SP || i < C) return (u32)L.exp[ row*C + i]; return w.sp[ P.spill.oExp + row*P.spill.maxRules + (i - C)]; }
+{ const u32 C = (u32)FAST_EXPCAP >> expShiftOf( P); if (!SP || i < C) return (u32)L.exp[ row*C + i]; return w.sp[ P.spill.oExp + row*P.spill.maxRules + (i - C)]; }
 template <bool SP> static __device__ __forceinline__ void stExp( LR L, const Wave& w, KP P, u32 row, u32 i, u32 r)
-{ const u32 C = (u32)FAST_EXPCAP >> P.expShift; if (!SP || i < C) L.exp[ row*C + i] = (u16)r; else w.sp[ P.spill.oExp + row*P.spill.maxRules + (i - C)] = r; }
+{ const u32 C = (u32)FAST_EXPCAP >> expShiftOf( P); if (!SP || i < C) L.exp[ row*C + i] = (u16)r; else w.sp[ P.spill.oExp + row*P.spill.maxRules + (i - C)] = r; }
 template <bool SP> static __device__ __forceinline__ u32 ldEv( LR L, const Wave& w, KP P, u32 h, u32 meta, u32 pos)
 { if (!SP || pos < (meta >> 16)) return (u32)L.ent[ (meta & 0xFFFFu) + pos]; return w.sp[ P.spill.oEnt + 2*(h*FAST_SPILL_BUCKET + pos - (meta >> 16))]; }
 template <bool SP> static __device__ __forceinline__ uint2 ldEnt( LR L, const Wave& w, KP P, u32 h, u32 meta, u32 pos)
@@ -211,7 +221,7 @@
 	bool newItem = false, newStart = false;
 	if (take)
 	{
-		if (hasVar && P.io.withItems)
+		if (hasVar && withItemsOf( P))
 		{
 			if (done)
 			{
@@ -342,7 +352,7 @@
 	u32 why = 0;
 	if (take)
 	{
-		if (hasVar && P.io.withItems)
+		if (hasVar && withItemsOf( P))
 		{
 			if (done) { if (nItems) why = FB_ITEM_AFTER_RESULT; }
 			else if (nItems < 3u) newItem = true;
@@ -459,7 +469,7 @@
 			hw = ldHot<SP>( L, w, P, r);
 		}
 		const bool act = have && (hw & H_ACTIVE) && !(isExp && (hw & H_LISTED));
-		const u32 mask = act ? ((hw >> H_TMASK_SHIFT) & H_TMASK_MASK) : 0u;
+		const u32 mask = act ? ((hw >> H_TMASK_SHIFT) & (SPEC::TWO ? 3u : (u32)H_TMASK_MASK)) : 0u;
 		if (act) stHot<SP>( L, w, P, r, hw & ~(H_ACTIVE | (H_TMASK_MASK << H_TMASK_SHIFT)));
 		if (__ballot( mask != 0))
 		{
@@ -469,7 +479,7 @@
 			if (__ballot( lk[ 0] == 0xFFFFFFFFu)) w.err = SPD_ERR_INTERNAL;
 #endif
 			PROF_D( 6);
-			const bool slot2 = __ballot( (mask & 4u) != 0) != 0;
+			const bool slot2 = !SPEC::TWO && __ballot( (mask & 4u) != 0) != 0;
 			u32 c0 = 0, c1 = 0, c2 = 0, c3 = 0;
 #pragma unroll
 			for (int j=0; j<2; ++j) if ((mask >> j) & 1u) byteInc( c0, c1, c2, c3, lk[ j] >> 12);
@@ -549,9 +559,12 @@
 	}
 }
 
+enum {BODY_LDS=0, BODY_SPILL=1, BODY_SWITCH=2};
+#define SPILL_PATH( BODY) ((BODY) == BODY_SPILL || ((BODY) == BODY_SWITCH && w.spill) || ((BODY) == BODY_LDS && __builtin_expect( w.spill != 0, 0)))
+template <int BODY>
 static __device__ __forceinline__ void setCurrentPos( LR L, Wave& w, KP P, u32 pos)
 {
-	const u32 W = 1u << P.expShift;
+	const u32 W = 1u << expShiftOf( P);
 	u32 wcnt = 0;
 	while (!w.err)
 	{
@@ -566,7 +579,7 @@
 		if (!n && !nD) break;
 		if (nD && n && nD + n > 64u) { n = 0; --wcnt; --w.curpos; }
 		w.nDispose = 0;
-		if (w.spill) deactivateList<true>( L, w, P, nD, n, row); else deactivateList<false>( L, w, P, nD, n, row);
+		if (BODY == BODY_SPILL || (BODY == BODY_SWITCH && w.spill)) deactivateList<true>( L, w, P, nD, n, row); else deactivateList<false>( L, w, P, nD, n, row);
 		if (n)
 		{
 			if (LANE == 0) L.expCnt[ row] = 0;
@@ -575,11 +588,11 @@
 		}
 	}
 	if (w.curpos < pos) w.curpos = pos;
-	if (w.spill)
+	if (BODY != BODY_LDS && w.spill)
 	{
 		bool over = false;
 		if (LANE < 16u) over = w.bsizeV > (w.bmetaV >> 16);
-		if (w.expCntV > ((u32)FAST_EXPCAP >> P.expShift)) over = true;
+		if (w.expCntV > ((u32)FAST_EXPCAP >> expShiftOf( P))) over = true;
 		if (!__ballot( over) && w.sFreeN == w.usedS) { w.spill = 0; w.sFreeN = 0; w.usedS = 0; }
 	}
 }
@@ -601,7 +614,7 @@
 	const u32 r = rIn;
 	if (nmat)
 	{
-		const u32 row = (sord + range) & ((1u << P.expShift) - 1u);
+		const u32 row = (sord + range) & ((1u << expShiftOf( P)) - 1u);
 		u64 same = matMask;
 #pragma unroll
 		for (int k=0; k<6; ++k)
@@ -618,9 +631,9 @@
 		}
 	}
 	u32 c0 = 0, c1 = 0, c2 = 0, c3 = 0;
-	u32 hB[ 3]; bool inst[ 3];
-#pragma unroll
-	for (int j=0; j<3; ++j)
+	u32 hB[ 3] = {0,0,0}; bool inst[ 3] = {false,false,false};
+#pragma unroll
+	for (int j=0; j<NT; ++j)
 	{
 		hB[ j] = (tInfo[ j] >> FTI_BUCKET_SHIFT) & 15u;
 		inst[ j] = mat && (tInfo[ j] & FTI_INSTALL);
@@ -636,7 +649,7 @@
 		u32 oldSize = 0, add = 0;
 		if (LANE < 16u) { oldSize = L.bsize[ LANE]; add = byteField( t0, t1, t2, t3, LANE); }
 #pragma unroll
-		for (int j=0; j<3; ++j)
+		for (int j=0; j<NT; ++j)
 		{
 			if (inst[ j])
 			{
@@ -720,7 +733,7 @@
 	const u32 hw0 = q2.z, ranksA = q2.w, ranksB = q3.x, fl = q3.w;
 	const u32 totals = uni( q3.y), itemsTotal = uni( q3.z) >> 24;
 	const u32 range = (meta >> FKI_RANGE_SHIFT) & FKI_RANGE_MASK;
-	const u32 row = (sord + range) & ((1u << P.expShift) - 1u);
+	const u32 row = (sord + range) & ((1u << expShiftOf( P)) - 1u);
 	u32 cnt = 0, oldB[ 3] = {0,0,0};
 	if (have)
 	{
@@ -741,7 +754,7 @@
 		}
 	}
 	WAVE_FENCE();
-	const u32 nItems = P.io.withItems ? ((hw0 >> H_NITEMS_SHIFT) & H_NITEMS_MASK) : 0u;
+	const u32 nItems = withItemsOf( P) ? ((hw0 >> H_NITEMS_SHIFT) & H_NITEMS_MASK) : 0u;
 	if (have)
 	{
 		const u32 close = (ranksA >> 8) & 0xFFu;
@@ -769,7 +782,7 @@
 			stageResult( w, P, w.nStaged + ((ranksA >> 16) & 0xFFu), handle, fmt, (fl & FKF_START_SET) ? w.lbase : 0u, w.lbase, nItems, vars, w.lbase, w.lbase, w.lbase);
 		}
 		w.nStaged += nres;
-		if (P.io.withItems) w.nStagedItems += itemsTotal;
+		if (withItemsOf( P)) w.nStagedItems += itemsTotal;
 	}
 	const u32 nd = totals >> 24;
 	if (nd)
@@ -834,7 +847,7 @@
 	{
 		u32 c0 = 0, c1 = 0, c2 = 0, c3 = 0;
 #pragma unroll
-		for (int j=0; j<3; ++j) if (inst[ j]) byteInc( c0, c1, c2, c3, hB[ j]);
+		for (int j=0; j<NT; ++j) if (inst[ j]) byteInc( c0, c1, c2, c3, hB[ j]);
 		const u32 i0 = waveScanAdd( c0), i1 = waveScanAdd( c1), i2 = waveScanAdd( c2), i3 = waveScanAdd( c3);
 		const u32 t0 = (u32)__builtin_amdgcn_readlane( i0, 63), t1 = (u32)__builtin_amdgcn_readlane( i1, 63);
 		const u32 t2 = (u32)__builtin_amdgcn_readlane( i2, 63), t3 = (u32)__builtin_amdgcn_readlane( i3, 63);
@@ -875,7 +888,7 @@
 		}
 	}
 	WAVE_FENCE();
-	const u32 nItems = P.io.withItems ? ((hw0 >> H_NITEMS_SHIFT) & H_NITEMS_MASK) : 0u;
+	const u32 nItems = withItemsOf( P) ? ((hw0 >> H_NITEMS_SHIFT) & H_NITEMS_MASK) : 0u;
 	if (have)
 	{
 		const u32 close = (misc >> FSM_EXPCLOSE_SHIFT) & 0xFFu;
@@ -894,7 +907,7 @@
 		if (have && (misc & FSM_RESULT_NOW))
 			stageLineResult( w, P, w.nStaged + (ranks & 0xFFu), ki0 + LANE, (misc & FSM_START_SET) ? w.lbase : 0u, w.lbase, nItems, 0u, 0u, w.lbase);
 		w.nStaged += nres;
-		if (P.io.withItems) w.nStagedItems += itemsTotal;
+		if (withItemsOf( P)) w.nStagedItems += itemsTotal;
 	}
 	const u32 nd = totals >> 24;
 	if (nd)
@@ -913,6 +926,7 @@
 	WAVE_FENCE();
 }
 
+template <int BODY>
 static __device__ __forceinline__ void installBatch( LR L, Wave& w, KP P, u32 kb, u32 kc, u32 sord, const uint4 pc0, const uint4 pc1)
 {
 	for (u32 base=0; base<kc && !w.err; base+=64)
@@ -935,7 +949,7 @@
 		{
 			PROF_I( 6, c1.y);
 			const u32 info[ 2] = {c0.y, c0.w};
-			const u32 row = (sord + (c1.y & FSM_RANGE_MASK)) & ((1u << P.expShift) - 1u);
+			const u32 row = (sord + (c1.y & FSM_RANGE_MASK)) & ((1u << expShiftOf( P)) - 1u);
 			u32 cnt = 0, oldB[ 2] = {0,0}, metaB[ 2] = {0,0};
 			bool inst[ 3] = {false,false,false}; u32 hB[ 3] = {0,0,0};
 			if (have)
@@ -952,11 +966,11 @@
 			if (!allocRuleIds( L, w, P, __ballot( have), r)) return;
 			if (!w.spill)
 			{
-				if (__ballot( have && cnt + nb > ((u32)FAST_EXPCAP >> P.expShift))) w.spill = 1;
+				if (__ballot( have && cnt + nb > ((u32)FAST_EXPCAP >> expShiftOf( P)))) w.spill = 1;
 			}
 			if (!checkBuckets( L, w, P, uni( c1.w) & 0xFFu, inst, hB)) return;
 			PROF_I( 7, cnt + oldB[ 0] + oldB[ 1] + r);
-			if (w.spill) installCompactT<true>( L, w, P, kb + base, nb, sord, r, c0, c1, row, cnt, oldB, metaB);
+			if (SPILL_PATH( BODY)) installCompactT<true>( L, w, P, kb + base, nb, sord, r, c0, c1, row, cnt, oldB, metaB);
 			else installCompactT<false>( L, w, P, kb + base, nb, sord, r, c0, c1, row, cnt, oldB, metaB);
 			PROF_I( 11, 0u);
 			w.bsizeV = L.bsize[ LANE & 15u];
@@ -966,9 +980,11 @@
 		if (have)
 		{
 			const FastKeyInst* K = &P.keyinst[ kb + base + LANE];
-			q0 = ld4( K); q1 = ld4( (const u32*)K + 4); q2 = ld4( (const u32*)K + 8); q3 = ld4( (const u32*)K + 12);
-		}
-		const bool isStatic = (uni( q3.w) & FKF_BATCH_STATIC) != 0 && sord != 0;
+			q0 = ld4( K); q1 = ld4( (const u32*)K + 4);
+			if (!SPEC::TWO) q2 = ld4( (const u32*)K + 8);
+			if (!SPEC::COMPACT) q3 = ld4( (const u32*)K + 12);
+		}
+		const bool isStatic = !SPEC::COMPACT && (uni( q3.w) & FKF_BATCH_STATIC) != 0 && sord != 0;
 		const u32 pastEvent = q0.z, meta = q0.w;
 		const u32 tEv[ 3] = {q1.x, q1.z, q2.x};
 		const u32 tInfo[ 3] = {q1.y, q1.w, q2.y};
@@ -985,7 +1001,7 @@
 			const u32 pts = (u32)__builtin_amdgcn_ds_bpermute( (int)((psi-1u) << 2), (int)w.stopTs);
 			u32 delTs[ 3];
 #pragma unroll
-			for (int j=0; j<3; ++j)
+			for (int j=0; j<NT; ++j)
 			{
 				const u32 esi = (tInfo[ j] >> FTI_DELSTOP_SHIFT) & FTI_DELSTOP_MASK;
 				delTs[ j] = (u32)__builtin_amdgcn_ds_bpermute( (int)((esi-1u) << 2), (int)w.stopTs);
@@ -996,13 +1012,13 @@
 				if (pts && psord + range >= w.curpos)
 				{
 #pragma unroll
-					for (int j=2; j>=0; --j)
+					for (int j=NT-1; j>=0; --j)
 					{
-						if ((tInfo[ j] & FTI_INSTALL) && tEv[ j] == pastEvent) fireLocal( sim, tInfo[ j], psord, plex, P.io.withItems);
+						if ((tInfo[ j] & FTI_INSTALL) && tEv[ j] == pastEvent) fireLocal( sim, tInfo[ j], psord, plex, withItemsOf( P));
 					}
 					bool cancelled = false;
 #pragma unroll
-					for (int j=0; j<3; ++j)
+					for (int j=0; j<NT; ++j)
 					{
 						if ((tInfo[ j] & FTI_INSTALL) && ((tInfo[ j] >> FTI_SIGTYPE_SHIFT) & FTI_SIGTYPE_MASK) == SIG_DEL)
 						{
@@ -1020,7 +1036,7 @@
 			if (have && !dropped)
 			{
 #pragma unroll
-				for (int j=0; j<3; ++j) if (tInfo[ j] & FTI_KEY) fireLocal( sim, tInfo[ j], sord, w.lbase, P.io.withItems);
+				for (int j=0; j<NT; ++j) if (tInfo[ j] & FTI_KEY) fireLocal( sim, tInfo[ j], sord, w.lbase, withItemsOf( P));
 			}
 			if (__ballot( (sim.flags & S_ODD) != 0)) { FALLBACK( FB_ITEMS); return; }
 		}
@@ -1038,22 +1054,22 @@
 		if (!allocRuleIds( L, w, P, matMask, r)) return;
 		if (nmat && !w.spill)
 		{
-			const u32 row = (sord + range) & ((1u << P.expShift) - 1u);
-			const bool over = mat && (u32)L.expCnt[ row] + nmat > ((u32)FAST_EXPCAP >> P.expShift);
+			const u32 row = (sord + range) & ((1u << expShiftOf( P)) - 1u);
+			const bool over = mat && (u32)L.expCnt[ row] + nmat > ((u32)FAST_EXPCAP >> expShiftOf( P));
 			if (__ballot( over)) w.spill = 1;
 		}
 		{
-			bool inst[ 3]; u32 hB[ 3];
-#pragma unroll
-			for (int j=0; j<3; ++j) { inst[ j] = mat && (tInfo[ j] & FTI_INSTALL); hB[ j] = (tInfo[ j] >> FTI_BUCKET_SHIFT) & 15u; }
+			bool inst[ 3] = {false,false,false}; u32 hB[ 3] = {0,0,0};
+#pragma unroll
+			for (int j=0; j<NT; ++j) { inst[ j] = mat && (tInfo[ j] & FTI_INSTALL); hB[ j] = (tInfo[ j] >> FTI_BUCKET_SHIFT) & 15u; }
 			if (!checkBuckets( L, w, P, isStatic ? (uni( q3.y) & 0xFFu) : 3*nmat, inst, hB)) return;
 		}
 		if (isStatic)
 		{
-			if (w.spill) installStaticT<true>( L, w, P, kb + base, nb, sord, r, q0, q1, q2, q3);
+			if (SPILL_PATH( BODY)) installStaticT<true>( L, w, P, kb + base, nb, sord, r, q0, q1, q2, q3);
 			else installStaticT<false>( L, w, P, kb + base, nb, sord, r, q0, q1, q2, q3);
 		}
-		else if (w.spill) installBatchT<true>( L, w, P, kb, nb, sord, matMask, r, q0, q1, q2, sim);
+		else if (SPILL_PATH( BODY)) installBatchT<true>( L, w, P, kb, nb, sord, matMask, r, q0, q1, q2, sim);
 		else installBatchT<false>( L, w, P, kb, nb, sord, matMask, r, q0, q1, q2, sim);
 		w.bsizeV = L.bsize[ LANE & 15u];
 	}
@@ -1085,6 +1101,50 @@
 			fireSignal<SP>( L, w, P, tsv, ordpos);
 		}
 	}
+}
+
+template <int BODY>
+static __device__ __forceinline__ bool oneEvent( LR L, Wave& w, KP P, const uint4 lx, const u32 seg, const u32 kBegin, const u32 kCount, const u32 kStop,
+	const u32 k, const u32 lbase, u32& curPosition)
+{
+	PROF_DECL;
+	const u32 id = __builtin_amdgcn_readlane( lx.x, k), ordpos = __builtin_amdgcn_readlane( lx.y, k);
+	const u32 origpos = __builtin_amdgcn_readlane( lx.z, k), origsize = __builtin_amdgcn_readlane( lx.w, k);
+	const u32 origseg = SPEC::ORIGSEG == 0 ? 0u : __builtin_amdgcn_readlane( seg, k);
+	if (curPosition > ordpos) { w.err = SPD_ERR_ORDER; return false; }
+	else if (curPosition < ordpos) { curPosition = ordpos; w.posLexems = 0; }
+	else if (origsize >= 0x7FFFFFFFu || origseg >= 0x7FFFFFFFu || origpos >= 0x7FFFFFFFu) { w.err = SPD_ERR_RANGE; return false; }
+	if (w.curpos != ordpos || w.nDispose) { setCurrentPos<BODY>( L, w, P, ordpos); PROF_ADD( 3); if (w.err) return false; }
+	if (id >= (1u<<29)) { w.err = SPD_ERR_RANGE; return false; }
+	w.lbase = lbase;
+	if (++w.posLexems > 60u) { FALLBACK( FB_POSLEXEMS); return false; }
+	{
+		const u32 lo = w.openLo + w.nTrig;
+		if (lo < w.openLo) w.openHi += 1;
+		w.openLo = lo;
+	}
+	const u32 kb = __builtin_amdgcn_readlane( kBegin, k), kc = __builtin_amdgcn_readlane( kCount, k);
+	const u32 stopIdx = __builtin_amdgcn_readlane( kStop, k);
+	uint4 pc0 = make_uint4( 0,0,0,0), pc1 = pc0;
+	if (LANE < kc) { const u32* S = (const u32*)&P.statics[ kb + LANE]; pc0 = ld4( S); pc1 = ld4( S+4); }
+	if (id)
+	{
+		if (BODY == BODY_SPILL || (BODY == BODY_SWITCH && w.spill)) scanAndFire<true>( L, w, P, id, ordpos); else scanAndFire<false>( L, w, P, id, ordpos);
+	}
+	PROF_ADD( 0);
+	if (w.err) return false;
+	if (kc) installBatch<BODY>( L, w, P, kb, kc, ordpos, pc0, pc1);
+	PROF_ADD( 1);
+	if (w.err) return false;
+	WAVE_FENCE();
+	if (stopIdx)
+	{
+		if (LANE == stopIdx-1u) { w.stopLex = w.lbase; w.stopOrd = ordpos; w.stopTs = w.timestamp + 1u; }
+		w.timestamp += 1;
+		WAVE_FENCE();
+	}
+	PROF_ADD( 2);
+	return true;
 }
 
 static __device__ __forceinline__ void runKernel()
@@ -1131,7 +1191,7 @@
 			if (mine)
 			{
 				lx = ((const uint4*)P.io.lexems)[ tile + LANE];
-				if (P.io.origseg) seg = P.io.origseg[ tile + LANE];
+				if (hasOrigseg( P)) seg = origsegOf( P)[ tile + LANE];
 			}
 			u32 kBegin = 0, kCount = 0, kStop = 0;
 			if (mine && lx.x && lx.x < (1u<<29))
@@ -1152,49 +1212,19 @@
 			PROF_ADD( 5);
 			for (u32 k=0; k<cnt && !w.err; ++k)
 			{
-				const u32 id = __builtin_amdgcn_readlane( lx.x, k), ordpos = __builtin_amdgcn_readlane( lx.y, k);
-				const u32 origpos = __builtin_amdgcn_readlane( lx.z, k), origsize = __builtin_amdgcn_readlane( lx.w, k);
-				const u32 origseg = __builtin_amdgcn_readlane( seg, k);
-				if (curPosition > ordpos) { w.err = SPD_ERR_ORDER; break; }
-				else if (curPosition < ordpos) { curPosition = ordpos; w.posLexems = 0; }
-				else if (origsize >= 0x7FFFFFFFu || origseg >= 0x7FFFFFFFu || origpos >= 0x7FFFFFFFu) { w.err = SPD_ERR_RANGE; break; }
-				if (w.curpos != ordpos || w.nDispose) { setCurrentPos( L, w, P, ordpos); PROF_ADD( 3); if (w.err) break; }
-				if (id >= (1u<<29)) { w.err = SPD_ERR_RANGE; break; }
-				w.lbase = (u32)(tile - lbeg) + k;
-				if (++w.posLexems > 60u) { FALLBACK( FB_POSLEXEMS); break; }
-				{
-					const u32 lo = w.openLo + w.nTrig;
-					if (lo < w.openLo) w.openHi += 1;
-					w.openLo = lo;
-				}
-				const u32 kb = __builtin_amdgcn_readlane( kBegin, k), kc = __builtin_amdgcn_readlane( kCount, k);
-				const u32 stopIdx = __builtin_amdgcn_readlane( kStop, k);
-				uint4 pc0 = make_uint4( 0,0,0,0), pc1 = pc0;
-				if (LANE < kc) { const u32* S = (const u32*)&P.statics[ kb + LANE]; pc0 = ld4( S); pc1 = ld4( S+4); }
-				if (id)
-				{
-					if (w.spill) scanAndFire<true>( L, w, P, id, ordpos); else scanAndFire<false>( L, w, P, id, ordpos);
-				}
-				PROF_ADD( 0);
-				if (w.err) break;
-				if (kc) installBatch( L, w, P, kb, kc, ordpos, pc0, pc1);
-				PROF_ADD( 1);
-				if (w.err) break;
-				WAVE_FENCE();
-				if (stopIdx)
-				{
-					if (LANE == stopIdx-1u) { w.stopLex = w.lbase; w.stopOrd = ordpos; w.stopTs = w.timestamp + 1u; }
-					w.timestamp += 1;
-					WAVE_FENCE();
-				}
-				PROF_ADD( 2);
+				const u32 lbase = (u32)(tile - lbeg) + k;
+				bool go;
+				if (!SPEC::SPECIAL) go = oneEvent<BODY_SWITCH>( L, w, P, lx, seg, kBegin, kCount, kStop, k, lbase, curPosition);
+				else if (__builtin_expect( w.spill != 0, 0)) go = oneEvent<BODY_SPILL>( L, w, P, lx, seg, kBegin, kCount, kStop, k, lbase, curPosition);
+				else go = oneEvent<BODY_LDS>( L, w, P, lx, seg, kBegin, kCount, kStop, k, lbase, curPosition);
+				if (!go) break;
 				++nEvents;
 			}
 		}
 
 		PROF_DECL;
 		u32 nres = w.err ? 0 : w.nStaged;
-		const u32 nitems = (w.err || !P.io.withItems) ? 0 : w.nStagedItems;
+		const u32 nitems = (w.err || !withItemsOf( P)) ? 0 : w.nStagedItems;
 		u64 resBase = 0, itemBase = 0;
 		if (nres && !reserveOutput( P.io, SPC_RESULTS, nres, resBase)) { w.err = SPD_ERR_OUTPUT; nres = 0; }
 		if (nres && nitems && !reserveOutput( P.io, SPC_ITEMS, nitems, itemBase)) { w.err = SPD_ERR_OUTPUT; nres = 0; }
@@ -1229,17 +1259,17 @@
 					s0.x = handle; s0.y = fmt;
 					s1.x = n | (vv[ 0] << 8) | (vv[ 1] << 16) | (vv[ 2] << 24); s1.y = ll[ 0]; s1.z = ll[ 1]; s1.w = ll[ 2];
 				}
-				const u32 ni = P.io.withItems ? (s1.x & 0xFFu) : 0u;
+				const u32 ni = withItemsOf( P) ? (s1.x & 0xFFu) : 0u;
 				u32 incl = waveScanAdd( ni);
 				const u64 mine = ip + (incl - ni);
 				if (hv)
 				{
 					const uint4 a = ((const uint4*)P.io.lexems)[ lbeg + s0.z], z = ((const uint4*)P.io.lexems)[ lbeg + s0.w];
-					const u32 sa = P.io.origseg ? P.io.origseg[ lbeg + s0.z] : 0u, sz = P.io.origseg ? P.io.origseg[ lbeg + s0.w] : 0u;
+					const u32 sa = hasOrigseg( P) ? origsegOf( P)[ lbeg + s0.z] : 0u, sz = hasOrigseg( P) ? origsegOf( P)[ lbeg + s0.w] : 0u;
 					u32* o = P.io.results + (resBase + ri)*9;
 					o[0] = s0.x; o[1] = a.y; o[2] = z.y + 1u; o[3] = sa; o[4] = a.z; o[5] = sz; o[6] = z.z + z.w;
-					o[7] = P.io.withItems ? (u32)mine : 0u; o[8] = ni;
-					if (P.io.withFormats) P.io.resultFormat[ resBase + ri] = s0.y;
+					o[7] = withItemsOf( P) ? (u32)mine : 0u; o[8] = ni;
+					if (withFormatsOf( P)) P.io.resultFormat[ resBase + ri] = s0.y;
 					const u32 il[ 3] = {s1.y, s1.z, s1.w};
 #pragma unroll
 					for (int q=0; q<3; ++q)
@@ -1247,10 +1277,10 @@
 						if ((u32)q < ni)
 						{
 							const uint4 t = ((const uint4*)P.io.lexems)[ lbeg + il[ q]];
-							const u32 st = P.io.origseg ? P.io.origseg[ lbeg + il[ q]] : 0u;
+							const u32 st = hasOrigseg( P) ? origsegOf( P)[ lbeg + il[ q]] : 0u;
 							u32* io = P.io.items + (mine + (u32)q)*7;
 							io[0] = (s1.x >> (8 + 8*q)) & 0xFFu; io[1] = t.y; io[2] = t.y + 1u; io[3] = st; io[4] = t.z; io[5] = st; io[6] = t.z + t.w;
-							if (P.io.withFormats) { P.io.itemFormat[ 2*(mine + (u32)q)] = 0; P.io.itemFormat[ 2*(mine + (u32)q)+1] = 0; }
+							if (withFormatsOf( P)) { P.io.itemFormat[ 2*(mine + (u32)q)] = 0; P.io.itemFormat[ 2*(mine + (u32)q)+1] = 0; }
 						}
 					}
 				}
@@ -1281,39 +1311,37 @@
 #define SPA_L2_FAST_WAVES_PER_EU 4
 #endif
 #define SPA_L2_FAST_OCC __attribute__((amdgpu_waves_per_eu( SPA_L2_FAST_WAVES_PER_EU, SPA_L2_FAST_WAVES_PER_EU)))
-#define SPA_FAST_VARIANTS( V) \
-	V( s, 192, 312) \
-	V( m, 320, 512) \
-	V( l, 512, 1024) \
-	V( t, 8, 128)		 \
-	V( n, 256, 448)
 #define SPA_FAST_INSTANCE( X, RR, TT) \
-	extern "C" __global__ __launch_bounds__(64) SPA_L2_FAST_OCC void spa_l2_fast_kernel_##X( FastParams kernelArgs) { Engine<RR,TT>::runKernel(); }
+	extern "C" __global__ __launch_bounds__(64) SPA_L2_FAST_OCC void spa_l2_fast_kernel_##X( FastParams kernelArgs) { Engine<RR,TT,SpecGeneral>::runKernel(); }
+#define SPA_FAST_SPECIAL( X, RR, TT, TWO, COMPACT, ITEMS, FORMATS, ORIGSEG, EXPSHIFT) \
+	extern "C" __global__ __launch_bounds__(64) SPA_L2_FAST_OCC void spa_l2_fast_kernel_##X( FastParams kernelArgs) { Engine<RR,TT,Spec<TWO,COMPACT,ITEMS,FORMATS,ORIGSEG,EXPSHIFT> >::runKernel(); }
 SPA_FAST_VARIANTS( SPA_FAST_INSTANCE)
+SPA_FAST_SPECIALISED( SPA_FAST_SPECIAL)
 
 namespace spa {
-struct FastVariant { void (*kernel)( FastParams); uint32_t R, T; const char* name; };
-#define SPA_FAST_ENTRY( X, RR, TT) {spa_l2_fast_kernel_##X, RR, TT, "spa_l2_fast_kernel_" #X},
-static const FastVariant fastVariants[ FAST_VARIANTS] = { SPA_FAST_VARIANTS( SPA_FAST_ENTRY) };
-static const FastVariant& fastVariantOf( unsigned variant) { return fastVariants[ variant < FAST_VARIANTS ? variant : FAST_VARIANTS-1]; }
+typedef void (*FastKernel)( FastParams);
+#define SPA_FAST_ENTRY( X, RR, TT) spa_l2_fast_kernel_##X,
+#define SPA_FAST_ENTRY_SPECIAL( X, RR, TT, TWO, COMPACT, ITEMS, FORMATS, ORIGSEG, EXPSHIFT) spa_l2_fast_kernel_##X,
+static const FastKernel fastKernels[ FAST_INSTANCES] = { SPA_FAST_VARIANTS( SPA_FAST_ENTRY) SPA_FAST_SPECIALISED( SPA_FAST_ENTRY_SPECIAL) };
+static FastKernel fastKernelOf( unsigned instance) { return fastKernels[ instance < FAST_INSTANCES ? instance : FAST_VARIANTS-1]; }
 
 unsigned fastVariantNamed( const char* size)
 {
-	for (unsigned v=0; v<FAST_VARIANTS; ++v) if (size[ 0] == fastVariants[ v].name[ sizeof("spa_l2_fast_kernel_")-1]) return v;
+	for (unsigned v=0; v<FAST_VARIANTS; ++v) if (size[ 0] == fastInstanceDesc( v).name[ sizeof("spa_l2_fast_kernel_")-1]) return v;
 	return FAST_VARIANTS-1;
 }
-const char* fastKernelName( unsigned variant) { return fastVariantOf( variant).name; }
-void fastCapacities( unsigned variant, uint32_t& R, uint32_t& T) { R = fastVariantOf( variant).R; T = fastVariantOf( variant).T; }
-int fastBlocksPerCU( unsigned variant)
+const char* fastKernelName( unsigned instance) { return fastInstanceDesc( instance).name; }
+void fastCapacities( unsigned variant, uint32_t& R, uint32_t& T) { R = fastInstanceDesc( variant).R; T = fastInstanceDesc( variant).T; }
+int fastBlocksPerCU( unsigned instance)
 {
 	int n = 0;
-	if (hipOccupancyMaxActiveBlocksPerMultiprocessor( &n, (const void*)fastVariantOf( variant).kernel, 64, 0) != hipSuccess || n < 1) n = 1;
+	if (hipOccupancyMaxActiveBlocksPerMultiprocessor( &n, (const void*)fastKernelOf( instance), 64, 0) != hipSuccess || n < 1) n = 1;
 	if (n > 32) n = 32;
 	return n;
 }
-hipError_t launchL2Fast( const FastParams& P, unsigned variant, unsigned nblocks, hipStream_t stream)
-{
-	hipLaunchKernelGGL( fastVariantOf( variant).kernel, dim3( nblocks), dim3( 64), 0, stream, P);
+hipError_t launchL2Fast( const FastParams& P, unsigned instance, unsigned nblocks, hipStream_t stream)
+{
+	hipLaunchKernelGGL( fastKernelOf( instance), dim3( nblocks), dim3( 64), 0, stream, P);
 	return hipGetLastError();
 }
 }
diff --git a/struspattern_amd/csrc/l2_fast_tables.cpp b/struspattern_amd/csrc/l2_fast_tables.cpp
--- a/struspattern_amd/csrc/l2_fast_tables.cpp
+++ b/struspattern_amd/csrc/l2_fast_tables.cpp
@@ -231,4 +231,57 @@
 	S.totalWords = (w + 63u) & ~63u;
 }
 
-}
+void fastFactsOf( const FlatTables& ft, const std::vector<FastKeyInst>& keyinst, const std::vector<FastStatic>* statics, FastFacts& facts)
+{
+	std::memset( &facts, 0, sizeof(facts));
+	for (size_t ei=0; ei<ft.keytab.size(); ++ei)
+	{
+		const DevKeyEntry& e = ft.keytab[ ei];
+		if (!e.event || e.listBegin + (size_t)e.listCount > keyinst.size()) continue;
+		for (uint32_t k=0; k<e.listCount; ++k)
+		{
+			const FastKeyInst& ki = keyinst[ e.listBegin + k];
+			const uint32_t ntrig = (ki.meta >> FKI_NTRIG_SHIFT) & FKI_NTRIG_MASK, rg = (ki.meta >> FKI_RANGE_SHIFT) & FKI_RANGE_MASK;
+			facts.lines += 1;
+			if (ntrig > facts.maxTriggers) facts.maxTriggers = ntrig;
+			if (rg > facts.maxRange) facts.maxRange = rg;
+			if (ki.pastEvent) facts.altKeyLines += 1;
+			if (k % 64u) continue;
+			const bool isStatic = (ki.flags & FKF_BATCH_STATIC) != 0;
+			const bool compact = isStatic && statics && ((*statics)[ e.listBegin + k].misc & FSM_BATCH_COMPACT);
+			facts.batches += 1;
+			if (compact) facts.compactBatches += 1; else if (isStatic) facts.staticBatches += 1; else facts.dynamicBatches += 1;
+		}
+	}
+	while ((1u << facts.expShift) < facts.maxRange + 1u) ++facts.expShift;
+}
+
+static const FastInstanceDesc fastInstanceDescs[ FAST_INSTANCES] = {
+#define SPA_FAST_DESC_GENERAL( X, RR, TT) {"spa_l2_fast_kernel_" #X, RR, TT, 0, 0, -1, -1, -1, -1},
+#define SPA_FAST_DESC_SPECIAL( X, RR, TT, TWO, COMPACT, ITEMS, FORMATS, ORIGSEG, EXPSHIFT) {"spa_l2_fast_kernel_" #X, RR, TT, TWO, COMPACT, ITEMS, FORMATS, ORIGSEG, EXPSHIFT},
+	SPA_FAST_VARIANTS( SPA_FAST_DESC_GENERAL)
+	SPA_FAST_SPECIALISED( SPA_FAST_DESC_SPECIAL)
+};
+const FastInstanceDesc& fastInstanceDesc( unsigned instance) { return fastInstanceDescs[ instance < FAST_INSTANCES ? instance : FAST_VARIANTS-1]; }
+
+unsigned fastSelectInstance( unsigned variant, const FastFacts* facts, const FastLaunchFacts* launch, bool generic)
+{
+	if (variant >= FAST_VARIANTS) variant = FAST_VARIANTS-1;
+	if (generic || !facts || !launch || !facts->maxTriggers) return variant;
+	const FastInstanceDesc& g = fastInstanceDescs[ variant];
+	for (unsigned i=FAST_VARIANTS; i<FAST_INSTANCES; ++i)
+	{
+		const FastInstanceDesc& d = fastInstanceDescs[ i];
+		if (d.R != g.R || d.T != g.T) continue;
+		if (d.two && facts->maxTriggers > 2) continue;
+		if (d.compact && facts->staticBatches != 0) continue;
+		if (d.expShift >= 0 && (uint32_t)d.expShift != facts->expShift) continue;
+		if (d.items >= 0 && (d.items != 0) != (launch->withItems != 0)) continue;
+		if (d.formats >= 0 && (d.formats != 0) != (launch->withFormats != 0)) continue;
+		if (d.origseg >= 0 && (d.origseg != 0) != (launch->hasOrigseg != 0)) continue;
+		return i;
+	}
+	return variant;
+}
+
+}
```
